# vaultah/replicat

Hardware: AMD Instinct MI355X
Metric: GiB/s chunked, device-resident streams (higher is better)
Workload: dtype u8

## Files before the change

include/replicat_chunker.h:

```cpp
#ifndef REPLICAT_CHUNKER_H
#define REPLICAT_CHUNKER_H

#include <stdint.h>

#ifdef __cplusplus
extern "C" {
#endif

#define RC_OK 0
#define RC_ERR_KEY_LENGTH 1
#define RC_ERR_MIN_GT_MAX 2
#define RC_ERR_BAD_KEY 3
#define RC_ERR_ARGUMENT 10
#define RC_ERR_ALIGN 11
#define RC_ERR_HIP 12
#define RC_ERR_OVERFLOW 13
#define RC_ERR_NO_DEVICE 14
#define RC_ERR_DEVICE_FAULT 15

#define RC_COUNT_OVERFLOW (-1)
#define RC_COUNT_FAULT (-3)

#define RC_OPEN 1u
#define RC_PIPELINED 2u
#define RC_PIPELINE_END 4u

typedef struct rc_chunker rc_chunker;

int rc_version(void);

const char *rc_build_id(void);

const char *rc_last_error(void);

int rc_chunker_create(uint64_t min_length, uint64_t max_length, const uint8_t *key,
                      uint64_t key_len, int device, rc_chunker **out);
void rc_chunker_destroy(rc_chunker *ch);

uint64_t rc_chunker_min_length(const rc_chunker *ch);
uint64_t rc_chunker_max_length(const rc_chunker *ch);

int rc_next_cut(rc_chunker *ch, const uint8_t *buffer, uint64_t size, int final,
                uint64_t *out_cut);

uint64_t rc_cut_capacity(const rc_chunker *ch, uint64_t n, const uint64_t *lens,
                         uint64_t *caps );

int rc_chunk_device(rc_chunker *ch, uint64_t n, const uint8_t *const *d_streams,
                    const uint64_t *lens, const uint64_t *last_piece, uint32_t flags,
                    uint64_t *d_cuts, int64_t *d_counts, void *hip_stream);

int rc_chunker_overlap(rc_chunker *ch, uint32_t reserve_cus);
uint32_t rc_chunker_overlap_cus(const rc_chunker *ch);
uint64_t rc_chunker_pipelined_calls(const rc_chunker *ch);

int rc_chunk_wait(rc_chunker *ch, void *hip_stream);

int rc_stream_create(int device, void **out_stream);
void rc_stream_destroy(void *stream);

int rc_chunk_host(rc_chunker *ch, uint64_t n, const uint8_t *const *streams,
                  const uint64_t *lens, const uint64_t *last_piece, uint32_t flags,
                  uint64_t *cuts, int64_t *counts);

int rc_chunker_check(rc_chunker *ch);

int rc_timing_enable(rc_chunker *ch, int enable);
int rc_timing_read_kernels(rc_chunker *ch, double *tile_ms, double *edge_ms, double *chain_ms,
                           uint64_t *calls);
int rc_timing_read(rc_chunker *ch, double *phase_a_ms, double *phase_b_ms, uint64_t *calls);

int rc_fill_splitmix(uint8_t *d_dst, uint64_t nbytes, uint64_t seed, uint64_t stream,
                     void *hip_stream);
int rc_fill_splitmix_streams(uint8_t *d_dst, uint64_t n, uint64_t nbytes, uint64_t slot,
                             uint64_t seed, uint64_t first_stream, uint64_t stream_step,
                             void *hip_stream);
int rc_fill_splitmix_at(uint8_t *d_dst, uint64_t nbytes, uint64_t seed, uint64_t stream,
                        uint64_t word0, void *hip_stream);

int rc_read_probe(const uint8_t *d_src, uint64_t nbytes, uint32_t *d_out, void *hip_stream);
int rc_chunker_read_probe(rc_chunker *ch, const uint8_t *d_src, uint64_t nbytes, uint32_t *d_out,
                          void *hip_stream);

uint64_t rc_keys_needed(uint64_t max_length, uint64_t L, uint64_t P);

uint64_t rc_host_key(const rc_chunker *ch, uint64_t d);

int rc_tile_records(rc_chunker *ch, uint64_t n, const uint8_t *const *d_streams,
                    const uint64_t *lens, const uint64_t *last_piece, uint64_t *keys,
                    uint64_t *js, uint64_t *gmax, uint64_t *ghot, uint64_t cap,
                    uint64_t *n_tiles);
uint32_t rc_group_hot_threshold(const rc_chunker *ch);
uint64_t rc_tile_keys(void);

int rc_tile_schedule(uint64_t n_tiles, uint32_t waves, uint32_t permille, uint32_t chunk,
                     uint32_t dyn_min, uint32_t *ranges, uint64_t cap, uint64_t *n_units);

int rc_tables_key(const uint8_t *key16, uint64_t n, const uint64_t *ds, uint64_t *out,
                  uint32_t *top16);

#ifdef __cplusplus
}
#endif

#endif
```

replicat_amd/_lib.py:

```python
import ctypes
import os
import threading

HERE = os.path.dirname(os.path.abspath(__file__))
LIB_PATH = os.environ.get('RC_LIB_PATH') or os.path.join(HERE, 'libreplicat_chunker.so')

RC_OK = 0
RC_ERR_KEY_LENGTH = 1
RC_ERR_MIN_GT_MAX = 2
RC_ERR_BAD_KEY = 3
RC_ERR_DIGEST_SIZE = 4
RC_ERR_B2_PARAM = 5
RC_ERR_KEY_SIZE = 6
RC_ERR_NONCE_SIZE = 7
RC_ERR_TAG = 8
RC_ERR_DIGEST_BITS = 9
RC_ERR_ARGUMENT = 10
RC_ERR_ALIGN = 11
RC_ERR_HIP = 12
RC_ERR_OVERFLOW = 13
RC_ERR_NO_DEVICE = 14
RC_ERR_DEVICE_FAULT = 15
RC_ERR_CORRUPT = 16
RC_ERR_INDEX_FULL = 17
RC_ERR_PROBE_BOUND = 18
RC_INDEX_ABSENT, RC_INDEX_EXHAUSTED = -1, -2
RC_GC_REFERENCED, RC_GC_DELETE, RC_GC_TAG_MISMATCH, RC_GC_EXHAUSTED = 0, 1, 2, 3
RC_COUNT_OVERFLOW = -1
RC_COUNT_FAULT = -3
RC_OPEN = 1
RC_PIPELINED = 2
RC_PIPELINE_END = 4
RC_DIGEST_SLOT = 64
RC_HASH_BLAKE2B, RC_HASH_SHA2, RC_HASH_SHA3 = 0, 1, 2
RC_CIPHER_NONE, RC_CIPHER_AES_GCM, RC_CIPHER_CHACHA20_POLY1305 = 0, 1, 2
RC_CHUNK_OK, RC_CHUNK_BAD_TAG, RC_CHUNK_CORRUPT = 0, 1, 2
RC_TABLE_OK, RC_TABLE_BAD_TAG, RC_TABLE_NOT_CANONICAL = 0, 1, 2
RC_PARTS_OK, RC_PARTS_NOT_CANONICAL = 0, 2
RC_PART_FIRST, RC_PART_LAST = 1, 2
RC_SNAPSHOT_PART_WORDS = 8
RC_SNAPSHOT_TEXT_DESC_BYTES = 32

_u64, _i64, _u32, _int, _p = ctypes.c_uint64, ctypes.c_int64, ctypes.c_uint32, ctypes.c_int, ctypes.c_void_p
SIGNATURES = {
    'rc_version': (_int, []),
    'rc_build_id': (ctypes.c_char_p, []),
    'rc_last_error': (ctypes.c_char_p, []),
    'rc_chunker_create': (_int, [_u64, _u64, _p, _u64, _int, ctypes.POINTER(_p)]),
    'rc_chunker_destroy': (None, [_p]),
    'rc_chunker_min_length': (_u64, [_p]),
    'rc_chunker_max_length': (_u64, [_p]),
    'rc_next_cut': (_int, [_p, _p, _u64, _int, ctypes.POINTER(_u64)]),
    'rc_cut_capacity': (_u64, [_p, _u64, _p, _p]),
    'rc_chunk_device': (_int, [_p, _u64, _p, _p, _p, _u32, _p, _p, _p]),
    'rc_chunk_host': (_int, [_p, _u64, _p, _p, _p, _u32, _p, _p]),
    'rc_chunker_overlap': (_int, [_p, _u32]),
    'rc_chunker_overlap_cus': (_u32, [_p]),
    'rc_chunker_pipelined_calls': (_u64, [_p]),
    'rc_chunker_check': (_int, [_p]),
    'rc_chunk_wait': (_int, [_p, _p]),
    'rc_stream_create': (_int, [_int, ctypes.POINTER(_p)]),
    'rc_stream_destroy': (None, [_p]),
    'rc_timing_enable': (_int, [_p, _int]),
    'rc_timing_read': (_int, [_p, ctypes.POINTER(ctypes.c_double), ctypes.POINTER(ctypes.c_double),
                              ctypes.POINTER(_u64)]),
    'rc_timing_read_kernels': (_int, [_p, ctypes.POINTER(ctypes.c_double),
                                      ctypes.POINTER(ctypes.c_double),
                                      ctypes.POINTER(ctypes.c_double), ctypes.POINTER(_u64)]),
    'rc_fill_splitmix': (_int, [_p, _u64, _u64, _u64, _p]),
    'rc_fill_splitmix_at': (_int, [_p, _u64, _u64, _u64, _u64, _p]),
    'rc_fill_splitmix_streams': (_int, [_p, _u64, _u64, _u64, _u64, _u64, _u64, _p]),
    'rc_read_probe': (_int, [_p, _u64, _p, _p]),
    'rc_chunker_read_probe': (_int, [_p, _p, _u64, _p, _p]),
    'rc_keys_needed': (_u64, [_u64, _u64, _u64]),
    'rc_host_key': (_u64, [_p, _u64]),
    'rc_tables_key': (_int, [_p, _u64, _p, _p, _p]),
    'rc_tile_records': (_int, [_p, _u64, _p, _p, _p, _p, _p, _p, _p, _u64, ctypes.POINTER(_u64)]),
    'rc_group_hot_threshold': (_u32, [_p]),
    'rc_tile_keys': (_u64, []),
    'rc_tile_schedule': (_int, [_u64, _u32, _u32, _u32, _u32, _p, _u64, ctypes.POINTER(_u64)]),
    'rc_blake2b_create': (_int, [_u32, _int, ctypes.POINTER(_p)]),
    'rc_blake2b_destroy': (None, [_p]),
    'rc_blake2b_digest_size': (_u32, [_p]),
    'rc_blake2b_device': (_int, [_p, _u64, _p, _p, _p, _p]),
    'rc_blake2b_host': (_int, [_p, _u64, _p, _p, _p]),
    'rc_blake2b_chunks': (_int, [_p, _p, _u64, _p, _p, _p, _p, _p, _p]),
    'rc_chunk_digest_host': (_int, [_p, _p, _u64, _p, _p, _p, _u32, _p, _p, _p]),
    'rc_blake2b_state_init': (_int, [_u32, _p, _u32, _p, _u32, _p, _u32, _p]),
    'rc_blake2b_update_device': (_int, [_p, _u64, _p, _p, _p, _p, _p, _p]),
    'rc_blake2b_timing_enable': (_int, [_p, _int]),
    'rc_blake2b_timing_read': (_int, [_p, ctypes.POINTER(ctypes.c_double), ctypes.POINTER(_u64)]),
    'rc_blake2b_derive_chunks': (_int, [_p, _p, _u64, _p, _p, _p, _p, _u32, _p, _p]),
    'rc_sha2_create': (_int, [_u32, _int, ctypes.POINTER(_p)]),
    'rc_sha3_create': (_int, [_u32, _int, ctypes.POINTER(_p)]),
    'rc_sha2_state_init': (_int, [_u32, _p]),
    'rc_sha3_state_init': (_int, [_u32, _p]),
    'rc_hash_destroy': (None, [_p]),
    'rc_hash_digest_size': (_u32, [_p]),
    'rc_hash_algorithm': (_u32, [_p]),
    'rc_hash_device': (_int, [_p, _u64, _p, _p, _p, _p]),
    'rc_hash_host': (_int, [_p, _u64, _p, _p, _p]),
    'rc_hash_chunks': (_int, [_p, _p, _u64, _p, _p, _p, _p, _p, _p]),
    'rc_hash_update_device': (_int, [_p, _u64, _p, _p, _p, _p, _p, _p]),
    'rc_hash_timing_enable': (_int, [_p, _int]),
    'rc_hash_timing_read': (_int, [_p, ctypes.POINTER(ctypes.c_double), ctypes.POINTER(_u64)]),
    'rc_gcm_create': (_int, [_u32, _u32, _int, ctypes.POINTER(_p)]),
    'rc_gcm_destroy': (None, [_p]),
    'rc_gcm_key_bytes': (_u32, [_p]),
    'rc_gcm_nonce_bytes': (_u32, [_p]),
    'rc_gcm_encrypt_device': (_int, [_p, _u64, _p, _p, _p, _p, _p, _p]),
    'rc_gcm_decrypt_device': (_int, [_p, _u64, _p, _p, _p, _p, _p, _p]),
    'rc_gcm_encrypt_host': (_int, [_p, _u64, _p, _p, _p, _p, _p]),
    'rc_gcm_decrypt_host': (_int, [_p, _u64, _p, _p, _p, _p, _p]),
    'rc_gcm_chunks_layout': (_u64, [_p, _p, _u64, _p, _p]),
    'rc_gcm_encrypt_chunks': (_int, [_p, _p, _u64, _p, _p, _p, _p, _p, _p, _p, _p]),
    'rc_gcm_encrypt_chunks_select': (_int, [_p, _p, _u64, _p, _p, _p, _p, _p, _p, _p, _p, _p, _p, _p]),
    'rc_gcm_timing_enable': (_int, [_p, _int]),
    'rc_gcm_timing_read': (_int, [_p, ctypes.POINTER(ctypes.c_double), ctypes.POINTER(_u64)]),
    'rc_chacha_create': (_int, [_int, ctypes.POINTER(_p)]),
    'rc_chacha_destroy': (None, [_p]),
    'rc_chacha_key_bytes': (_u32, [_p]),
    'rc_chacha_nonce_bytes': (_u32, [_p]),
    'rc_chacha_encrypt_device': (_int, [_p, _u64, _p, _p, _p, _p, _p, _p]),
    'rc_chacha_decrypt_device': (_int, [_p, _u64, _p, _p, _p, _p, _p, _p]),
    'rc_chacha_encrypt_host': (_int, [_p, _u64, _p, _p, _p, _p, _p]),
    'rc_chacha_decrypt_host': (_int, [_p, _u64, _p, _p, _p, _p, _p]),
    'rc_chacha_chunks_layout': (_u64, [_p, _p, _u64, _p, _p]),
    'rc_chacha_encrypt_chunks': (_int, [_p, _p, _u64, _p, _p, _p, _p, _p, _p, _p, _p]),
    'rc_chacha_encrypt_chunks_select': (_int, [_p, _p, _u64, _p, _p, _p, _p, _p, _p, _p, _p, _p, _p, _p]),
    'rc_chacha_timing_enable': (_int, [_p, _int]),
    'rc_chacha_timing_read': (_int, [_p, ctypes.POINTER(ctypes.c_double), ctypes.POINTER(_u64)]),
    'rc_poly1305_host': (_int, [_u64, _p, _p, _p, _p]),
    'rc_restore_create': (_int, [_p, _int, _p, _p, ctypes.POINTER(_p)]),
    'rc_restore_destroy': (None, [_p]),
    'rc_restore_overhead': (_u32, [_p]),
    'rc_restore_verify_device': (_int, [_p, _u64, _p, _p, _p, _p, _p, _p]),
    'rc_restore_verify_host': (_int, [_p, _u64, _p, _p, _p, _p, _p]),
    'rc_restore_timing_enable': (_int, [_p, _int]),
    'rc_restore_timing_read': (_int, [_p, ctypes.POINTER(ctypes.c_double), ctypes.POINTER(_u64)]),
    'rc_index_create': (_int, [_u32, _u64, _int, ctypes.POINTER(_p)]),
    'rc_index_destroy': (None, [_p]),
    'rc_index_name_bytes': (_u32, [_p]),
    'rc_index_used': (_u64, [_p]),
    'rc_index_add_host': (_int, [_p, _u64, _p, ctypes.POINTER(_u64)]),
    'rc_index_resolve_chunks': (_int, [_p, _p, _u64, _p, _p, _p, ctypes.POINTER(_u64), _p, _p, _p]),
    'rc_index_reserve': (_int, [_p, _u64]),
    'rc_index_lookup_device': (_int, [_p, _u64, _p, _p, _p]),
    'rc_index_resolve_names_device': (_int, [_p, _u64, _p, ctypes.POINTER(_u64), _p, _p, _p]),
    'rc_gc_create': (_int, [_u32, _u32, _p, _u32, _u64, _int, ctypes.POINTER(_p)]),
    'rc_gc_destroy': (None, [_p]),
    'rc_gc_name_bytes': (_u32, [_p]),
    'rc_gc_used': (_u64, [_p]),
    'rc_gc_capacity': (_u64, [_p]),
    'rc_gc_reference_host': (_int, [_p, _u64, _p]),
    'rc_gc_reference_device': (_int, [_p, _u64, _p]),
    'rc_gc_sweep_device': (_int, [_p, _u64, _p, _p, _u64, _p, _p, _p, _p]),
    'rc_gc_sweep_host': (_int, [_p, _u64, _p, _p, _p, _p, ctypes.POINTER(_u64)]),
    'rc_gc_unreferenced_host': (_int, [_p, _u64, _p, _p, _p, _p, ctypes.POINTER(_u64)]),
    'rc_gc_timing_enable': (_int, [_p, _int]),
    'rc_gc_timing_read': (_int, [_p, ctypes.POINTER(ctypes.c_double), ctypes.POINTER(ctypes.c_double),
                                 ctypes.POINTER(ctypes.c_double), ctypes.POINTER(_u64)]),
    'rc_snapshot_create': (_int, [_u32, _int, _p, _p, _int, ctypes.POINTER(_p)]),
    'rc_snapshot_destroy': (None, [_p]),
    'rc_snapshot_stride': (_u32, [_p]),
    'rc_snapshot_overhead': (_u32, [_p]),
    'rc_snapshot_table_count': (_u64, [_p, _u64]),
    'rc_snapshot_table_count_for': (_u64, [_u32, _u64]),
    'rc_snapshot_tables_device': (_int, [_p, _u64, _p, _p, _p, _p, _p, _p, _p, _p]),
    'rc_snapshot_tables_host': (_int, [_p, _u64, _p, _p, _p, _p, _p, _p]),
    'rc_snapshot_b64_device': (_int, [_p, _u64, _p, _p, _p, _p, _p]),
    'rc_snapshot_timing_enable': (_int, [_p, _int]),
    'rc_snapshot_timing_read': (_int, [_p, ctypes.POINTER(ctypes.c_double), ctypes.POINTER(ctypes.c_double),
                                       ctypes.POINTER(ctypes.c_double), ctypes.POINTER(_u64)]),
    'rc_snapshot_table_len': (_u64, [_p, _u64]),
    'rc_snapshot_table_len_for': (_u64, [_u32, _u64]),
    'rc_snapshot_b64_len': (_u64, [_u64]),
    'rc_snapshot_b64_encode_device': (_int, [_p, _u64, _p, _p, _p, _p]),
    'rc_snapshot_seal_tables_device': (_int, [_p, _u64, _p, _p, _p, _p, _p, _p, _p, _p]),
    'rc_snapshot_seal_tables_host': (_int, [_p, _u64, _p, _p, _p, _p, _p]),
    'rc_snapshot_write_timing_read': (_int, [_p, ctypes.POINTER(ctypes.c_double), ctypes.POINTER(ctypes.c_double),
                                             ctypes.POINTER(ctypes.c_double), ctypes.POINTER(_u64)]),
    'rc_snapshot_part_len_for': (_u32, [_u32, _u32, _u32, _u32]),
    'rc_snapshot_parts_capacity': (_u64, [_u64, _u64]),
    'rc_snapshot_parts_device': (_int, [_p, _u64, _p, _p, _u32, _u64, _p, _p, _p, _p, _p, _p, _p]),
    'rc_snapshot_data_len_device': (_int, [_p, _u64, _u64, _p, _p, _p, _p, _p, _p, _p]),
    'rc_snapshot_encode_data_device': (_int, [_p, _u64, _u64, _p, _p, _p, _p, _p, _p, _p, _p]),
    'rc_snapshot_data_timing_read': (_int, [_p, ctypes.POINTER(ctypes.c_double), ctypes.POINTER(ctypes.c_double),
                                            ctypes.POINTER(ctypes.c_double), ctypes.POINTER(_u64)]),
    'rc_snapshot_path_text_len_for': (_u64, [_p, _u64]),
    'rc_snapshot_int64_len_for': (_u32, [ctypes.c_int64]),
    'rc_snapshot_file_text_len_device': (_int, [_p, _u64, _p, _p, _p, _u32, _p, _p, _p, _u64, _u64, _p, _p]),
    'rc_snapshot_encode_file_text_device': (_int, [_p, _u64, _p, _p, _p, _u32, _p, _p, _p, _p, _u64, _p, _u64, _p, _p,
                                                   _p]),
    'rc_snapshot_file_text_timing_read': (_int, [_p, ctypes.POINTER(ctypes.c_double), ctypes.POINTER(ctypes.c_double),
                                                 ctypes.POINTER(_u64)]),
    'rc_snapshot_parts_room': (_u64, [_u64]),
    'rc_snapshot_find_parts_device': (_int, [_p, _u64, _p, _p, _p, _p, _p, _p, _p, _p]),
    'rc_snapshot_parse_parts_device': (_int, [_p, _u64, _p, _u64, _p, _p, _p, _p, _p, _p, _p, _p]),
    'rc_snapshot_part_sums_device': (_int, [_p, _u64, _u64, _p, _p, _p, _p, _p, _p, _p, _p, _p, _p, _p, _p]),
    'rc_snapshot_strip_parts_device': (_int, [_p, _u64, _p, _u64, _p, _p, _p, _p, _p, _p, _p, _p, _p]),
    'rc_snapshot_read_timing_read': (_int, [_p, ctypes.POINTER(ctypes.c_double), ctypes.POINTER(ctypes.c_double),
                                            ctypes.POINTER(ctypes.c_double), ctypes.POINTER(ctypes.c_double),
                                            ctypes.POINTER(_u64)]),
}



class ChunkerUnavailable(RuntimeError):
    """The HIP chunker library is not built or cannot run here."""


class ChunkerError(RuntimeError):
    def __init__(self, code, message):
        super().__init__(f'{message} (rc={code})')
        self.code = code


class ChunkCorrupted(ChunkerError):
    """A chunk's digest is not the one the snapshot recorded (RC_ERR_CORRUPT): the reference's
    ReplicatError('Chunk at ... is corrupted') (repository.py:1738-1739)."""


class ChunkerFault(ChunkerError):
    """The tile kernel took its fail-safe stop (RC_ERR_DEVICE_FAULT, RC_COUNT_FAULT): the call's
    cuts are not the reference's and must not be used."""


class IndexFull(ChunkerError):
    """A call would take a chunk-name index past its max_names (RC_ERR_INDEX_FULL): reserve()
    more room first."""


def check_counts(counts):
    import numpy as np
    c = np.asarray(counts).reshape(-1)
    if c.size == 0 or int(c.min()) >= 0:
        return
    if (c == RC_COUNT_FAULT).any():
        raise ChunkerFault(RC_ERR_DEVICE_FAULT, 'tile kernel fail-safe stop: a workgroup grab was '
                           'never published, so the call\'s cuts are not the reference\'s')
    raise ChunkerError(RC_ERR_OVERFLOW, f'stream {int(np.argmax(c < 0))} overflowed its cut capacity')


_lock = threading.Lock()
_lib = None


def lib():
    global _lib
    if _lib is not None:
        return _lib
    with _lock:
        if _lib is None:
            if not os.path.exists(LIB_PATH):
                raise ChunkerUnavailable(
                    f'{LIB_PATH} is missing: build it with `python -m replicat_amd.build` '
                    '(hipcc, gfx950); there is no CPU fallback')
            try:
                L = ctypes.CDLL(LIB_PATH)
            except OSError as e:
                raise ChunkerUnavailable(f'cannot load {LIB_PATH}: {e}') from e
            for name, (res, args) in SIGNATURES.items():
                f = getattr(L, name)
                f.restype = res
                f.argtypes = args
            _lib = L
    return _lib


def last_error():
    msg = lib().rc_last_error()
    return msg.decode('utf-8', 'replace') if msg else ''


def check(code):
    if code == RC_OK:
        return
    msg = last_error()
    if code in (RC_ERR_KEY_LENGTH, RC_ERR_MIN_GT_MAX, RC_ERR_BAD_KEY, RC_ERR_DIGEST_SIZE,
                RC_ERR_B2_PARAM, RC_ERR_KEY_SIZE, RC_ERR_NONCE_SIZE, RC_ERR_DIGEST_BITS):
        raise ValueError(msg)
    if code == RC_ERR_NO_DEVICE:
        raise ChunkerUnavailable(msg)
    if code == RC_ERR_DEVICE_FAULT:
        raise ChunkerFault(code, msg)
    if code == RC_ERR_CORRUPT:
        raise ChunkCorrupted(code, msg)
    if code == RC_ERR_INDEX_FULL:
        raise IndexFull(code, msg)
    raise ChunkerError(code, msg)
```

replicat_amd/csrc/capi.cpp:

```cpp
#include <hip/hip_runtime.h>

#include <algorithm>
#include <array>
#include <cstdarg>
#include <cstdio>
#include <cstdlib>
#include <cstring>
#include <mutex>
#include <vector>

#include "../../include/replicat_chunker.h"
#include "capi_internal.h"
#include "gclmul.h"
#include "knobs.h"

using namespace rc;

static_assert(kCountFault == RC_COUNT_FAULT && kCtrFaultsWord * 4 < 256, "counter buffer layout");

constexpr uint64_t kDigestSlot = RC_DIGEST_SLOT;

namespace {

thread_local char g_err[512];

void clmul64(uint64_t a, uint64_t b, uint64_t &lo, uint64_t &hi) {
    lo = hi = 0;
    for (int i = 0; i < 64; ++i)
        if ((b >> i) & 1) {
            lo ^= a << i;
            if (i) hi ^= a >> (64 - i);
        }
}

uint64_t key_linear(uint64_t k0, uint64_t d) {
    uint64_t lo, hi, rlo, rhi;
    clmul64(k0, d, lo, hi);
    clmul64(0x1B, hi, rlo, rhi);
    return lo ^ rlo;
}

void build_tables(uint64_t k0, uint64_t k1, KeyTables &t) {
    uint64_t col[64];
    for (int c = 0; c < 64; ++c) col[c] = key_linear(k0, 1ull << c);
    for (int b = 0; b < 4; ++b)
        for (int v = 0; v < 256; ++v) {
            uint64_t l = 0, h = 0;
            for (int i = 0; i < 8; ++i)
                if ((v >> i) & 1) {
                    l ^= col[8 * b + i];
                    h ^= col[32 + 8 * b + i];
                }
            if (b == 0) h ^= k1;
            t.tl[b][v] = l;
            t.th[b][v] = h;
            t.pf[b][v] = (uint32_t)((l >> 48) << 16) | (uint32_t)(h >> 48);
        }
}

uint64_t load_le64(const uint8_t *p) {
    uint64_t v = 0;
    for (int i = 7; i >= 0; --i) v = (v << 8) | p[i];
    return v;
}

uint64_t window_keys(uint64_t max_length) { return max_length >= 1 ? (max_length - 1) / 4 : 0; }

}

int rc_fail(int code, const char *fmt, ...) {
    va_list ap;
    va_start(ap, fmt);
    vsnprintf(g_err, sizeof g_err, fmt, ap);
    va_end(ap);
    return code;
}

namespace {

struct LiveHandle {
    void *h;
    void (*destroy)(void *);
};
std::mutex g_live_mu;
std::vector<LiveHandle> *g_live = nullptr;
bool g_exiting = false;

void destroy_live_at_exit() {
    std::vector<LiveHandle> left;
    {
        std::lock_guard<std::mutex> lock(g_live_mu);
        g_exiting = true;
        if (g_live) left.swap(*g_live);
    }
    for (auto it = left.rbegin(); it != left.rend(); ++it) it->destroy(it->h);
}

}

void rc_track(void *handle, void (*destroy)(void *)) {
    std::lock_guard<std::mutex> lock(g_live_mu);
    if (!g_live) {
        g_live = new std::vector<LiveHandle>();
        std::atexit(destroy_live_at_exit);
    }
    g_live->push_back({handle, destroy});
}

void rc_untrack(void *handle) {
    std::lock_guard<std::mutex> lock(g_live_mu);
    if (!g_live || g_exiting) return;
    for (size_t i = 0; i < g_live->size(); ++i)
        if ((*g_live)[i].h == handle) {
            (*g_live)[i] = g_live->back();
            g_live->pop_back();
            return;
        }
}

struct rc_chunker {
    uint64_t min_length = 0, max_length = 0, window = 0;
    bool small = false;
    bool groups = false;
    uint64_t seg_force = 0, ext_steps = 2;
    uint64_t seg_floor = 2;
    uint64_t k0 = 0, k1 = 0;
    int device = 0;
    Knobs knobs;
    TileSched sched;
    KeyTables tables;
    KeyTables *d_tables = nullptr;
    std::mutex mu;

    struct Workspace {
        PinnedBuf h_desc;
        DevBuf d_desc;
        DevBuf d_records;
        DevBuf d_scratch;
        DevBuf d_seg_counts;
        DevBuf d_ctr;
        bool ctr_dirty = false;
        uint64_t epoch = 0;
        std::vector<uint64_t> xtiles;
        hipEvent_t done = nullptr;
        bool pending = false;
        bool piped = false;
    } ws[2];
    unsigned next_ws = 0;

    DevBuf d_buf, d_out;
    PinnedBuf h_out;

    DevBuf d_stage[2], d_hcuts[2], d_hcounts[2], d_hdig[2];
    hipStream_t hstream[2] = {nullptr, nullptr};

    hipStream_t cstream = nullptr;
    hipEvent_t uploaded[2] = {nullptr, nullptr};

    uint32_t reserve_req = 0;
    uint32_t reserve = 0, tile_cus = 0;
    hipStream_t tstream = nullptr, xstream = nullptr;
    hipStream_t tstream2 = nullptr;
    hipStream_t fstream = nullptr;
    hipEvent_t in_ev[2] = {nullptr, nullptr}, tiled[2] = {nullptr, nullptr};
    uint64_t pipelined_calls = 0;
    bool overlap_failed = false;

    bool timing = false;
    std::vector<hipEvent_t> ev_pool, ev_pool_sync;
    std::vector<std::array<hipEvent_t, 4>> ev_rec;
};

namespace {

struct Plan {
    uint64_t n = 0, n_tiles = 0, total_cap = 0, max_len = 0;
    uint64_t n_segs = 0, scratch_entries = 0;
    uint64_t seg_bytes = 0, seg_cap = 0;
    bool any_multi = false;
    size_t bytes = 0;
};

StreamDesc desc_view(void *base, uint64_t n) {
    uint64_t *u = static_cast<uint64_t *>(base);
    StreamDesc d;
    d.ptr = reinterpret_cast<const uint8_t *const *>(u);
    d.len = u + n;
    d.last = u + 2 * n;
    d.jneed = u + 3 * n;
    d.tile_base = u + 4 * n;
    d.cut_base = u + 5 * n + 1;
    d.cut_cap = u + 6 * n + 1;
    d.seg_base = u + 7 * n + 1;
    d.scratch_base = u + 8 * n + 2;
    d.xtiles = u + 9 * n + 2;
    return d;
}

bool argmax_bound(uint64_t max_length, uint64_t L, uint64_t P, uint64_t &bound) {
    bool any = false;
    bound = 0;
    if (P >= max_length) {
        any = true;
        bound = P - max_length;
    }
    if (L >= 2 * max_length) {
        const uint64_t b2 = L - 2 * max_length;
        if (!any || b2 > bound) bound = b2;
        any = true;
    }
    return any;
}

uint64_t cut_cap_of(uint64_t min_length, uint64_t L) {
    const uint64_t step = std::max<uint64_t>(4, (min_length + 3) & ~3ull);
    return L / step + 3;
}

int validate_streams(uint64_t n, const uint8_t *const *ptrs, const uint64_t *lens,
                     const uint64_t *last, bool device_aligned) {
    if (n && (!ptrs || !lens)) return rc_fail(RC_ERR_ARGUMENT, "null stream arrays");
    if (n >= (1ull << 31))
        return rc_fail(RC_ERR_ARGUMENT, "too many streams in one call: %llu", (unsigned long long)n);
    for (uint64_t i = 0; i < n; ++i) {
        const uint64_t P = last ? last[i] : 0;
        if (P > lens[i]) return rc_fail(RC_ERR_ARGUMENT, "stream %llu: last piece start %llu > length %llu",
                                        (unsigned long long)i, (unsigned long long)P,
                                        (unsigned long long)lens[i]);
        if (lens[i] && !ptrs[i]) return rc_fail(RC_ERR_ARGUMENT, "stream %llu: null pointer", (unsigned long long)i);
        if (device_aligned && lens[i] && (reinterpret_cast<uintptr_t>(ptrs[i]) & 15))
            return rc_fail(RC_ERR_ALIGN, "stream %llu: device pointer not 16-byte aligned",
                           (unsigned long long)i);
    }
    return 0;
}

using Workspace = rc_chunker::Workspace;

Workspace &acquire_ws(rc_chunker *ch) {
    Workspace &w = ch->ws[ch->next_ws & 1];
    ++ch->next_ws;
    return w;
}

int stage_descriptors(rc_chunker *ch, Workspace &ws, uint64_t n, const uint8_t *const *ptrs,
                      const uint64_t *lens, const uint64_t *last, Plan &plan, bool open = false,
                      bool single = false, uint64_t walkers = 0) {
    plan.n = n;
    if (ws.pending) {
        RC_HIP_TRY(hipEventSynchronize(ws.done));
        ws.pending = false;
    }
    std::vector<uint64_t> &xt = ws.xtiles;
    xt.clear();
    {
        uint64_t tiles = 0;
        for (uint64_t i = 0; i < n; ++i) {
            const uint64_t L = lens[i], P = open ? L : (last ? last[i] : 0);
            const uint64_t jneed = rc_keys_needed(ch->max_length, L, P);
            const uint64_t nt = jneed ? jneed / kTileKeys + 1 : 0;
            const uint64_t jmax = L >= 8 ? (L - 4) / 4 : 0;
            auto fast = [&](uint64_t t) { return L >= 8 && t * kTileKeys + kTileKeys - 1 <= jmax; };
            if (nt && !fast(0)) xt.push_back(tiles);
            if (nt > 1 && !fast(nt - 1)) xt.push_back(tiles + nt - 1);
            tiles += nt;
        }
    }
    plan.bytes = (9 * n + 3 + xt.size()) * sizeof(uint64_t);
    if (int rc = ws.h_desc.ensure(plan.bytes)) return rc;
    uint64_t *u = static_cast<uint64_t *>(ws.h_desc.p);
    u[9 * n + 2] = xt.size();
    std::copy(xt.begin(), xt.end(), u + 9 * n + 3);
    {
        const uint64_t kChainWalkers = walkers ? walkers : 4096;
        uint64_t total = 0;
        for (uint64_t i = 0; i < n; ++i) {
            uint64_t b = 0;
            const uint64_t P = open ? lens[i] : (last ? last[i] : 0);
            if (argmax_bound(ch->max_length, lens[i], P, b)) total += b;
        }
        uint64_t seg = ch->seg_force ? ch->seg_force
                                     : std::max<uint64_t>(total / kChainWalkers / 4 * 5 + 4, 1);
        const uint64_t floor_len =
            ch->max_length < (1ull << 60) ? ch->seg_floor * ch->max_length : ~0ull >> 2;
        if (!ch->seg_force) seg = std::max(seg, std::max<uint64_t>(floor_len, 4ull << 20));
        seg = std::max<uint64_t>((seg + 3) & ~3ull, 4);
        const uint64_t step = std::max<uint64_t>(4, (ch->min_length + 3) & ~3ull);
        plan.seg_bytes = seg;
        plan.seg_cap = seg / step + ch->ext_steps + 4;
    }
    uint64_t tiles = 0, cuts = 0, segs = 0, scratch = 0;
    plan.any_multi = false;
    for (uint64_t i = 0; i < n; ++i) {
        const uint64_t L = lens[i], P = open ? L : (last ? last[i] : 0);
        uint64_t bound = 0, nseg = 1;
        if (!single && argmax_bound(ch->max_length, L, P, bound)) nseg = bound / plan.seg_bytes + 1;
        u[7 * n + 1 + i] = segs;
        u[8 * n + 2 + i] = scratch;
        segs += nseg;
        if (nseg > 1) {
            scratch += nseg * plan.seg_cap;
            plan.any_multi = true;
        }
        const uint64_t jneed = rc_keys_needed(ch->max_length, L, P);
        plan.max_len = std::max(plan.max_len, L);
        u[i] = reinterpret_cast<uint64_t>(ptrs[i]);
        u[n + i] = L;
        u[2 * n + i] = P;
        u[3 * n + i] = jneed;
        u[4 * n + i] = tiles;
        tiles += jneed ? jneed / kTileKeys + 1 : 0;
        const uint64_t cap = cut_cap_of(ch->min_length, L);
        u[5 * n + 1 + i] = cuts;
        u[6 * n + 1 + i] = cap;
        cuts += cap;
    }
    u[5 * n] = tiles;
    u[8 * n + 1] = segs;
    if (tiles >= (1ull << 32) - (1ull << 20))
        return rc_fail(RC_ERR_ARGUMENT, "too many bytes in one call: %llu tiles", (unsigned long long)tiles);
    plan.n_tiles = tiles;
    plan.total_cap = cuts;
    plan.n_segs = segs;
    plan.scratch_entries = scratch;
    return 0;
}

GroupRecord *group_records(Workspace &ws, const Plan &plan) {
    return reinterpret_cast<GroupRecord *>(static_cast<char *>(ws.d_records.p) +
                                           (plan.n_tiles + 1) * sizeof(TileRecord));
}

uint32_t *tie_lists(Workspace &ws, const Plan &plan) {
    return reinterpret_cast<uint32_t *>(group_records(ws, plan) + plan.n_tiles + 1);
}

size_t records_bytes(const Plan &plan) {
    return (plan.n_tiles + 1) * (sizeof(TileRecord) + sizeof(GroupRecord)) +
           rc_tie_list_words(plan.n_tiles) * 4;
}

int ensure_ctr(Workspace &ws, hipStream_t st) {
    size_t zero = kCtrFaultsWord * 4;
    if (!ws.d_ctr.p) {
        if (int rc = ws.d_ctr.ensure(256)) return rc;
        ws.ctr_dirty = true;
        zero = 256;
    }
    if (ws.ctr_dirty) {
        RC_HIP_TRY(hipMemsetAsync(ws.d_ctr.p, 0, zero, st));
        ws.ctr_dirty = false;
    }
    return 0;
}

const char kFaultMsg[] =
    "tile kernel fail-safe stop: a workgroup grab was never published, so the launch's records "
    "are incomplete and its cuts are not the reference's";

int grab_fault(Workspace &ws) {
    if (!ws.d_ctr.p || !ws.epoch) return 0;
    uint64_t stamp = 0;
    RC_HIP_TRY(hipMemcpy(&stamp, static_cast<uint32_t *>(ws.d_ctr.p) + kCtrStampWord, 8,
                         hipMemcpyDeviceToHost));
    return stamp == ws.epoch ? rc_fail(RC_ERR_DEVICE_FAULT, "%s", kFaultMsg) : 0;
}

int take_faults(Workspace &ws, uint32_t &n) {
    n = 0;
    if (!ws.d_ctr.p) return 0;
    uint32_t *w = static_cast<uint32_t *>(ws.d_ctr.p) + kCtrFaultsWord;
    RC_HIP_TRY(hipMemcpy(&n, w, 4, hipMemcpyDeviceToHost));
    if (n) RC_HIP_TRY(hipMemset(w, 0, 4));
    return 0;
}

int abandon_launch(Workspace &ws, hipStream_t ts, hipStream_t xs, int rc) {
    (void)hipStreamSynchronize(ts);
    if (xs != ts) (void)hipStreamSynchronize(xs);
    ws.ctr_dirty = true;
    ws.pending = false;
    return rc;
}

constexpr uint64_t kLaneMinStreams = 256;

int upload_and_launch(rc_chunker *ch, Workspace &ws, const Plan &plan, ChainParams prm,
                      uint64_t *d_cuts, int64_t *d_counts, hipStream_t stream,
                      bool pipelined = false, bool end = false) {
    if (int rc = ws.d_desc.ensure(plan.bytes)) return rc;
    if (int rc = ws.d_records.ensure(records_bytes(plan))) return rc;
    if (int rc = ws.d_scratch.ensure(std::max<uint64_t>(plan.scratch_entries, 1) * 8)) return rc;
    if (int rc = ws.d_seg_counts.ensure(std::max<uint64_t>(plan.n_segs, 1) * 40)) return rc;
    const int wi = &ws == &ch->ws[0] ? 0 : 1;
    if (!ch->cstream) RC_HIP_TRY(hipStreamCreateWithFlags(&ch->cstream, hipStreamNonBlocking));
    if (!ch->uploaded[wi]) RC_HIP_TRY(hipEventCreateWithFlags(&ch->uploaded[wi], hipEventDisableTiming));
    RC_HIP_TRY(hipMemcpyAsync(ws.d_desc.p, ws.h_desc.p, plan.bytes, hipMemcpyHostToDevice, ch->cstream));
    RC_HIP_TRY(hipEventRecord(ch->uploaded[wi], ch->cstream));
    hipStream_t ts = stream, xs = stream;
    if (pipelined) {
        ts = wi == 1 && ch->tstream2 ? ch->tstream2 : ch->tstream;
        xs = end ? ch->fstream : ch->xstream;
        if (hipStreamQuery(stream) != hipSuccess) {
            RC_HIP_TRY(hipEventRecord(ch->in_ev[wi], stream));
            RC_HIP_TRY(hipStreamWaitEvent(ts, ch->in_ev[wi], 0));
        }
        RC_HIP_TRY(hipStreamWaitEvent(xs, ch->ws[wi ^ 1].done, 0));
    }
    RC_HIP_TRY(hipStreamWaitEvent(ts, ch->uploaded[wi], 0));
    if (int rc = ensure_ctr(ws, ts)) return rc;
    prm.fault = reinterpret_cast<const uint64_t *>(static_cast<uint32_t *>(ws.d_ctr.p) + kCtrStampWord);
    prm.epoch = ++ws.epoch;
    const StreamDesc d = desc_view(ws.d_desc.p, plan.n);
    std::array<hipEvent_t, 4> ev{};
    if (ch->timing) {
        for (int k = 0; k < 4; ++k) {
            std::vector<hipEvent_t> &pool = k == 1 ? ch->ev_pool_sync : ch->ev_pool;
            if (pool.empty()) {
                RC_HIP_TRY(k == 1 ? hipEventCreate(&ev[k])
                                  : hipEventCreateWithFlags(&ev[k], hipEventDisableSystemFence));
            } else {
                ev[k] = pool.back();
                pool.pop_back();
            }
        }
        RC_HIP_TRY(hipEventRecord(ev[0], ts));
    }
    GroupRecord *grp = ch->groups ? group_records(ws, plan) : nullptr;
    prm.grp = grp;
    prm.n_tiles = plan.n_tiles;
    switch (ch->knobs[knLaneChain]) {
    case 1: prm.lane = 0u; break;
    case 2: prm.lane = 2u; break;
    default: prm.lane = plan.n >= kLaneMinStreams ? 1u : 0u;
    }
    prm.lean = ch->small && plan.max_len < (16ull << 30) ? 1u : 0u;
    prm.hot = group_hot_threshold(ch->window);
    if (int rc = rc_launch_tiles(ch->d_tables, d, plan.n, plan.n_tiles,
                                 static_cast<TileRecord *>(ws.d_records.p), grp, prm.hot, tie_lists(ws, plan),
                                 static_cast<uint32_t *>(ws.d_ctr.p), prm.epoch, ts,
                                 ch->timing ? ev[1] : nullptr,
                                 pipelined ? ch->tile_cus : 0u, xs,
                                 !pipelined ? nullptr : ch->timing ? ev[1] : ch->tiled[wi], ch->sched))
        return abandon_launch(ws, ts, xs, rc);
    const Workspace &prev = ch->ws[wi ^ 1];
    if (!pipelined && prev.piped && hipStreamWaitEvent(xs, prev.done, 0) != hipSuccess)
        return abandon_launch(ws, ts, xs, rc_fail(RC_ERR_HIP, "hipStreamWaitEvent failed"));
    if (ch->timing && hipEventRecord(ev[2], xs) != hipSuccess)
        return abandon_launch(ws, ts, xs, rc_fail(RC_ERR_HIP, "hipEventRecord failed"));
    const uint32_t join = (ch->knobs[knJoinWalk] ? RC_JOIN_WALK_ONLY : 0u) |
                          (ch->knobs[knRepair] ? RC_JOIN_REPAIR : 0u);
    if (int rc = rc_launch_chain(ch->d_tables, d, plan.n, prm, plan.n_segs,
                                 static_cast<const TileRecord *>(ws.d_records.p), d_cuts, d_counts,
                                 static_cast<uint64_t *>(ws.d_scratch.p),
                                 static_cast<uint64_t *>(ws.d_seg_counts.p), plan.any_multi, join, xs))
        return abandon_launch(ws, ts, xs, rc);
    if (hipEventRecord(ws.done, xs) != hipSuccess)
        return abandon_launch(ws, ts, xs, rc_fail(RC_ERR_HIP, "hipEventRecord failed"));
    ws.pending = true;
    ws.piped = pipelined;
    if (ch->timing) {
        RC_HIP_TRY(hipEventRecord(ev[3], xs));
        ch->ev_rec.push_back(ev);
    }
    return 0;
}

int setup_overlap(rc_chunker *ch) {
    const uint32_t want = ch->reserve_req ? ch->reserve_req : (uint32_t)ch->knobs[knOverlapCus];
    if (ch->tstream && ch->reserve == want) return 0;
    int cus = 0;
    RC_HIP_TRY(hipDeviceGetAttribute(&cus, hipDeviceAttributeMultiprocessorCount, ch->device));
    if (want == 0 || (int)want >= cus)
        return rc_fail(RC_ERR_ARGUMENT, "overlap: %u reserved CUs of %d", want, cus);
    if (ch->tstream) {
        if (ch->tstream2) {
            RC_HIP_TRY(hipStreamSynchronize(ch->tstream2));
            (void)hipStreamDestroy(ch->tstream2);
            ch->tstream2 = nullptr;
        }
        RC_HIP_TRY(hipStreamSynchronize(ch->tstream));
        RC_HIP_TRY(hipStreamSynchronize(ch->xstream));
        (void)hipStreamDestroy(ch->tstream);
        (void)hipStreamDestroy(ch->xstream);
        ch->tstream = ch->xstream = nullptr;
    }
    std::vector<uint32_t> tm((cus + 31) / 32, 0u), xm((cus + 31) / 32, 0u);
    for (int i = 0; i < cus; ++i) ((uint32_t)i < want ? xm : tm)[i / 32] |= 1u << (i % 32);
    const int64_t tmask = ch->knobs[knTileMask];
    if (tmask == 1)
        for (int i = 0; i < cus; ++i) tm[i / 32] |= 1u << (i % 32);
    if (tmask == 2)
        RC_HIP_TRY(hipStreamCreateWithFlags(&ch->tstream, hipStreamNonBlocking));
    else
        RC_HIP_TRY(hipExtStreamCreateWithCUMask(&ch->tstream, (uint32_t)tm.size(), tm.data()));
    const hipError_t ex = hipExtStreamCreateWithCUMask(&ch->xstream, (uint32_t)xm.size(), xm.data());
    if (ex != hipSuccess) {
        (void)hipStreamDestroy(ch->tstream);
        ch->tstream = ch->xstream = nullptr;
        return rc_fail(RC_ERR_HIP, "hipExtStreamCreateWithCUMask failed: %s", hipGetErrorString(ex));
    }
    if (ch->knobs[knTileStreams] == 2 &&
        (tmask == 2 ? hipStreamCreateWithFlags(&ch->tstream2, hipStreamNonBlocking)
                    : hipExtStreamCreateWithCUMask(&ch->tstream2, (uint32_t)tm.size(), tm.data())) !=
            hipSuccess)
        ch->tstream2 = nullptr;
    if (!ch->fstream) RC_HIP_TRY(hipStreamCreateWithFlags(&ch->fstream, hipStreamNonBlocking));
    for (int i = 0; i < 2; ++i) {
        if (!ch->in_ev[i]) RC_HIP_TRY(hipEventCreateWithFlags(&ch->in_ev[i], hipEventDisableTiming));
        if (!ch->tiled[i]) RC_HIP_TRY(hipEventCreateWithFlags(&ch->tiled[i], hipEventDisableTiming));
    }
    ch->reserve = want;
    ch->tile_cus = (uint32_t)cus - (tmask ? 0u : want);
    return 0;
}

ChainParams chain_params(const rc_chunker *ch, const Plan &plan, uint64_t max_steps,
                         uint32_t flags = 0) {
    ChainParams p;
    p.open = (flags & RC_OPEN) ? 1u : 0u;
    p.min_length = ch->min_length;
    p.max_length = ch->max_length;
    p.window = ch->window;
    p.max_steps = max_steps;
    p.seg_bytes = plan.seg_bytes;
    p.seg_cap = plan.seg_cap;
    p.ext_steps = ch->ext_steps;
    p.grp = nullptr;
    p.n_tiles = 0;
    p.lean = 0;
    p.lane = 0;
    p.hot = 0;
    p.fault = nullptr;
    p.epoch = 0;
    return p;
}

}

extern "C" {

int rc_version(void) { return 300; }

#ifndef RC_BUILD_ID
#define RC_BUILD_ID "unknown"
#endif
static const char kBuildId[] = "RC_BUILD_ID:" RC_BUILD_ID;
const char *rc_build_id(void) { return kBuildId + 12; }

const char *rc_last_error(void) { return g_err; }

uint32_t rc_group_hot_threshold(const rc_chunker *ch) { return ch ? group_hot_threshold(ch->window) : 0u; }

uint64_t rc_keys_needed(uint64_t max_length, uint64_t L, uint64_t P) {
    const uint64_t T = window_keys(max_length);
    if (T == 0 || L < 8) return 0;
    bool any = false;
    uint64_t bound = 0;
    if (P >= max_length) {
        any = true;
        bound = P - max_length;
    }
    if (L >= 2 * max_length) {
        const uint64_t b2 = L - 2 * max_length;
        if (!any || b2 > bound) bound = b2;
        any = true;
    }
    if (!any) return 0;
    const uint64_t jneed = bound / 4 + T, jmax = (L - 4) / 4;
    return std::min(jneed, jmax);
}

int rc_chunker_create(uint64_t min_length, uint64_t max_length, const uint8_t *key,
                      uint64_t key_len, int device, rc_chunker **out) {
    if (!out) return rc_fail(RC_ERR_ARGUMENT, "null output handle");
    *out = nullptr;
    if (key_len != 16 || !key) return rc_fail(RC_ERR_KEY_LENGTH, "key must contain exactly 16 characters");
    if (min_length > max_length)
        return rc_fail(RC_ERR_MIN_GT_MAX, "Minimum length is greater than the maximum one");
    const uint64_t k0 = load_le64(key), k1 = load_le64(key + 8);
    if (k0 == 0) return rc_fail(RC_ERR_BAD_KEY, "Bad key contents");
    Knobs knobs;
    if (read_knobs(knobs, g_err, sizeof g_err)) return RC_ERR_ARGUMENT;

    int ndev = 0;
    if (hipGetDeviceCount(&ndev) != hipSuccess || ndev <= 0)
        return rc_fail(RC_ERR_NO_DEVICE, "no HIP device available (the chunker runs on MI355X only)");
    if (device < 0 || device >= ndev) return rc_fail(RC_ERR_NO_DEVICE, "device %d out of range", device);
    hipDeviceProp_t prop;
    RC_HIP_TRY(hipGetDeviceProperties(&prop, device));
    if (std::strncmp(prop.gcnArchName, "gfx950", 6) != 0)
        return rc_fail(RC_ERR_NO_DEVICE, "device %d is %s, not gfx950", device, prop.gcnArchName);

    rc_chunker *ch = new rc_chunker();
    ch->min_length = min_length;
    ch->max_length = max_length;
    ch->window = window_keys(max_length);
    ch->knobs = knobs;
    ch->small = ch->window / kTileKeys + 3 <= 64;
    ch->groups = knobs[knTileGroups] == 0 ? ch->small : knobs[knTileGroups] == 2;
    if (knobs[knChainLean] == 1) ch->small = false;
    ch->sched.permille = (uint32_t)knobs[knTileStatic];
    ch->sched.chunk = (uint32_t)knobs[knTileChunk];
    ch->sched.dyn_min = (uint32_t)knobs[knTileDynMin];
    ch->sched.group = (uint32_t)knobs[knTileGroup];
    ch->k0 = k0;
    ch->k1 = k1;
    ch->device = device;
    build_tables(k0, k1, ch->tables);
    ch->seg_force = (uint64_t)knobs[knSegmentBytes];
    ch->ext_steps = (uint64_t)knobs[knSegmentExt];
    ch->seg_floor = (uint64_t)knobs[knSegmentFloor];
    {
        DeviceGuard g(device);
        hipError_t e = hipMalloc(&ch->d_tables, sizeof(KeyTables));
        if (e == hipSuccess)
            e = hipMemcpy(ch->d_tables, &ch->tables, sizeof(KeyTables), hipMemcpyHostToDevice);
        for (auto &w : ch->ws)
            if (e == hipSuccess) e = hipEventCreateWithFlags(&w.done, hipEventDisableTiming);
        if (e != hipSuccess) {
            rc_chunker_destroy(ch);
            return rc_fail(RC_ERR_HIP, "device setup failed: %s", hipGetErrorString(e));
        }
    }
    rc_track(ch, [](void *h) { rc_chunker_destroy(static_cast<rc_chunker *>(h)); });
    *out = ch;
    return RC_OK;
}

void rc_chunker_destroy(rc_chunker *ch) {
    if (!ch) return;
    teardown(ch, [ch] {
        if (ch->d_tables) (void)hipFree(ch->d_tables);
        for (auto &w : ch->ws) {
            w.d_desc.release();
            w.d_records.release();
            w.d_scratch.release();
            w.d_seg_counts.release();
            w.d_ctr.release();
            w.h_desc.release();
            if (w.done) (void)hipEventDestroy(w.done);
        }
        ch->d_buf.release();
        ch->d_out.release();
        for (int i = 0; i < 2; ++i) {
            ch->d_stage[i].release();
            ch->d_hcuts[i].release();
            ch->d_hcounts[i].release();
            ch->d_hdig[i].release();
            if (ch->hstream[i]) (void)hipStreamDestroy(ch->hstream[i]);
        }
        ch->h_out.release();
        if (ch->cstream) (void)hipStreamDestroy(ch->cstream);
        if (ch->tstream) (void)hipStreamDestroy(ch->tstream);
        if (ch->tstream2) (void)hipStreamDestroy(ch->tstream2);
        if (ch->xstream) (void)hipStreamDestroy(ch->xstream);
        if (ch->fstream) (void)hipStreamDestroy(ch->fstream);
        for (auto e : ch->uploaded)
            if (e) (void)hipEventDestroy(e);
        for (int i = 0; i < 2; ++i) {
            if (ch->in_ev[i]) (void)hipEventDestroy(ch->in_ev[i]);
            if (ch->tiled[i]) (void)hipEventDestroy(ch->tiled[i]);
        }
        for (auto &r : ch->ev_rec)
            for (auto e : r) (void)hipEventDestroy(e);
        for (auto e : ch->ev_pool) (void)hipEventDestroy(e);
        for (auto e : ch->ev_pool_sync) (void)hipEventDestroy(e);
    });
    delete ch;
}

uint64_t rc_chunker_min_length(const rc_chunker *ch) { return ch ? ch->min_length : 0; }
uint64_t rc_chunker_max_length(const rc_chunker *ch) { return ch ? ch->max_length : 0; }

uint64_t rc_host_key(const rc_chunker *ch, uint64_t d) {
    const uint32_t lo = (uint32_t)d, hi = (uint32_t)(d >> 32);
    uint64_t k = 0;
    for (int b = 0; b < 4; ++b) k ^= ch->tables.tl[b][(lo >> (8 * b)) & 255] ^ ch->tables.th[b][(hi >> (8 * b)) & 255];
    return k;
}

int rc_tables_key(const uint8_t *key16, uint64_t n, const uint64_t *ds, uint64_t *out,
                  uint32_t *top16) {
    if (!key16 || (n && (!ds || !out))) return rc_fail(RC_ERR_ARGUMENT, "null argument");
    KeyTables *t = new KeyTables;
    build_tables(load_le64(key16), load_le64(key16 + 8), *t);
    for (uint64_t i = 0; i < n; ++i) {
        const uint32_t lo = (uint32_t)ds[i], hi = (uint32_t)(ds[i] >> 32);
        uint64_t k = 0;
        uint32_t el = 0, eh = 0;
        for (int b = 0; b < 4; ++b) {
            k ^= t->tl[b][(lo >> (8 * b)) & 255] ^ t->th[b][(hi >> (8 * b)) & 255];
            el ^= t->pf[b][(lo >> (8 * b)) & 255];
            eh ^= t->pf[b][(hi >> (8 * b)) & 255];
        }
        out[i] = k;
        if (top16) top16[i] = ((el & 0xffff0000u) ^ (eh << 16)) >> 16;
    }
    delete t;
    return RC_OK;
}

uint64_t rc_cut_capacity(const rc_chunker *ch, uint64_t n, const uint64_t *lens, uint64_t *caps) {
    uint64_t total = 0;
    for (uint64_t i = 0; i < n; ++i) {
        const uint64_t c = cut_cap_of(ch->min_length, lens[i]);
        if (caps) caps[i] = c;
        total += c;
    }
    return total;
}

int rc_next_cut(rc_chunker *ch, const uint8_t *buffer, uint64_t size, int final, uint64_t *out_cut) {
    if (!ch || !out_cut) return rc_fail(RC_ERR_ARGUMENT, "null argument");
    if (size && !buffer) return rc_fail(RC_ERR_ARGUMENT, "null buffer");
    const uint64_t mn = ch->min_length, mx = ch->max_length;
    if (final && size < 2 * mx) {
        *out_cut = size <= mx ? size : (size < mx + mn ? size / 2 : mx);
        return RC_OK;
    }
    if (!final && size < mx) {
        *out_cut = 0;
        return RC_OK;
    }
    if (ch->window == 0) {
        *out_cut = (mn + 3) & ~3ull;
        return RC_OK;
    }
    std::lock_guard<std::mutex> lock(ch->mu);
    DeviceGuard g(ch->device);
    const uint64_t ncopy = std::min<uint64_t>(size, 4 * ch->window + 4);
    if (int rc = ch->d_buf.ensure(ncopy + 16)) return rc;
    if (int rc = ch->d_out.ensure(64)) return rc;
    if (int rc = ch->h_out.ensure(64)) return rc;
    hipStream_t stream = nullptr;
    RC_HIP_TRY(hipMemcpyAsync(ch->d_buf.p, buffer, ncopy, hipMemcpyHostToDevice, stream));
    const uint8_t *ptr = static_cast<const uint8_t *>(ch->d_buf.p);
    const uint64_t L = ncopy, P = ncopy;
    Plan plan;
    Workspace &ws = acquire_ws(ch);
    if (int rc = stage_descriptors(ch, ws, 1, &ptr, &L, &P, plan, false, true)) return rc;
    uint64_t *d_cut = static_cast<uint64_t *>(ch->d_out.p);
    int64_t *d_count = reinterpret_cast<int64_t *>(d_cut + 1);
    const bool timing = ch->timing;
    ch->timing = false;
    int rc = upload_and_launch(ch, ws, plan, chain_params(ch, plan, 0), d_cut, d_count, stream);
    ch->timing = timing;
    if (rc) return rc;
    RC_HIP_TRY(hipMemcpyAsync(ch->h_out.p, d_cut, 16, hipMemcpyDeviceToHost, stream));
    RC_HIP_TRY(hipStreamSynchronize(stream));
    const uint64_t *h = static_cast<const uint64_t *>(ch->h_out.p);
    if ((int64_t)h[1] == kCountFault) return rc_fail(RC_ERR_DEVICE_FAULT, "%s", kFaultMsg);
    if ((int64_t)h[1] != 1) return rc_fail(RC_ERR_OVERFLOW, "device chain returned %lld cuts", (long long)h[1]);
    *out_cut = h[0];
    return RC_OK;
}

int rc_chunk_device(rc_chunker *ch, uint64_t n, const uint8_t *const *d_streams,
                    const uint64_t *lens, const uint64_t *last_piece, uint32_t flags,
                    uint64_t *d_cuts, int64_t *d_counts, void *hip_stream) {
    if (!ch) return rc_fail(RC_ERR_ARGUMENT, "null chunker");
    if (n == 0) return RC_OK;
    if (!d_cuts || !d_counts) return rc_fail(RC_ERR_ARGUMENT, "null output arrays");
    const bool open = (flags & RC_OPEN) != 0;
    if (int rc = validate_streams(n, d_streams, lens, open ? nullptr : last_piece, true)) return rc;
    std::lock_guard<std::mutex> lock(ch->mu);
    DeviceGuard g(ch->device);
    const bool all = ch->knobs[knPipeAll] != 0;
    bool pipelined = (flags & RC_PIPELINED) != 0 && (all || !ch->groups);
    if (pipelined && !ch->overlap_failed && setup_overlap(ch) != 0) {
        ch->overlap_failed = true;
        fprintf(stderr, "replicat_amd: pipelined calls run in sequence: %s\n", g_err);
    }
    if (ch->overlap_failed && !ch->tstream) pipelined = false;
    if (pipelined && !all) {
        uint64_t tiles = 0;
        for (uint64_t i = 0; i < n; ++i) {
            const uint64_t P = open ? lens[i] : (last_piece ? last_piece[i] : 0);
            const uint64_t j = rc_keys_needed(ch->max_length, lens[i], P);
            tiles += j ? j / kTileKeys + 1 : 0;
        }
        if (tiles < 16ull * ch->tile_cus) pipelined = false;
    }
    ch->pipelined_calls += pipelined ? 1 : 0;
    Plan plan;
    Workspace &ws = acquire_ws(ch);
    if (int rc = stage_descriptors(ch, ws, n, d_streams, lens, last_piece, plan, open, false,
                                   pipelined ? 16ull * ch->reserve : 0))
        return rc;
    return upload_and_launch(ch, ws, plan, chain_params(ch, plan, ~0ull, flags), d_cuts, d_counts,
                             static_cast<hipStream_t>(hip_stream), pipelined,
                             (flags & RC_PIPELINE_END) != 0);
}

int rc_stream_create(int device, void **out_stream) {
    if (!out_stream) return rc_fail(RC_ERR_ARGUMENT, "null output stream");
    *out_stream = nullptr;
    if (int rc = check_device(device)) return rc;
    DeviceGuard g(device);
    int cus = 0;
    RC_HIP_TRY(hipDeviceGetAttribute(&cus, hipDeviceAttributeMultiprocessorCount, device));
    std::vector<uint32_t> mask((cus + 31) / 32, 0u);
    for (int i = 0; i < cus; ++i) mask[i / 32] |= 1u << (i % 32);
    hipStream_t s = nullptr;
    RC_HIP_TRY(hipExtStreamCreateWithCUMask(&s, (uint32_t)mask.size(), mask.data()));
    rc_track(s, [](void *h) { rc_stream_destroy(h); });
    *out_stream = s;
    return RC_OK;
}

void rc_stream_destroy(void *stream) {
    if (!stream) return;
    rc_untrack(stream);
    (void)hipStreamSynchronize(static_cast<hipStream_t>(stream));
    (void)hipStreamDestroy(static_cast<hipStream_t>(stream));
}

int rc_chunker_overlap(rc_chunker *ch, uint32_t reserve_cus) {
    if (!ch) return rc_fail(RC_ERR_ARGUMENT, "null chunker");
    std::lock_guard<std::mutex> lock(ch->mu);
    DeviceGuard g(ch->device);
    ch->reserve_req = reserve_cus;
    const int rc = setup_overlap(ch);
    ch->overlap_failed = rc != 0 && !ch->tstream;
    return rc;
}

uint32_t rc_chunker_overlap_cus(const rc_chunker *ch) { return ch ? ch->reserve : 0u; }

uint64_t rc_chunker_pipelined_calls(const rc_chunker *ch) { return ch ? ch->pipelined_calls : 0; }

int rc_chunker_check(rc_chunker *ch) {
    if (!ch) return rc_fail(RC_ERR_ARGUMENT, "null chunker");
    std::lock_guard<std::mutex> lock(ch->mu);
    DeviceGuard g(ch->device);
    uint32_t faults = 0;
    for (auto &w : ch->ws) {
        if (w.pending) RC_HIP_TRY(hipEventSynchronize(w.done));
        uint32_t n = 0;
        if (int rc = take_faults(w, n)) return rc;
        faults += n;
    }
    if (faults)
        return rc_fail(RC_ERR_DEVICE_FAULT, "%s (%u call(s) since the last check)", kFaultMsg, faults);
    return RC_OK;
}

int rc_chunk_wait(rc_chunker *ch, void *hip_stream) {
    if (!ch) return rc_fail(RC_ERR_ARGUMENT, "null chunker");
    std::lock_guard<std::mutex> lock(ch->mu);
    DeviceGuard g(ch->device);
    for (auto &w : ch->ws)
        RC_HIP_TRY(hipStreamWaitEvent(static_cast<hipStream_t>(hip_stream), w.done, 0));
    return RC_OK;
}

}

namespace {

int chunk_host_impl(rc_chunker *ch, rc_hasher *hasher, uint64_t n, const uint8_t *const *streams,
                    const uint64_t *lens, const uint64_t *last_piece, uint32_t flags,
                    uint64_t *cuts, int64_t *counts, uint8_t *digests) {
    if (!ch) return rc_fail(RC_ERR_ARGUMENT, "null chunker");
    if (n == 0) return RC_OK;
    if (!cuts || !counts) return rc_fail(RC_ERR_ARGUMENT, "null output arrays");
    if (hasher && !digests) return rc_fail(RC_ERR_ARGUMENT, "null digest array");
    const bool open = (flags & RC_OPEN) != 0;
    if (int rc = validate_streams(n, streams, lens, open ? nullptr : last_piece, false)) return rc;
    std::lock_guard<std::mutex> lock(ch->mu);
    DeviceGuard g(ch->device);
    for (int i = 0; i < 2; ++i)
        if (!ch->hstream[i]) RC_HIP_TRY(hipStreamCreateWithFlags(&ch->hstream[i], hipStreamNonBlocking));
    struct Drain {
        rc_chunker *ch;
        bool armed = true;
        ~Drain() {
            if (!armed) return;
            for (hipStream_t s : ch->hstream)
                if (s) (void)hipStreamSynchronize(s);
        }
    } drain{ch};

    const uint64_t budget = uint64_t(ch->knobs[knHostBatchBytes]);
    std::vector<uint64_t> cut_base(n + 1, 0);
    for (uint64_t i = 0; i < n; ++i) cut_base[i + 1] = cut_base[i] + cut_cap_of(ch->min_length, lens[i]);

    struct Batch {
        uint64_t first = 0, count = 0;
    } inflight[2];
    bool busy[2] = {false, false};
    std::vector<const uint8_t *> dptr;
    std::vector<uint64_t> off;

    auto finish = [&](int slot) -> int {
        if (!busy[slot]) return 0;
        RC_HIP_TRY(hipStreamSynchronize(ch->hstream[slot]));
        busy[slot] = false;
        const Batch &b = inflight[slot];
        for (uint64_t i = 0; i < b.count; ++i) {
            if (counts[b.first + i] == kCountFault) return rc_fail(RC_ERR_DEVICE_FAULT, "%s", kFaultMsg);
            if (counts[b.first + i] < 0)
                return rc_fail(RC_ERR_OVERFLOW, "stream %llu overflowed its cut capacity",
                               (unsigned long long)(b.first + i));
        }
        return 0;
    };

    uint64_t i = 0;
    int slot = 0;
    while (i < n) {
        uint64_t j = i, bytes = 0;
        while (j < n && (j == i || bytes + ((lens[j] + 15) & ~15ull) <= budget)) {
            bytes += (lens[j] + 15) & ~15ull;
            ++j;
        }
        if (int rc = finish(slot)) return rc;
        const uint64_t nb = j - i;
        if (int rc = ch->d_stage[slot].ensure(bytes + 16)) return rc;
        const uint64_t ncut = cut_base[j] - cut_base[i];
        if (int rc = ch->d_hcuts[slot].ensure(ncut * 8)) return rc;
        if (int rc = ch->d_hcounts[slot].ensure(nb * 8)) return rc;
        hipStream_t st = ch->hstream[slot];
        dptr.resize(nb);
        uint64_t o = 0;
        for (uint64_t k = 0; k < nb; ++k) {
            uint8_t *dst = static_cast<uint8_t *>(ch->d_stage[slot].p) + o;
            dptr[k] = dst;
            if (lens[i + k]) RC_HIP_TRY(hipMemcpyAsync(dst, streams[i + k], lens[i + k], hipMemcpyHostToDevice, st));
            o += (lens[i + k] + 15) & ~15ull;
        }
        Plan plan;
        Workspace &ws = acquire_ws(ch);
        if (int rc = stage_descriptors(ch, ws, nb, dptr.data(), lens + i,
                                       last_piece ? last_piece + i : nullptr, plan, open))
            return rc;
        uint64_t *dc = static_cast<uint64_t *>(ch->d_hcuts[slot].p);
        int64_t *dn = static_cast<int64_t *>(ch->d_hcounts[slot].p);
        if (int rc = upload_and_launch(ch, ws, plan, chain_params(ch, plan, ~0ull, flags), dc, dn, st))
            return rc;
        if (hasher) {
            if (int rc = ch->d_hdig[slot].ensure(ncut * kDigestSlot)) return rc;
            uint8_t *dd = static_cast<uint8_t *>(ch->d_hdig[slot].p);
            std::vector<uint64_t> cb(nb);
            for (uint64_t k = 0; k < nb; ++k) cb[k] = cut_base[i + k] - cut_base[i];
            uint64_t bytes = 0, longest = 0;
            for (uint64_t k = 0; k < nb; ++k) {
                bytes += lens[i + k];
                longest = std::max(longest, lens[i + k]);
            }
            if (int rc = rc_hasher_enqueue_chunks(hasher, nb, dptr.data(), cb.data(), dc, dn, ncut,
                                                  bytes, std::min(longest, ch->max_length), dd, st))
                return rc;
            RC_HIP_TRY(hipMemcpyAsync(digests + cut_base[i] * kDigestSlot, dd, ncut * kDigestSlot,
                                      hipMemcpyDeviceToHost, st));
        }
        RC_HIP_TRY(hipMemcpyAsync(cuts + cut_base[i], dc, ncut * 8, hipMemcpyDeviceToHost, st));
        RC_HIP_TRY(hipMemcpyAsync(counts + i, dn, nb * 8, hipMemcpyDeviceToHost, st));
        inflight[slot] = {i, nb};
        busy[slot] = true;
        i = j;
        slot ^= 1;
    }
    if (int rc = finish(0)) return rc;
    if (int rc = finish(1)) return rc;
    drain.armed = false;
    return RC_OK;
}

}

extern "C" {

int rc_chunk_host(rc_chunker *ch, uint64_t n, const uint8_t *const *streams, const uint64_t *lens,
                  const uint64_t *last_piece, uint32_t flags, uint64_t *cuts, int64_t *counts) {
    return chunk_host_impl(ch, nullptr, n, streams, lens, last_piece, flags, cuts, counts, nullptr);
}

int rc_chunk_digest_host(rc_chunker *ch, rc_hasher *h, uint64_t n, const uint8_t *const *streams,
                         const uint64_t *lens, const uint64_t *last_piece, uint32_t flags,
                         uint64_t *cuts, int64_t *counts, uint8_t *digests) {
    if (!h) return rc_fail(RC_ERR_ARGUMENT, "null hasher");
    return chunk_host_impl(ch, h, n, streams, lens, last_piece, flags, cuts, counts, digests);
}

uint64_t rc_tile_keys(void) { return kTileKeys; }

int rc_tile_records(rc_chunker *ch, uint64_t n, const uint8_t *const *d_streams,
                    const uint64_t *lens, const uint64_t *last_piece, uint64_t *keys,
                    uint64_t *js, uint64_t *gmax, uint64_t *ghot, uint64_t cap,
                    uint64_t *n_tiles) {
    if (!ch || !n_tiles) return rc_fail(RC_ERR_ARGUMENT, "null argument");
    if (int rc = validate_streams(n, d_streams, lens, last_piece, true)) return rc;
    std::lock_guard<std::mutex> lock(ch->mu);
    DeviceGuard g(ch->device);
    Plan plan;
    Workspace &ws = acquire_ws(ch);
    if (int rc = stage_descriptors(ch, ws, n, d_streams, lens, last_piece, plan)) return rc;
    if (int rc = ws.d_desc.ensure(plan.bytes)) return rc;
    if (int rc = ws.d_records.ensure(records_bytes(plan))) return rc;
    RC_HIP_TRY(hipMemcpy(ws.d_desc.p, ws.h_desc.p, plan.bytes, hipMemcpyHostToDevice));
    if (int rc = ensure_ctr(ws, nullptr)) return rc;
    GroupRecord *d_grp = ch->groups ? group_records(ws, plan) : nullptr;
    if (plan.n_tiles)
        RC_HIP_TRY(hipMemset(ws.d_records.p, 0xab, (plan.n_tiles + 1) * sizeof(TileRecord)));
    if (int rc = rc_launch_tiles(ch->d_tables, desc_view(ws.d_desc.p, n), n, plan.n_tiles,
                                 static_cast<TileRecord *>(ws.d_records.p), d_grp,
                                 group_hot_threshold(ch->window), tie_lists(ws, plan),
                                 static_cast<uint32_t *>(ws.d_ctr.p), ++ws.epoch, nullptr, nullptr, 0u,
                                 nullptr, nullptr, ch->sched))
        return abandon_launch(ws, nullptr, nullptr, rc);
    RC_HIP_TRY(hipDeviceSynchronize());
    if (int rc = grab_fault(ws)) return rc;
    std::vector<TileRecord> h(plan.n_tiles);
    std::vector<GroupRecord> hg(plan.n_tiles, GroupRecord{~0ull, {~0ull, ~0ull, ~0ull, ~0ull}, 0ull});
    if (plan.n_tiles) {
        RC_HIP_TRY(hipMemcpy(h.data(), ws.d_records.p, plan.n_tiles * sizeof(TileRecord),
                             hipMemcpyDeviceToHost));
        if (d_grp)
            RC_HIP_TRY(hipMemcpy(hg.data(), d_grp, plan.n_tiles * sizeof(GroupRecord), hipMemcpyDeviceToHost));
    }
    *n_tiles = plan.n_tiles;
    for (uint64_t t = 0; t < plan.n_tiles && t < cap; ++t) {
        keys[t] = h[t].key;
        js[t] = h[t].j;
        if (gmax) gmax[t] = hg[t].max;
        if (ghot)
            for (int g = 0; g < kTileGroups; ++g) ghot[kTileGroups * t + g] = hg[t].hot[g];
    }
    return RC_OK;
}

int rc_timing_enable(rc_chunker *ch, int enable) {
    if (!ch) return rc_fail(RC_ERR_ARGUMENT, "null chunker");
    ch->timing = enable != 0;
    return RC_OK;
}

int rc_timing_read_kernels(rc_chunker *ch, double *tile_ms, double *edge_ms, double *chain_ms,
                           uint64_t *calls) {
    if (!ch) return rc_fail(RC_ERR_ARGUMENT, "null chunker");
    std::lock_guard<std::mutex> lock(ch->mu);
    DeviceGuard g(ch->device);
    double t[3] = {0, 0, 0};
    for (auto &r : ch->ev_rec) {
        RC_HIP_TRY(hipEventSynchronize(r[3]));
        for (int k = 0; k < 3; ++k) {
            float x = 0;
            RC_HIP_TRY(hipEventElapsedTime(&x, r[k], r[k + 1]));
            t[k] += x;
        }
        for (int k = 0; k < 4; ++k) (k == 1 ? ch->ev_pool_sync : ch->ev_pool).push_back(r[k]);
    }
    if (tile_ms) *tile_ms = t[0];
    if (edge_ms) *edge_ms = t[1];
    if (chain_ms) *chain_ms = t[2];
    if (calls) *calls = ch->ev_rec.size();
    ch->ev_rec.clear();
    return RC_OK;
}

int rc_timing_read(rc_chunker *ch, double *phase_a_ms, double *phase_b_ms, uint64_t *calls) {
    double tile = 0, edge = 0, chain = 0;
    if (int rc = rc_timing_read_kernels(ch, &tile, &edge, &chain, calls)) return rc;
    if (phase_a_ms) *phase_a_ms = tile + edge;
    if (phase_b_ms) *phase_b_ms = chain;
    return RC_OK;
}

int rc_read_probe(const uint8_t *d_src, uint64_t nbytes, uint32_t *d_out, void *hip_stream) {
    if (nbytes && (!d_src || !d_out)) return rc_fail(RC_ERR_ARGUMENT, "null argument");
    if (reinterpret_cast<uintptr_t>(d_src) & 15) return rc_fail(RC_ERR_ALIGN, "source not 16-byte aligned");
    const Knobs &k = process_knobs();
    TileSched sched;
    sched.permille = (uint32_t)k[knTileStatic];
    sched.chunk = (uint32_t)k[knTileChunk];
    sched.dyn_min = (uint32_t)k[knTileDynMin];
    sched.group = (uint32_t)k[knTileGroup];
    return rc_launch_read_probe(d_src, nbytes, d_out, (uint32_t)k[knProbeBlock], sched, hip_stream);
}

int rc_chunker_read_probe(rc_chunker *ch, const uint8_t *d_src, uint64_t nbytes, uint32_t *d_out,
                          void *hip_stream) {
    if (!ch) return rc_fail(RC_ERR_ARGUMENT, "null chunker");
    if (nbytes && (!d_src || !d_out)) return rc_fail(RC_ERR_ARGUMENT, "null argument");
    if (reinterpret_cast<uintptr_t>(d_src) & 15) return rc_fail(RC_ERR_ALIGN, "source not 16-byte aligned");
    DeviceGuard g(ch->device);
    return rc_launch_read_probe(d_src, nbytes, d_out, 0, ch->sched, hip_stream);
}

int rc_fill_splitmix(uint8_t *d_dst, uint64_t nbytes, uint64_t seed, uint64_t stream, void *hip_stream) {
// ... 23 lines not shown
```

replicat_amd/csrc/gclmul.h:

```cpp
#pragma once
#include <stdint.h>

namespace rc {

#ifndef RC_TILE_ITERS
#define RC_TILE_ITERS 16
#endif
constexpr int kTileIters = RC_TILE_ITERS;
constexpr int kTileKeys = 64 * 4 * kTileIters;
constexpr int kWaveSize = 64;
constexpr int kTileWaves = 16;
constexpr int kChainWaves = 4;
#ifndef RC_TILE_GROUPS
#define RC_TILE_GROUPS 4
#endif
constexpr int kTileGroups = RC_TILE_GROUPS;
constexpr int kGroupKeys = kTileKeys / kTileGroups;

constexpr uint32_t kPfBytes = 131072;
constexpr uint32_t kFullOff = kPfBytes;
constexpr uint32_t kFullBytes = 2 * 4 * 256 * 8;
constexpr uint32_t kTileLdsBytes = kPfBytes + kFullBytes;

struct KeyTables {
    uint64_t tl[4][256];
    uint64_t th[4][256];
    uint32_t pf[4][256];
};

struct StreamDesc {
    const uint8_t *const *ptr;
    const uint64_t *len;
    const uint64_t *last;
    const uint64_t *jneed;
    const uint64_t *tile_base;
    const uint64_t *cut_base;
    const uint64_t *cut_cap;
    const uint64_t *seg_base;
    const uint64_t *scratch_base;
    const uint64_t *xtiles;
};

struct TileRecord {
    uint64_t key;
    uint64_t j;
};

struct GroupRecord {
    uint64_t max;
    uint64_t hot[kTileGroups];
    uint64_t pad;
};
static_assert(kTileGroups % 2 == 0 && sizeof(GroupRecord) % 16 == 0, "group record layout");

__host__ __device__ inline uint32_t group_hot_threshold(uint64_t window) {
    if (window < (uint64_t)kTileKeys) return 0;
    const uint64_t below = (10 * 65536 + window - 1) / window;
    return below >= 65536 ? 0u : (uint32_t)(65536 - below);
}

struct ChainParams {
    uint64_t min_length;
    uint64_t max_length;
    uint64_t window;
    uint64_t max_steps;
    uint64_t seg_bytes;
    uint64_t seg_cap;
    uint64_t ext_steps;
    const GroupRecord *grp;
    uint64_t n_tiles;
    uint32_t open;
    uint32_t lean;
    uint32_t lane;
    uint32_t hot;
    const uint64_t *fault;
    uint64_t epoch;
};

constexpr uint32_t kCtrErrWord = 32, kCtrStampWord = 34, kCtrFaultsWord = 36;
constexpr int64_t kCountFault = -3;

struct TileSched {
    uint32_t permille = 0;
    uint32_t chunk = 3;
    uint32_t dyn_min = 0;
    uint32_t group = 64;
};

__host__ __device__ inline uint64_t splitmix64(uint64_t x) {
    uint64_t z = x + 0x9E3779B97F4A7C15ull;
    z = (z ^ (z >> 30)) * 0xBF58476D1CE4E5B9ull;
    z = (z ^ (z >> 27)) * 0x94D049BB133111EBull;
    return z ^ (z >> 31);
}

}

extern "C" {
int rc_launch_tiles(const rc::KeyTables *d_tables, rc::StreamDesc desc, uint64_t n_streams,
                    uint64_t n_tiles, rc::TileRecord *d_records, rc::GroupRecord *d_grp,
                    uint32_t hot, uint32_t *d_xlist, uint32_t *d_ctr, uint64_t epoch,
                    void *stream, void *mid_event, uint32_t cus, void *edge_stream, void *tiled,
                    rc::TileSched sched);
uint64_t rc_tie_list_words(uint64_t n_tiles);
enum : uint32_t { RC_JOIN_WALK_ONLY = 1, RC_JOIN_REPAIR = 2 };
int rc_launch_chain(const rc::KeyTables *d_tables, rc::StreamDesc desc, uint64_t n_streams,
                    rc::ChainParams prm, uint64_t n_segs, const rc::TileRecord *d_records,
                    uint64_t *d_cuts, int64_t *d_counts, uint64_t *d_scratch,
                    uint64_t *d_seg_counts, bool any_multi, uint32_t join, void *stream);
int rc_launch_fill(uint8_t *d_dst, uint64_t nbytes, uint64_t seed, uint64_t stream_id,
                   uint64_t word0, void *stream);
int rc_launch_fill_streams(uint8_t *d_dst, uint64_t n, uint64_t nbytes, uint64_t slot,
                           uint64_t seed, uint64_t id0, uint64_t id_step, void *stream);
int rc_launch_read_probe(const uint8_t *d_src, uint64_t nbytes, uint32_t *d_out, uint32_t block,
                         rc::TileSched sched, void *stream);
}
```

replicat_amd/csrc/kernels.hip:

```cpp
#include <hip/hip_runtime.h>
#include <stdint.h>

#include "capi_internal.h"
#include "gclmul.h"
#include "diag.h"

using namespace rc;

namespace {

typedef uint32_t u32x4 __attribute__((ext_vector_type(4)));
typedef __attribute__((address_space(1))) const u32x4 gu32x4;
typedef __attribute__((address_space(1))) const uint32_t gu32;

constexpr int kStreamAux = RC_DIAG_STREAM_AUX;

__device__ __forceinline__ __amdgpu_buffer_rsrc_t tile_rsrc(const uint8_t *base,
                                                             uint32_t bytes = 0xffffffffu) {
    return __builtin_amdgcn_make_buffer_rsrc(const_cast<uint8_t *>(base), 0, bytes, 0x00020000);
}
__device__ __forceinline__ u32x4 ring_load(__amdgpu_buffer_rsrc_t r, uint32_t lane_off, int it) {
    return __builtin_amdgcn_raw_buffer_load_b128(r, lane_off, it * 1024, kStreamAux);
}

__device__ __forceinline__ uint32_t lane_id() { return threadIdx.x & 63; }

__device__ __forceinline__ uint32_t max3_u32(uint32_t a, uint32_t b, uint32_t c) {
    uint32_t r;
    asm("v_max3_u32 %0, %1, %2, %3" : "=v"(r) : "v"(a), "v"(b), "v"(c));
    return r;
}


__device__ __forceinline__ uint64_t lane_u64(uint64_t v, int l) {
    const uint32_t lo = (uint32_t)__builtin_amdgcn_readlane((uint32_t)v, l);
    const uint32_t hi = (uint32_t)__builtin_amdgcn_readlane((uint32_t)(v >> 32), l);
    return ((uint64_t)hi << 32) | lo;
}

typedef __attribute__((address_space(4))) const uint64_t cu64;
__device__ __forceinline__ uint64_t sload(const uint64_t *p) { return *(cu64 *)(p); }
__device__ __forceinline__ const uint8_t *sload_ptr(const uint8_t *const *p) {
    return reinterpret_cast<const uint8_t *>(sload(reinterpret_cast<const uint64_t *>(p)));
}

__device__ __forceinline__ uint32_t ld_u32(const uint8_t *p) {
    return *(gu32 *)(p);
}
__device__ __forceinline__ gu32x4 *as_global_x4(const uint8_t *p) { return (gu32x4 *)(p); }

__device__ __forceinline__ uint64_t full_key(const uint64_t *__restrict__ tl,
                                             const uint64_t *__restrict__ th, uint32_t wlo,
                                             uint32_t whi) {
    return tl[wlo & 255] ^ tl[256 + ((wlo >> 8) & 255)] ^ tl[512 + ((wlo >> 16) & 255)] ^
           tl[768 + (wlo >> 24)] ^ th[whi & 255] ^ th[256 + ((whi >> 8) & 255)] ^
           th[512 + ((whi >> 16) & 255)] ^ th[768 + (whi >> 24)];
}

template <int kCtrl, int kRowMask>
__device__ __forceinline__ uint64_t dpp_u64(uint64_t v) {
    const uint32_t lo = (uint32_t)__builtin_amdgcn_update_dpp((int)(uint32_t)v, (int)(uint32_t)v,
                                                              kCtrl, kRowMask, 0xf, false);
    const uint32_t hi = (uint32_t)__builtin_amdgcn_update_dpp((int)(uint32_t)(v >> 32),
                                                              (int)(uint32_t)(v >> 32), kCtrl,
                                                              kRowMask, 0xf, false);
    return ((uint64_t)hi << 32) | lo;
}

template <int kCtrl, int kRowMask>
__device__ __forceinline__ void best_step(uint64_t &k, uint64_t &j) {
    const uint64_t ko = dpp_u64<kCtrl, kRowMask>(k), jo = dpp_u64<kCtrl, kRowMask>(j);
    if (ko > k || (ko == k && jo < j)) {
        k = ko;
        j = jo;
    }
}

__device__ __forceinline__ void wave_best(uint64_t &k, uint64_t &j) {
    best_step<0x111, 0xf>(k, j);
    best_step<0x112, 0xf>(k, j);
    best_step<0x114, 0xf>(k, j);
    best_step<0x118, 0xf>(k, j);
    best_step<0x142, 0xa>(k, j);
    best_step<0x143, 0xc>(k, j);
    k = lane_u64(k, 63);
    j = lane_u64(j, 63);
}


__shared__ __attribute__((aligned(16))) uint32_t s_tile_lds[kTileLdsBytes / 4];

__device__ __forceinline__ uint32_t pf_lds(uint32_t byte_addr) {
    return *reinterpret_cast<const uint32_t *>(reinterpret_cast<const char *>(s_tile_lds) +
                                               byte_addr);
}

__device__ __forceinline__ void pf_addrs(uint32_t w, uint32_t lb_a, uint32_t lb_b, uint32_t *a) {
    a[0] = __builtin_amdgcn_perm(w, lb_a, 0x0c020400u);
    a[1] = __builtin_amdgcn_perm(w, lb_a, 0x0c020500u) + 128;
    a[2] = __builtin_amdgcn_perm(w, lb_b, 0x0c020600u);
    a[3] = __builtin_amdgcn_perm(w, lb_b, 0x0c020700u) + 128;
}
__device__ __forceinline__ uint32_t pf_gather(const uint32_t *a) {
    return __builtin_amdgcn_bitop3_b32(pf_lds(a[0]), pf_lds(a[1]), pf_lds(a[2]), 0x96) ^ pf_lds(a[3]);
}

__device__ __forceinline__ uint32_t pf_entry(uint32_t w, uint32_t lb_a, uint32_t lb_b) {
    const uint32_t a0 = __builtin_amdgcn_perm(w, lb_a, 0x0c020400u);
    const uint32_t a1 = __builtin_amdgcn_perm(w, lb_a, 0x0c020500u);
    const uint32_t a2 = __builtin_amdgcn_perm(w, lb_b, 0x0c020600u);
    const uint32_t a3 = __builtin_amdgcn_perm(w, lb_b, 0x0c020700u);
    return pf_lds(a0) ^ pf_lds(a1 + 128) ^ pf_lds(a2) ^ pf_lds(a3 + 128);
}

__shared__ __attribute__((aligned(16))) uint32_t s_chain_lds[1024 + 4096];

__device__ __forceinline__ uint32_t pfc_entry(const uint32_t *pf, uint32_t w) {
    return pf[w & 255] ^ pf[256 + ((w >> 8) & 255)] ^ pf[512 + ((w >> 16) & 255)] ^
           pf[768 + (w >> 24)];
}

__device__ __forceinline__ void stage_chain_tables(const KeyTables *tab) {
    const uint32_t nt = blockDim.x;
    const uint32_t *gpf = &tab->pf[0][0];
    for (uint32_t i = threadIdx.x; i < 1024u; i += nt) s_chain_lds[i] = gpf[i];
    uint64_t *full = reinterpret_cast<uint64_t *>(s_chain_lds + 1024);
    const uint64_t *gfull = &tab->tl[0][0];
    for (uint32_t i = threadIdx.x; i < 2048u; i += nt) full[i] = gfull[i];
    __syncthreads();
}

template <typename I>
__device__ __forceinline__ void take_best(uint64_t k, I j, uint64_t &bk, I &bj) {
    if (k > bk || (k == bk && j < bj)) {
        bk = k;
        bj = j;
    }
}

constexpr int kScanUnroll = 16;
#ifndef RC_CHAIN_SCAN_UNROLL
#define RC_CHAIN_SCAN_UNROLL 4
#endif
constexpr int kChainScanUnroll = RC_CHAIN_SCAN_UNROLL;

template <int kScanUnroll>
__device__ __forceinline__ void scan_ranges(const uint64_t *tl, const uint64_t *th,
                                            const uint8_t *base, uint64_t a0, uint64_t b0,
                                            uint64_t a1, uint64_t b1, uint64_t &bk,
                                            uint64_t &bj) {
    const bool e0 = a0 <= b0, e1 = a1 <= b1;
    if (!e0 && !e1) return;
    if (!e0) a0 = b0 = a1;
    if (!e1) a1 = b1 = a0;
    const uint64_t lane = lane_id();
    for (uint64_t r = 0;; r += 64 * kScanUnroll) {
        const bool live0 = e0 && a0 + r <= b0, live1 = e1 && a1 + r <= b1;
        if (!live0 && !live1) break;
        uint2 w0[kScanUnroll], w1[kScanUnroll];
#pragma unroll
        for (int u = 0; u < kScanUnroll; ++u) {
            const uint64_t j0 = min(a0 + r + 64 * u + lane, b0);
            const uint64_t j1 = min(a1 + r + 64 * u + lane, b1);
            w0[u].x = ld_u32(base + 4 * j0 - 4);
            w0[u].y = ld_u32(base + 4 * j0);
            w1[u].x = ld_u32(base + 4 * j1 - 4);
            w1[u].y = ld_u32(base + 4 * j1);
        }
#pragma unroll
        for (int u = 0; u < kScanUnroll; ++u) {
            const uint64_t j0 = a0 + r + 64 * u + lane, j1 = a1 + r + 64 * u + lane;
            if (e0 && j0 <= b0) take_best(full_key(tl, th, w0[u].x, w0[u].y), j0, bk, bj);
            if (e1 && j1 <= b1) take_best(full_key(tl, th, w1[u].x, w1[u].y), j1, bk, bj);
        }
    }
}

#ifndef RC_REC_UNROLL
#define RC_REC_UNROLL 4
#endif
constexpr int kRecUnroll = RC_REC_UNROLL;

__device__ __forceinline__ void scan_records(const TileRecord *rec, uint64_t t_lo, uint64_t t_hi,
                                             uint64_t &bk, uint64_t &bj) {
    const uint64_t lane = lane_id();
    for (uint64_t r = t_lo; r < t_hi; r += 64 * kRecUnroll) {
        TileRecord v[kRecUnroll];
#pragma unroll
        for (int u = 0; u < kRecUnroll; ++u) v[u] = rec[min(r + 64 * u + lane, t_hi - 1)];
#pragma unroll
        for (int u = 0; u < kRecUnroll; ++u)
            if (r + 64 * u + lane < t_hi && v[u].key != 0) take_best(v[u].key, v[u].j, bk, bj);
    }
}

struct TileRef {
    const uint8_t *base;
    uint64_t j0;
    uint32_t s;
    uint32_t fast;
};

__device__ __forceinline__ bool tile_fast(uint64_t j0, uint64_t L) {
    return L >= 8 && j0 + kTileKeys - 1 <= (L - 4) / 4;
}

__device__ __forceinline__ uint64_t tile_key_end(uint64_t j0, uint64_t L, uint64_t jneed) {
    return tile_fast(j0, L) ? j0 + kTileKeys - 1 : min(j0 + kTileKeys - 1, jneed);
}

constexpr uint64_t kTieMark = ~0ull;

__device__ __forceinline__ uint32_t key_top16(uint32_t a, uint32_t b) {
    uint32_t r;
    asm("v_xor_b32_sdwa %0, %1, %2 dst_sel:WORD_1 dst_unused:UNUSED_PAD src0_sel:WORD_1 "
        "src1_sel:WORD_0"
        : "=v"(r) : "v"(a), "v"(b));
    return r;
}
__device__ __forceinline__ uint32_t max_u32_op(uint32_t a, uint32_t b) {
    uint32_t r;
    asm("v_max_u32 %0, %1, %2" : "=v"(r) : "v"(a), "v"(b));
    return r;
}

template <int G>
__device__ __forceinline__ void tile_scan(const TileRef &tr, const TileRef &nx,
                                          u32x4 (&x)[kTileIters], uint32_t &prev_word,
                                          uint32_t lb_a, uint32_t lb_b, uint32_t &top,
                                          uint32_t &fs, uint32_t &ls,
                                          uint32_t (&gpk)[(G + 1) / 2]) {
    static_assert(G == 1 || (G % 2 == 0 && kTileIters % G == 0), "groups: 1 or an even divisor");
    static_assert(kTileIters <= 16, "slice indices: 4 bits");
    constexpr int kPer = kTileIters / G;
    const uint32_t lane = lane_id();
    const uint8_t *nbase = nx.fast ? nx.base + 4 * nx.j0 : tr.base + 4 * tr.j0;
    const __amdgpu_buffer_rsrc_t nsrc =
        G > 1 ? tile_rsrc(nbase, (nx.fast ? nx.fast : tr.fast) * 1024u) : tile_rsrc(nbase);
    uint32_t carry = pf_entry(prev_word, lb_a, lb_b);
    const uint64_t nj0 = nx.fast ? nx.j0 : tr.j0;
    const bool consec = nx.fast && nx.s == tr.s && nx.j0 == tr.j0 + kTileKeys;
    const uint32_t pw_loaded = __builtin_amdgcn_raw_buffer_load_b32(
        tile_rsrc(nj0 ? nbase - 4 : nbase, consec ? 0u : 4u), 0, 0, 0);
    uint32_t last_w = 0;
    const uint32_t key0_mask = (tr.j0 == 0 && lane == 0) ? 0u : ~0u;
    uint32_t acc_first = 0, acc_last = 0, acc_grp = 0;
#pragma unroll
    for (int it = 0; it < kTileIters; ++it) {
        uint32_t a[16], r[16];
        pf_addrs(x[it].x, lb_a, lb_b, a + 0);
        pf_addrs(x[it].y, lb_a, lb_b, a + 4);
        pf_addrs(x[it].z, lb_a, lb_b, a + 8);
        pf_addrs(x[it].w, lb_a, lb_b, a + 12);
        if (it == kTileIters - 1) last_w = (uint32_t)__builtin_amdgcn_readlane(x[it].w, 63);
        x[it] = ring_load(nsrc, lane * 16, it);
        uint32_t e0, e1, e2, e3;
        if constexpr (RC_DIAG_SLICE_FENCE) {
#pragma unroll
            for (int q = 0; q < 16; ++q) r[q] = pf_lds(a[q]);
            __builtin_amdgcn_sched_barrier(0);
            e0 = __builtin_amdgcn_bitop3_b32(r[0], r[1], r[2], 0x96) ^ r[3];
            e1 = __builtin_amdgcn_bitop3_b32(r[4], r[5], r[6], 0x96) ^ r[7];
            e2 = __builtin_amdgcn_bitop3_b32(r[8], r[9], r[10], 0x96) ^ r[11];
            e3 = __builtin_amdgcn_bitop3_b32(r[12], r[13], r[14], 0x96) ^ r[15];
        } else {
            e0 = pf_gather(a + 0);
            e1 = pf_gather(a + 4);
            e2 = pf_gather(a + 8);
            e3 = pf_gather(a + 12);
        }
        const uint32_t rot = __builtin_amdgcn_mov_dpp(e3, 0x13C, 0xf, 0xf, false);
        const uint32_t ep = lane == 0 ? carry : rot;
        carry = rot;
        uint32_t b0 = key_top16(ep, e0);
        if (it == 0) b0 &= key0_mask;
        const uint32_t b1 = key_top16(e0, e1), b2 = key_top16(e1, e2), b3 = key_top16(e2, e3);
        uint32_t sm = max_u32_op(max3_u32(b0, b1, b2), b3);
        if constexpr (G > 1) sm &= (uint32_t)it < tr.fast ? ~0u : 0u;
        acc_first = max_u32_op(acc_first, sm | (uint32_t)(kTileIters - 1 - it));
        acc_last = max_u32_op(acc_last, sm | (uint32_t)it);
        if constexpr (G > 1) {
            acc_grp = max_u32_op(acc_grp, sm);
            if ((it + 1) % kPer == 0) {
                const int g = it / kPer;
                if (g % 2 == 0) gpk[g / 2] = acc_grp >> 16;
                else gpk[g / 2] |= acc_grp & 0xffff0000u;
                acc_grp = 0;
            }
        }
    }
    top = acc_first >> 16;
    fs = (uint32_t)(kTileIters - 1) - (acc_first & 0xffffu);
    ls = acc_last & 0xffffu;
    prev_word = consec ? last_w : pw_loaded;
}

__device__ __forceinline__ uint32_t wave_max_u32(uint32_t v) {
    v = max(v, (uint32_t)__builtin_amdgcn_update_dpp(0, (int)v, 0x111, 0xf, 0xf, false));
    v = max(v, (uint32_t)__builtin_amdgcn_update_dpp(0, (int)v, 0x112, 0xf, 0xf, false));
    v = max(v, (uint32_t)__builtin_amdgcn_update_dpp(0, (int)v, 0x114, 0xf, 0xf, false));
    v = max(v, (uint32_t)__builtin_amdgcn_update_dpp(0, (int)v, 0x118, 0xf, 0xf, false));
    const uint32_t r0 = __builtin_amdgcn_readlane(v, 15), r1 = __builtin_amdgcn_readlane(v, 31);
    const uint32_t r2 = __builtin_amdgcn_readlane(v, 47), r3 = __builtin_amdgcn_readlane(v, 63);
    return max(max(r0, r1), max(r2, r3));
}

__device__ __forceinline__ uint32_t pk_max_u16(uint32_t a, uint32_t b) {
    uint32_t r;
    asm("v_pk_max_u16 %0, %1, %2" : "=v"(r) : "v"(a), "v"(b));
    return r;
}
__device__ __forceinline__ uint32_t pk_max_u16_s(uint32_t a, uint32_t b) {
    return max(a & 0xffffu, b & 0xffffu) | (max(a >> 16, b >> 16) << 16);
}

__device__ __forceinline__ uint32_t wave_max_pk16(uint32_t v) {
    v = pk_max_u16(v, (uint32_t)__builtin_amdgcn_update_dpp(0, (int)v, 0x111, 0xf, 0xf, false));
    v = pk_max_u16(v, (uint32_t)__builtin_amdgcn_update_dpp(0, (int)v, 0x112, 0xf, 0xf, false));
    v = pk_max_u16(v, (uint32_t)__builtin_amdgcn_update_dpp(0, (int)v, 0x114, 0xf, 0xf, false));
    v = pk_max_u16(v, (uint32_t)__builtin_amdgcn_update_dpp(0, (int)v, 0x118, 0xf, 0xf, false));
    const uint32_t r0 = __builtin_amdgcn_readlane(v, 15), r1 = __builtin_amdgcn_readlane(v, 31);
    const uint32_t r2 = __builtin_amdgcn_readlane(v, 47), r3 = __builtin_amdgcn_readlane(v, 63);
    return pk_max_u16_s(pk_max_u16_s(r0, r1), pk_max_u16_s(r2, r3));
}

template <bool kCache, bool kClip = false>
struct TileCursor {
    StreamDesc d;
    uint64_t s, cur, next;
    const uint8_t *base;
    uint32_t nfast;
    uint32_t nlast;
    __device__ void enter() {
        if constexpr (!kCache) return;
        base = sload_ptr(d.ptr + s);
        const uint64_t L = sload(d.len + s);
        nfast = L >= 8 && (L - 4) / 4 >= kTileKeys - 1
                    ? (uint32_t)(((L - 4) / 4 - (kTileKeys - 1)) / kTileKeys + 1) : 0u;
        if constexpr (kClip) {
            const uint64_t jl = sload(d.jneed + s) - (next - cur - 1) * kTileKeys;
            nlast = jl < (uint64_t)kTileKeys ? (uint32_t)(jl >> 8) + 1u : (uint32_t)kTileIters;
        }
    }
    __device__ void init(const StreamDesc &dd, uint64_t n_streams, uint64_t t) {
        d = dd;
        uint64_t lo = 0, hi = n_streams;
        while (hi - lo > 1) {
            const uint64_t mid = (lo + hi) >> 1;
            if (sload(d.tile_base + mid) <= t) lo = mid;
            else hi = mid;
        }
        s = lo;
        cur = sload(d.tile_base + s);
        next = sload(d.tile_base + s + 1);
        enter();
    }
    __device__ TileRef at(uint64_t t) {
        if (t >= next) {
            do {
                ++s;
                cur = next;
                next = sload(d.tile_base + s + 1);
            } while (t >= next);
            enter();
        }
        TileRef r;
        r.j0 = (t - cur) * kTileKeys;
        r.s = (uint32_t)s;
        if constexpr (kCache) {
            r.base = base;
            r.fast = t - cur < nfast ? (kClip && t + 1 == next ? nlast : (uint32_t)kTileIters) : 0u;
        } else {
            r.base = sload_ptr(d.ptr + s);
            r.fast = __builtin_amdgcn_readfirstlane((uint32_t)tile_fast(r.j0, sload(d.len + s))) != 0;
        }
        return r;
    }
};

__device__ __forceinline__ void stage_tile_tables_nb(const KeyTables *tab) {
    const uint32_t nt = blockDim.x;
    for (uint32_t e0 = 0; e0 < 1024u; e0 += 4 * nt) {
        uint32_t v[4];
        uint32_t ent[4];
#pragma unroll
        for (int k = 0; k < 4; ++k) {
            ent[k] = e0 + k * nt + threadIdx.x;
            v[k] = ent[k] < 1024u ? (&tab->pf[0][0])[ent[k]] : 0u;
        }
#pragma unroll
        for (int k = 0; k < 4; ++k) {
            if (ent[k] >= 1024u) continue;
            const uint32_t b = ent[k] >> 8, vv = ent[k] & 255;
            uint32_t *row = s_tile_lds + ((b >> 1) * 65536u + vv * 256u + (b & 1) * 128u) / 4;
            for (uint32_t c = 0; c < 32; ++c) row[(c + threadIdx.x) & 31] = v[k];
        }
    }
    uint64_t *full = reinterpret_cast<uint64_t *>(s_tile_lds + kFullOff / 4);
    const uint64_t *gfull = &tab->tl[0][0];
    for (uint32_t i = threadIdx.x; i < 2048u; i += nt) full[i] = gfull[i];
}

template <int G>
__device__ __forceinline__ GroupRecord tile_groups(const uint32_t (&gpk)[(G + 1) / 2], uint32_t hot) {
    GroupRecord r;
    r.max = 0;
    r.pad = 0;
#pragma unroll
    for (int i = 0; i < (G + 1) / 2; ++i) {
        const uint32_t v = gpk[i];
        r.max |= (uint64_t)wave_max_pk16(v) << (32 * i);
        r.hot[2 * i] = __ballot((v & 0xffffu) >= hot);
        r.hot[2 * i + 1] = __ballot((v >> 16) >= hot);
    }
    return r;
}

struct TileUnits {
    uint32_t n_tiles, nw, s0, chunk, dyn0, n_units;
    uint32_t gshift;
    uint32_t n_groups;
    __device__ __host__ void range(uint32_t u, uint32_t &b, uint32_t &e) const {
        if (u < nw) {
            b = u * s0;
            e = b + s0;
        } else {
            b = dyn0 + (u - nw) * chunk;
            e = b + chunk;
        }
        if (b > n_tiles) b = n_tiles;
        if (e > n_tiles) e = n_tiles;
    }
};

constexpr uint64_t kDynChunkMin = 2;
constexpr uint32_t kGrabMinShift = 4;
__host__ inline TileUnits tile_units(uint64_t n_tiles, uint64_t nw, TileSched sched) {
    TileUnits U;
    U.n_tiles = (uint32_t)n_tiles;
    U.nw = (uint32_t)nw;
    U.gshift = 0;
    U.n_groups = 0;
    uint64_t permille = sched.permille, chunk = sched.chunk, dyn_min = sched.dyn_min;
    if (permille > 1000) permille = 1000;
    if (chunk < kDynChunkMin) chunk = kDynChunkMin;
    if (n_tiles < dyn_min * nw || permille == 1000) {
        U.s0 = (uint32_t)((n_tiles + nw - 1) / nw);
        U.chunk = 1;
        U.dyn0 = (uint32_t)n_tiles;
        U.n_units = (uint32_t)nw;
        return U;
    }
    U.s0 = (uint32_t)(n_tiles * permille / 1000 / nw);
    const uint64_t dyn = n_tiles - nw * U.s0, fit = dyn / (4 * nw);
    if (chunk > fit) chunk = fit > kDynChunkMin ? fit : kDynChunkMin;
    U.chunk = (uint32_t)chunk;
    U.dyn0 = (uint32_t)(nw * U.s0);
    U.n_units = (uint32_t)(nw + (n_tiles - U.dyn0 + chunk - 1) / chunk);
    if (sched.group) {
        uint32_t sh = 0;
        while ((2u << sh) <= sched.group && sh < 8) ++sh;
        if (sh < kGrabMinShift) sh = kGrabMinShift;
        U.gshift = sh;
        U.n_groups = (uint32_t)(((uint64_t)(U.n_units - U.nw) + (1u << sh) - 1) >> sh);
    }
    return U;
}

constexpr uint32_t kGrabSlots = 16;
constexpr uint32_t kGrabSpinLimit = 1u << 24;
__shared__ uint32_t s_grab_ord;
__shared__ uint32_t s_grab_cfg[2];
__shared__ uint64_t s_grab_slot[kGrabSlots];

constexpr uint32_t kGrabErrWord = kCtrErrWord;

template <bool kGroup>
struct UnitGrab {
    uint32_t v;

    __device__ void start(const TileUnits &U, uint32_t *ctr) {
        v = 0;
        if (U.n_units <= U.nw) return;
        if (kGroup ? threadIdx.x == 0 : lane_id() == 0) v = atomicAdd(ctr, 1u);
    }
    __device__ void seed(const TileUnits &U) {
        if (!kGroup || U.n_units <= U.nw || threadIdx.x != 0) return;
        s_grab_ord = 0;
        s_grab_cfg[0] = U.gshift;
        s_grab_cfg[1] = U.n_groups;
        s_grab_slot[0] = (uint64_t)v;
        for (uint32_t i = 1; i < kGrabSlots; ++i) s_grab_slot[i] = ~0ull;
    }
    __device__ uint32_t next(const TileUnits &U, uint32_t *ctr, uint32_t *err) {
        if (U.n_units <= U.nw) return U.n_units;
        if constexpr (!kGroup) {
            const uint32_t u = U.nw + (uint32_t)__builtin_amdgcn_readfirstlane(v);
            if (u < U.n_units && lane_id() == 0) v = atomicAdd(ctr, 1u);
            return u;
        }
        uint32_t o = 0;
        if (lane_id() == 0)
            o = __hip_atomic_fetch_add(&s_grab_ord, 1u, __ATOMIC_RELAXED, __HIP_MEMORY_SCOPE_WORKGROUP);
        o = (uint32_t)__builtin_amdgcn_readfirstlane(o);
        const uint32_t gshift = (uint32_t)__builtin_amdgcn_readfirstlane(s_grab_cfg[0]);
        const uint32_t n_groups = (uint32_t)__builtin_amdgcn_readfirstlane(s_grab_cfg[1]);
        const uint32_t k = o >> gshift, sub = o & ((1u << gshift) - 1);
        uint32_t g = ~0u;
        for (uint32_t spins = 0;; ++spins) {
            const uint64_t e = __hip_atomic_load(&s_grab_slot[k % kGrabSlots], __ATOMIC_RELAXED,
                                                 __HIP_MEMORY_SCOPE_WORKGROUP);
            const uint32_t tag = (uint32_t)__builtin_amdgcn_readfirstlane((uint32_t)(e >> 32));
            if (tag == k) {
                g = (uint32_t)__builtin_amdgcn_readfirstlane((uint32_t)e);
                break;
            }
            if ((tag != ~0u && (int32_t)(tag - k) > 0) || spins == kGrabSpinLimit) {
                if (err && lane_id() == 0) atomicOr(err, 1u);
                break;
            }
            __builtin_amdgcn_s_sleep(2);
        }
        const bool live = g < n_groups;
        if (sub == 0) {
            uint32_t nv = ~0u;
            if (live && lane_id() == 0) nv = atomicAdd(ctr, 1u);
            nv = (uint32_t)__builtin_amdgcn_readfirstlane(nv);
            if (lane_id() == 0)
                __hip_atomic_store(&s_grab_slot[(k + 1) % kGrabSlots], ((uint64_t)(k + 1) << 32) | nv,
                                   __ATOMIC_RELAXED, __HIP_MEMORY_SCOPE_WORKGROUP);
        }
        if (RC_DIAG_FORCE_GRAB_STOP() && err) {
            if (lane_id() == 0) atomicOr(err, 1u);
            return U.n_units;
        }
        return live ? U.nw + (g << gshift) + sub : U.n_units;
    }
};

template <int G, bool kGroup>
__global__ __launch_bounds__(1024) void rc_tile_kernel(const KeyTables *__restrict__ tab,
                                                       StreamDesc d, uint64_t n_streams,
                                                       TileUnits U,
                                                       TileRecord *__restrict__ rec,
                                                       GroupRecord *__restrict__ grp,
                                                       uint32_t hot,
                                                       uint32_t *__restrict__ xlist,
                                                       uint32_t *__restrict__ xcount,
                                                       uint32_t *__restrict__ ctr) {
    UnitGrab<kGroup> grab;
    grab.start(U, ctr);
    stage_tile_tables_nb(tab);
    grab.seed(U);
    __syncthreads();
    const uint64_t *full = reinterpret_cast<const uint64_t *>(s_tile_lds + kFullOff / 4);
    const uint64_t *tl = full, *th = full + 1024;
    const uint64_t n_tiles = U.n_tiles;

    const uint32_t lane = lane_id();
    const uint32_t lb_a = (lane & 31) * 4, lb_b = lb_a | 0x10000u;
    const uint32_t wave = __builtin_amdgcn_readfirstlane(threadIdx.x >> 6);
    const uint64_t gw = (uint64_t)blockIdx.x * (blockDim.x >> 6) + wave;
    uint32_t u = (uint32_t)gw, ub, ue;
    U.range(u, ub, ue);
    uint32_t n_ties = 0;
    RC_TILE_STAMP_BEGIN();

    TileCursor<true, (G > 1)> cursor;
    TileRef cur;
    uint64_t t = ub;
    bool seek = true;
    for (;;) {
        if (t < ue) {
            if (seek) cursor.init(d, n_streams, t);
            seek = false;
            cur = cursor.at(t);
            if (cur.fast) break;
            ++t;
            continue;
        }
        if (lane == 0) xcount[u] = 0;
        u = grab.next(U, ctr, ctr + kGrabErrWord);
        if (u >= U.n_units) return;
        U.range(u, ub, ue);
        t = ub;
        seek = true;
    }
    u32x4 x[kTileIters];
    uint32_t prev_word = ld_u32(cur.base + 4 * cur.j0 - (cur.j0 ? 4 : 0));
    {
        const __amdgpu_buffer_rsrc_t src = tile_rsrc(cur.base + 4 * cur.j0);
#pragma unroll
        for (int it = 0; it < kTileIters; ++it) {
            x[it] = ring_load(src, lane * 16, it);
            __builtin_amdgcn_sched_barrier(0);
        }
    }
    uint64_t pend_t = n_tiles;
    uint64_t pend_jm = 0;
    uint64_t pend_mask = 0;
    uint32_t pend_st = 0;
    uint32_t pend_lo = 0, pend_hi = 0, pend_jl = 0;

    auto retire = [&]() {
        const uint64_t k = full_key(tl, th, pend_lo, pend_hi);
        const bool ptie = pend_st >> 31;
        const uint64_t pj0 = pend_jm & ((1ull << 48) - 1);
        const uint32_t pm = (uint32_t)(pend_jm >> 48);
        const uint64_t hold = ptie ? 0 : pend_mask;
        uint64_t bk = ptie ? pend_mask : 0, bj = kTieMark ^ (pend_st & 0x7fffffffu);
        const bool win = ((hold >> lane) & 1) && (uint32_t)(k >> 48) == pm &&
                         pj0 + pend_jl != 0;
        const uint64_t wm = __ballot(win);
        for (uint64_t m = wm; m; m &= m - 1) {
            const int l = __builtin_ctzll(m);
            const uint64_t kl = lane_u64(k, l);
            const uint64_t jl = pj0 + (uint32_t)__builtin_amdgcn_readlane(pend_jl, l);
            if (m == wm || kl > bk || (kl == bk && jl < bj)) {
                bk = kl;
                bj = jl;
            }
        }
        if (lane == 0) {
            rec[pend_t].key = bk;
            rec[pend_t].j = bj;
        }
    };

    for (;;) {
        TileRef nx = cur;
        nx.fast = false;
        uint64_t tn = t + 1;
        uint32_t nu = u, nub = ub, nue = ue;
        for (;;) {
            if (tn < nue) {
                nx = cursor.at(tn);
                if (nx.fast) break;
                ++tn;
                continue;
            }
            if (nu != u && lane == 0) xcount[nu] = 0;
            nu = grab.next(U, ctr, ctr + kGrabErrWord);
            if (nu >= U.n_units) {
                nu = u;
                break;
            }
            U.range(nu, nub, nue);
            tn = nub;
            if (tn < nue) cursor.init(d, n_streams, tn);
        }
        uint32_t top, fs, ls;
        uint32_t gpk[(G + 1) / 2];
        tile_scan<G>(cur, nx, x, prev_word, lb_a, lb_b, top, fs, ls, gpk);
        if constexpr (G > 1) {
            const GroupRecord g = tile_groups<G>(gpk, hot);
            if (lane == 0) grp[t] = g;
        }

        retire();

        const uint32_t M = wave_max_u32(top);
        const bool cand = top == M;
        const uint64_t cmask = __ballot(cand);
        const uint32_t nc = (uint32_t)__builtin_popcountll(cmask);
        const bool tie = __ballot(cand && fs != ls) != 0 || nc > 16;
        const uint32_t c0 = (uint32_t)__builtin_ctzll(cmask);
        const uint32_t f0 = (uint32_t)__builtin_amdgcn_readlane(fs, c0);
        uint32_t jl = f0 * 256 + c0 * 4 + (lane & 3);
        if (!tie) {
            uint64_t m = cmask & (cmask - 1);
            for (uint32_t q = 1; m; m &= m - 1, ++q) {
                const uint32_t c = (uint32_t)__builtin_ctzll(m);
                const uint32_t f = (uint32_t)__builtin_amdgcn_readlane(fs, c);
                if ((lane >> 2) == q) jl = f * 256 + c * 4 + (lane & 3);
            }
        }
        if (lane == 0) xlist[ub + n_ties] = (uint32_t)t;
        n_ties += tie ? 1u : 0u;
        pend_t = t;
        pend_jm = cur.j0 | ((uint64_t)M << 48);
        pend_mask = tie ? cmask : (nc >= 16 ? ~0ull : (1ull << (4 * nc)) - 1);
        pend_st = (tie ? 0x80000000u : 0u) | (uint32_t)cur.s;
        pend_jl = jl;
        const uint8_t *q = cur.base + 4 * (cur.j0 + pend_jl);
        pend_lo = ld_u32(q - (cur.j0 + pend_jl ? 4 : 0));
        pend_hi = ld_u32(q);
        RC_TILE_STAMP_TILE();
        if (nu != u) {
            if (lane == 0) xcount[u] = n_ties;
            n_ties = 0;
            u = nu;
            ub = nub;
            ue = nue;
        }
        if (!nx.fast) break;
        t = tn;
        cur = nx;
    }
    retire();
    if (lane == 0) {
        xcount[u] = n_ties;
        RC_TILE_STAMP_END(gw);
    }
}

__device__ __forceinline__ uint64_t stream_of_tile(const StreamDesc &d, uint64_t n_streams,
                                                   uint64_t t) {
    uint64_t lo = 0, hi = n_streams;
    while (hi - lo > 1) {
        const uint64_t mid = (lo + hi) >> 1;
        if (sload(d.tile_base + mid) <= t) lo = mid;
        else hi = mid;
    }
    return lo;
}

__device__ __forceinline__ void exact_tile(const uint64_t *tl, const uint64_t *th,
                                           const StreamDesc &d, uint64_t s, uint64_t t,
                                           TileRecord *rec, GroupRecord *grp) {
    const uint64_t j0 = (t - sload(d.tile_base + s)) * kTileKeys;
    const uint64_t jb = tile_key_end(j0, sload(d.len + s), sload(d.jneed + s));
    uint64_t bk = 0, bj = ~0ull;
    scan_ranges<kScanUnroll>(tl, th, sload_ptr(d.ptr + s), max(j0, (uint64_t)1), jb, 1, 0, bk, bj);
    wave_best(bk, bj);
    if (lane_id() == 0) {
        rec[t].key = bk;
        rec[t].j = bj;
        if (grp) grp[t] = GroupRecord{~0ull, {~0ull, ~0ull, ~0ull, ~0ull}, 0ull};
    }
}

constexpr int kTieLanes = 4;
__device__ __forceinline__ void exact_lanes(const uint64_t *tl, const uint64_t *th,
                                            const StreamDesc &d, uint64_t s, uint64_t t,
                                            uint64_t lanes, TileRecord *rec) {
    const uint64_t j0 = (t - sload(d.tile_base + s)) * kTileKeys;
    const uint8_t *base = sload_ptr(d.ptr + s);
    const uint32_t i = lane_id();
    const uint64_t local = (i >> 2) * 256 + (i & 3);
    uint32_t lo[kTieLanes], hi[kTieLanes];
    uint64_t jj[kTieLanes];
    uint64_t m = lanes;
#pragma unroll
    for (int q = 0; q < kTieLanes; ++q) {
        const uint32_t c = m ? (uint32_t)__builtin_ctzll(m) : 0u;
        const uint64_t j = j0 + local + 4 * c;
        const uint8_t *p = base + 4 * j;
        lo[q] = ld_u32(j ? p - 4 : p);
        hi[q] = ld_u32(p);
        jj[q] = (m && j) ? j : ~0ull;
        m &= m - 1;
    }
    uint64_t bk = 0, bj = ~0ull;
#pragma unroll
    for (int q = 0; q < kTieLanes; ++q)
        if (jj[q] != ~0ull) take_best(full_key(tl, th, lo[q], hi[q]), jj[q], bk, bj);
    wave_best(bk, bj);
    if (lane_id() == 0) {
        rec[t].key = bk;
        rec[t].j = bj;
    }
}

__global__ __launch_bounds__(256) void rc_edge_kernel(const KeyTables *__restrict__ tab,
                                                      StreamDesc d, uint64_t n_streams,
                                                      TileUnits U,
                                                      TileRecord *__restrict__ rec,
                                                      GroupRecord *__restrict__ grp,
                                                      const uint32_t *__restrict__ xlist,
                                                      const uint32_t *__restrict__ xcount,
                                                      uint32_t *__restrict__ ctr, uint64_t epoch) {
    __shared__ __attribute__((aligned(16))) uint64_t s_full[2048];
    __shared__ uint32_t s_fault;
    if (threadIdx.x == 0) {
        uint32_t *err = ctr + kCtrErrWord;
        uint64_t *stamp = reinterpret_cast<uint64_t *>(ctr + kCtrStampWord);
        uint32_t f = __hip_atomic_load(err, __ATOMIC_ACQUIRE, __HIP_MEMORY_SCOPE_AGENT);
        if (blockIdx.x == 0) {
            *ctr = 0u;
            if (f) {
                __hip_atomic_store(stamp, epoch, __ATOMIC_RELAXED, __HIP_MEMORY_SCOPE_AGENT);
                atomicAdd(ctr + kCtrFaultsWord, 1u);
                __hip_atomic_store(err, 0u, __ATOMIC_RELEASE, __HIP_MEMORY_SCOPE_AGENT);
            }
        } else if (!f) {
            f = __hip_atomic_load(stamp, __ATOMIC_RELAXED, __HIP_MEMORY_SCOPE_AGENT) == epoch;
        }
        s_fault = f;
    }
    __syncthreads();
    if (s_fault) return;
    const uint64_t gw = (uint64_t)blockIdx.x * (blockDim.x >> 6) +
                        __builtin_amdgcn_readfirstlane(threadIdx.x >> 6);
    const uint64_t nw = (uint64_t)gridDim.x * (blockDim.x >> 6);
    const uint64_t n_host = sload(d.xtiles);
    const uint64_t n_units = U.n_units;
    const uint64_t n_items = n_units + n_host;
    const uint32_t lane = lane_id();
    const uint64_t n_runs = (n_items + 63) / 64;
    auto needs = [&](uint64_t c) -> uint64_t {
        const uint64_t e = c * 64 + lane;
        const bool w = e < n_items && (e >= n_units || xcount[e] != 0);
        return __ballot(w);
    };
    bool work = false;
    for (uint64_t c = gw; c < n_runs && !work; c += nw) work = needs(c) != 0;
    if (!__syncthreads_or(work)) return;
    const uint64_t *gfull = &tab->tl[0][0];
    for (uint32_t i = threadIdx.x; i < 2048u; i += blockDim.x) s_full[i] = gfull[i];
    __syncthreads();
    const uint64_t *tl = s_full, *th = s_full + 1024;
    for (uint64_t c = gw; c < n_runs; c += nw) {
        for (uint64_t m = needs(c); m; m &= m - 1) {
            const uint64_t e = c * 64 + (uint64_t)__builtin_ctzll(m);
            if (e < n_units) {
                uint32_t t0, t1;
                U.range((uint32_t)e, t0, t1);
                const uint32_t c = (uint32_t)__builtin_amdgcn_readfirstlane(xcount[e]);
                for (uint32_t i = 0; i < c; ++i) {
                    const uint64_t t = (uint32_t)__builtin_amdgcn_readfirstlane(xlist[t0 + i]);
                    const uint64_t lanes = sload(&rec[t].key), s = ~sload(&rec[t].j) & 0x7fffffffu;
                    if (__builtin_popcountll(lanes) <= kTieLanes)
                        exact_lanes(tl, th, d, s, t, lanes, rec);
                    else
                        exact_tile(tl, th, d, s, t, rec, grp);
                }
            } else {
                const uint64_t t = sload(d.xtiles + 1 + (e - n_units));
                exact_tile(tl, th, d, stream_of_tile(d, n_streams, t), t, rec, grp);
            }
        }
    }
}


__device__ __forceinline__ bool call_faulted(const ChainParams &prm) {
    return prm.fault != nullptr && sload(prm.fault) == prm.epoch;
}
__device__ __forceinline__ void fault_counts(int64_t *counts, uint64_t n_streams) {
    for (uint64_t s = (uint64_t)blockIdx.x * blockDim.x + threadIdx.x; s < n_streams;
         s += (uint64_t)gridDim.x * blockDim.x)
        counts[s] = kCountFault;
}

struct ChainStream {
    const uint8_t *base;
    uint64_t L, P, tb0, nt, jmax;
    RC_DIAG_ONLY(bool diag;)
};

__device__ __forceinline__ ChainStream chain_stream(const StreamDesc &d, uint64_t s) {
    ChainStream st;
    st.base = sload_ptr(d.ptr + s);
    st.L = sload(d.len + s);
    st.P = sload(d.last + s);
    st.tb0 = sload(d.tile_base + s);
    st.nt = sload(d.tile_base + s + 1) - st.tb0;
    st.jmax = st.L >= 8 ? (st.L - 4) / 4 : 0;
    RC_DIAG_ONLY(st.diag = s == 0;)
    return st;
}

#ifndef RC_EDGE_ITERS
#define RC_EDGE_ITERS 2
#endif
constexpr int kEdgeIters = RC_EDGE_ITERS;

struct EdgeRange {
    const uint8_t *p;
    uint64_t a, q0;
    uint32_t nk, wlast;
    uint32_t lo, span;
    uint32_t it0;
    uint32_t carry;
    uint32_t carry_word;
    uint32_t R;
    bool live;

    __device__ void init(const uint8_t *base, uint64_t wmax, uint64_t a_, uint64_t b_, uint32_t R_) {
        R = R_;
        live = a_ <= b_;
        a = a_;
        q0 = a_ & ~3ull;
        nk = live ? (uint32_t)(b_ - q0) : 0;
        lo = (uint32_t)(a_ - q0);
        span = nk - lo;
        p = base + 4 * q0;
        wlast = live ? (uint32_t)(wmax - q0) : 0;
        it0 = 0;
        carry_word = 0;
        carry = 0;
    }
    __device__ bool more() const { return live && it0 * 256 <= nk; }
    __device__ void load(uint32_t (&w)[kEdgeIters][4]) {
        const uint32_t lane = lane_id();
        if (it0 == 0) carry_word = ld_u32(q0 ? p - 4 : p);
#pragma unroll
        for (int i = 0; i < kEdgeIters; ++i) {
            const uint32_t o = min((it0 + i) * 256 + lane * 4, wlast & ~3u);
            const u32x4 v = *as_global_x4(p + 4 * o);
            w[i][0] = v.x;
            w[i][1] = v.y;
            w[i][2] = v.z;
            w[i][3] = v.w;
        }
    }
    template <bool kCompact>
    __device__ void compute(const uint32_t (&w)[kEdgeIters][4], uint32_t lb_a, uint32_t lb_b,
                            const uint32_t *pf, uint32_t &acc_first, uint32_t &acc_last) {
        const uint32_t lane = lane_id();
        if (it0 == 0) carry = kCompact ? pfc_entry(pf, carry_word) : pf_entry(carry_word, lb_a, lb_b);
#pragma unroll
        for (int i = 0; i < kEdgeIters; ++i) {
            const uint32_t it = it0 + i;
            uint32_t e0, e1, e2, e3;
            if constexpr (kCompact) {
                e0 = pfc_entry(pf, w[i][0]);
                e1 = pfc_entry(pf, w[i][1]);
                e2 = pfc_entry(pf, w[i][2]);
                e3 = pfc_entry(pf, w[i][3]);
            } else {
                uint32_t ad[16];
                pf_addrs(w[i][0], lb_a, lb_b, ad + 0);
                pf_addrs(w[i][1], lb_a, lb_b, ad + 4);
                pf_addrs(w[i][2], lb_a, lb_b, ad + 8);
                pf_addrs(w[i][3], lb_a, lb_b, ad + 12);
                e0 = pf_gather(ad + 0);
                e1 = pf_gather(ad + 4);
                e2 = pf_gather(ad + 8);
                e3 = pf_gather(ad + 12);
            }
            const uint32_t rot = __builtin_amdgcn_mov_dpp(e3, 0x13C, 0xf, 0xf, false);
            const uint32_t ep = lane == 0 ? carry : rot;
            carry = rot;
            const uint32_t t[4] = {(ep & 0xffff0000u) ^ (e0 << 16), (e0 & 0xffff0000u) ^ (e1 << 16),
                                   (e1 & 0xffff0000u) ^ (e2 << 16), (e2 & 0xffff0000u) ^ (e3 << 16)};
            const uint32_t it_lo = it * 256u, it_hi = it * 256u + 255u;
            if (it_lo >= lo && it_hi <= nk) {
                const uint32_t lf = 511u - 256u * R - it * 4u, ll = 256u * R + it * 4u;
                acc_first = max3_u32(acc_first, t[0] | 0x8000u | lf, t[1] | 0x8000u | (lf - 1u));
                acc_first = max3_u32(acc_first, t[2] | 0x8000u | (lf - 2u), t[3] | 0x8000u | (lf - 3u));
                acc_last = max3_u32(acc_last, t[0] | 0x8000u | ll, t[1] | 0x8000u | (ll + 1u));
                acc_last = max3_u32(acc_last, t[2] | 0x8000u | (ll + 2u), t[3] | 0x8000u | (ll + 3u));
                continue;
            }
#pragma unroll
            for (int k = 0; k < 4; ++k) {
                const uint32_t off = it * 256 + lane * 4 + k;
                const bool valid = off - lo <= span;
                const uint32_t local = 256u * R + it * 4 + k;
                acc_first = max3_u32(acc_first, valid ? (t[k] | 0x8000u | (511u - local)) : 0u, 0u);
                acc_last = max3_u32(acc_last, valid ? (t[k] | 0x8000u | local) : 0u, 0u);
            }
        }
        it0 += kEdgeIters;
    }
};

enum : int { kStepStop = 0, kStepCut = 1, kStepTail1 = 2, kStepTail2 = 3 };

template <typename I>
__device__ __forceinline__ I argmax_offset(uint64_t bk, I bj, I s4, I minl) {
    I idx = bk > 0 ? 4 * (bj - s4) : 0;
    if (idx < minl) idx = (minl + 3) & ~(I)3;
    return idx;
}

__device__ __forceinline__ int step_cuts(bool argmax, uint64_t idx, bool far, bool open,
                                         uint64_t pos, uint64_t rem, uint64_t minl, uint64_t maxl,
                                         uint64_t L, uint64_t &c1, uint64_t &c2) {
    if (open && !argmax) return kStepStop;
    if (argmax) {
        if (idx != 0) {
            c1 = pos + idx;
            return kStepCut;
        }
        if (far || open) return kStepStop;
    }
    uint64_t c;
    if (rem <= maxl) c = rem;
    else if (rem < maxl + minl) c = rem / 2;
    else c = maxl;
    if (c == 0) return kStepStop;
    c1 = pos + c;
    if (c < rem) {
        c2 = L;
        return kStepTail2;
    }
    return kStepTail1;
}

template <typename I>
__device__ __forceinline__ void trim_groups(uint64_t gm, I te, uint32_t tb16, I &a, I &b) {
    const I tj0 = te * kTileKeys;
    uint32_t ga = (uint32_t)((a - tj0) / kGroupKeys), gb = (uint32_t)((b - tj0) / kGroupKeys);
    while (ga <= gb && ((gm >> (16 * ga)) & 0xffffu) < tb16) ++ga;
    while (gb > ga && ((gm >> (16 * gb)) & 0xffffu) < tb16) --gb;
    if (ga > gb) {
        a = 1;
        b = 0;
        return;
    }
    a = max(a, tj0 + (I)ga * kGroupKeys);
    b = min(b, tj0 + (I)(gb + 1) * kGroupKeys - 1);
}

template <int R>
struct RecCache {
    uint32_t c0 = 0, n = 0;
    TileRecord v[R];
    uint64_t g[R];

    __device__ bool has(uint64_t t) const { return t >= c0 && t - c0 < n; }
    __device__ void load(const TileRecord *rec, const GroupRecord *grp, const ChainStream &st,
                         uint64_t lo) {
        c0 = (uint32_t)lo;
        n = (uint32_t)min(st.nt - lo, (uint64_t)64 * R);
        const uint64_t lane = lane_id();
#pragma unroll
        for (int u = 0; u < R; ++u)
            if ((uint64_t)64 * u < n) {
                const uint64_t t = st.tb0 + lo + min((uint64_t)64 * u + lane, n - 1);
                v[u] = rec[t];
                if (grp) g[u] = grp[t].max;
            }
    }
    __device__ TileRecord get(uint64_t t, uint64_t &gm) const {
        const uint64_t off = t - c0;
        const int row = (int)(off >> 6), l = (int)(off & 63);
        TileRecord r = {0, 0};
        gm = ~0ull;
#pragma unroll
        for (int u = 0; u < R; ++u)
            if (u == row) {
                r.key = lane_u64(v[u].key, l);
                r.j = lane_u64(v[u].j, l);
                gm = lane_u64(g[u], l);
            }
        return r;
    }
    __device__ void reduce(uint64_t t_lo, uint64_t t_hi, uint64_t &bk, uint64_t &bj) const {
        const uint64_t lane = lane_id();
#pragma unroll
        for (int u = 0; u < R; ++u) {
            const uint64_t t = c0 + 64 * u + lane;
            if ((uint64_t)64 * u < n && t - c0 < n && t >= t_lo && t < t_hi && v[u].key != 0)
                take_best(v[u].key, v[u].j, bk, bj);
        }
    }
};


template <bool kTail, typename I>
__device__ __forceinline__ bool edge_settled(uint64_t rk, I rj, I a, I b, uint64_t &bk, I &bj) {
    const bool inr = rk != 0 && rj >= a && rj <= b;
    if (inr) take_best(rk, rj, bk, bj);
    return rk == 0 || inr || (kTail ? rk <= bk : rk < bk);
}

template <typename I>
__device__ __forceinline__ void scan_edges(const uint64_t *tl, const uint64_t *th,
                                           const uint32_t *pf, const ChainStream &st, I a0, I b0,
                                           I a1, I b1, uint32_t lb_a, uint32_t lb_b, uint64_t &bk,
                                           I &bj) {
    if (a0 > b0 && a1 > b1) return;
    EdgeRange r0, r1;
    r0.init(st.base, st.L / 4 - 1, a0, b0, 0);
    r1.init(st.base, st.L / 4 - 1, a1, b1, 1);
    uint32_t w0[kEdgeIters][4], w1[kEdgeIters][4];
    uint32_t acc_first = 0, acc_last = 0;
    if (r0.more()) r0.load(w0);
    if (r1.more()) r1.load(w1);
    for (;;) {
        const bool m0 = r0.more(), m1 = r1.more();
        if (!m0 && !m1) break;
        if (m0) {
            r0.template compute<true>(w0, lb_a, lb_b, pf, acc_first, acc_last);
            if (r0.more()) r0.load(w0);
        }
        if (m1) {
            r1.template compute<true>(w1, lb_a, lb_b, pf, acc_first, acc_last);
            if (r1.more()) r1.load(w1);
        }
    }
    const uint32_t m = wave_max_u32(acc_first);
    if (!((m & 0x8000u) && (m >> 16) >= (uint32_t)(bk >> 48))) return;
    const bool cand = (acc_first >> 16) == (m >> 16) && (acc_first & 0x8000u);
    const uint32_t fl = 511u - (acc_first & 0x1ffu), ll = acc_last & 0x1ffu;
    if (__any(cand && fl != ll)) {
        uint64_t ek = 0, ej = ~0ull;
        scan_ranges<kChainScanUnroll>(tl, th, st.base, a0, b0, a1, b1, ek, ej);
        uint64_t bj64 = bj == (I)~(I)0 ? ~0ull : bj;
        take_best(ek, ej, bk, bj64);
        wave_best(bk, bj64);
        bj = (I)bj64;
    } else {
        const uint32_t lo = fl & 255u;
        const I jc = ((fl < 256 ? a0 : a1) & ~(I)3) + 256u * (lo >> 2) + 4u * lane_id() + (lo & 3);
        const I jl = cand ? jc : a0 <= b0 ? a0 : a1;
        const uint64_t k = full_key(tl, th, ld_u32(st.base + 4ull * jl - 4),
                                    ld_u32(st.base + 4ull * jl));
        for (uint64_t cm = __ballot(cand); cm; cm &= cm - 1) {
            const int l = __builtin_ctzll(cm);
            take_best(lane_u64(k, l), (I)lane_u64(jl, l), bk, bj);
        }
    }
}

template <int R>
__device__ int chain_step(const uint64_t *tl, const uint64_t *th, const uint32_t *pf,
                          const TileRecord *rec, const ChainStream &st, const ChainParams &prm,
                          RecCache<R> &cache, uint64_t pos, uint32_t lb_a, uint32_t lb_b,
                          uint64_t &c1, uint64_t &c2) {
    const uint64_t minl = prm.min_length, maxl = prm.max_length, T = prm.window;
    const bool single = prm.max_steps == 0;
    const uint64_t rem = st.L - pos;
    const bool far = rem >= 2 * maxl;
    const bool argmax = single || (st.P >= pos && st.P - pos >= maxl) || far;
    if (argmax) {
        const uint64_t s4 = pos >> 2;
        const uint64_t ja = s4 + 1, jb = min(s4 + T, st.jmax);
        uint64_t bk = 0, bj = ~0ull;
        RC_STAMP(1);
        if (T > 0 && ja <= jb) {
            const uint64_t t_lo = (ja + kTileKeys - 1) / kTileKeys;
            const uint64_t t_hi = (jb + 1) / kTileKeys;
            uint64_t a0 = ja, b0 = jb, a1 = 1, b1 = 0;
            const bool have_rec = t_lo < t_hi;
            if (have_rec) {
                b0 = t_lo * kTileKeys - 1;
                a1 = t_hi * kTileKeys;
                b1 = jb;
            }
            bool live0 = a0 <= b0, live1 = a1 <= b1;
            const bool one0 = live0 && a0 / kTileKeys == b0 / kTileKeys;
            const bool one1 = live1 && a1 / kTileKeys == b1 / kTileKeys;
            const uint64_t te0 = a0 / kTileKeys, te1 = a1 / kTileKeys;
            uint64_t need_lo = ~0ull, need_hi = 0;
            if (have_rec) {
                need_lo = t_lo;
                need_hi = t_hi - 1;
            }
            if (one0) {
                need_lo = min(need_lo, te0);
                need_hi = max(need_hi, te0);
            }
            if (one1) {
                need_lo = min(need_lo, te1);
                need_hi = max(need_hi, te1);
            }
            if (need_lo <= need_hi && !(cache.has(need_lo) && cache.has(need_hi)))
                cache.load(rec, prm.grp, st, need_lo);
            TileRecord er0 = {}, er1 = {};
            uint64_t gm0 = ~0ull, gm1 = ~0ull;
            const bool g0 = one0 && !cache.has(te0), g1 = one1 && !cache.has(te1);
            if (g0) {
                er0 = rec[st.tb0 + te0];
                if (prm.grp) gm0 = prm.grp[st.tb0 + te0].max;
            }
            if (g1) {
                er1 = rec[st.tb0 + te1];
                if (prm.grp) gm1 = prm.grp[st.tb0 + te1].max;
            }
            if (have_rec) {
                cache.reduce(t_lo, t_hi, bk, bj);
                if (t_hi > cache.c0 + cache.n)
                    scan_records(rec, st.tb0 + max(cache.c0 + cache.n, t_lo), st.tb0 + t_hi, bk, bj);
            }
            if (one0 && !g0) er0 = cache.get(te0, gm0);
            if (one1 && !g1) er1 = cache.get(te1, gm1);
            wave_best(bk, bj);
            if (one0 && edge_settled<false>(er0.key, er0.j, a0, b0, bk, bj)) live0 = false;
            if (one1 && edge_settled<true>(er1.key, er1.j, a1, b1, bk, bj)) live1 = false;
            if (prm.grp) {
                const uint32_t tb16 = (uint32_t)(bk >> 48);
                if (one0 && live0) trim_groups(gm0, te0, tb16, a0, b0);
                if (one1 && live1) trim_groups(gm1, te1, tb16, a1, b1);
            }
            if (!live0) a0 = 1, b0 = 0;
            if (!live1) a1 = 1, b1 = 0;
            RC_STAMP(2);
            scan_edges<uint64_t>(tl, th, pf, st, a0, b0, a1, b1, lb_a, lb_b, bk, bj);
            RC_STAMP(3);
        }
        RC_STAMP(4);
        const uint64_t idx = argmax_offset<uint64_t>(bk, bj, s4, minl);
        if (single) {
            c1 = idx;
            return kStepCut;
        }
        return step_cuts(true, idx, far, prm.open, pos, rem, minl, maxl, st.L, c1, c2);
    }
    return step_cuts(false, 0, far, prm.open, pos, rem, minl, maxl, st.L, c1, c2);
}


__device__ __forceinline__ bool ge64(uint64_t a, uint32_t b) {
    return (uint32_t)(a >> 32) != 0u || (uint32_t)a >= b;
}

__device__ __forceinline__ void take_best32(uint64_t k, uint32_t j, uint64_t &bk, uint32_t &bj) {
    take_best(k, j, bk, bj);
}

__device__ int chain_step_small(const uint64_t *tl, const uint64_t *th, const uint32_t *pf,
                                const TileRecord *rec, const ChainStream &st,
                                const ChainParams &prm, RecCache<1> &cache, uint64_t pos,
                                uint32_t lb_a, uint32_t lb_b, uint64_t &c1, uint64_t &c2) {
    const uint32_t minl = (uint32_t)prm.min_length, maxl = (uint32_t)prm.max_length;
    const uint32_t T = (uint32_t)prm.window;
    const bool single = prm.max_steps == 0;
    const uint64_t rem = st.L - pos;
    const bool far = ge64(rem, 2 * maxl);
    const bool argmax = single || (st.P >= pos && ge64(st.P - pos, maxl)) || far;
    if (argmax) {
        const uint32_t s4 = (uint32_t)(pos >> 2), jmax = (uint32_t)st.jmax;
        const uint32_t ja = s4 + 1, jb = min(s4 + T, jmax);
        uint64_t bk = 0;
        uint32_t bj = ~0u;
        if (T > 0 && ja <= jb) {
            const uint32_t t_lo = (ja + kTileKeys - 1) / kTileKeys, t_hi = (jb + 1) / kTileKeys;
            const bool have_rec = t_lo < t_hi;
            uint32_t a0 = ja, b0 = jb, a1 = 1, b1 = 0;
            if (have_rec) {
                b0 = t_lo * kTileKeys - 1;
                a1 = t_hi * kTileKeys;
                b1 = jb;
            }
            const bool one0 = a0 <= b0 && a0 / kTileKeys == b0 / kTileKeys;
            const bool one1 = a1 <= b1 && a1 / kTileKeys == b1 / kTileKeys;
            const uint32_t te0 = a0 / kTileKeys, te1 = a1 / kTileKeys;
            uint32_t need_lo = have_rec ? t_lo : ~0u, need_hi = have_rec ? t_hi - 1 : 0u;
            if (one0) {
                need_lo = min(need_lo, te0);
                need_hi = max(need_hi, te0);
            }
            if (one1) {
                need_lo = min(need_lo, te1);
                need_hi = max(need_hi, te1);
            }
            if (need_lo <= need_hi && !(cache.has(need_lo) && cache.has(need_hi)))
                cache.load(rec, prm.grp, st, need_lo);
            const uint32_t lane = lane_id();
            const uint64_t key = cache.v[0].key;
            if (have_rec) {
                const uint32_t t = cache.c0 + lane;
                const bool inr = lane < cache.n && t >= t_lo && t < t_hi && key != 0;
                const uint32_t hi = inr ? (uint32_t)(key >> 32) : 0u;
                const uint32_t mhi = wave_max_u32(hi);
                const bool top = inr && hi == mhi;
                uint64_t m = __ballot(top);
                if (m & (m - 1)) {
                    const uint32_t lo = top ? (uint32_t)key : 0u;
                    const uint32_t mlo = wave_max_u32(lo);
                    m = __ballot(top && lo == mlo);
                }
                if (m) {
                    const int w = __builtin_ctzll(m);
                    bk = lane_u64(key, w);
                    bj = (uint32_t)__builtin_amdgcn_readlane((uint32_t)cache.v[0].j, w);
                }
            }
            uint64_t ek0 = 0, ek1 = 0, gm0 = ~0ull, gm1 = ~0ull;
            uint32_t ej0 = 0, ej1 = 0;
            if (one0) {
                const int l = (int)(te0 - cache.c0);
                ek0 = lane_u64(key, l);
                ej0 = (uint32_t)__builtin_amdgcn_readlane((uint32_t)cache.v[0].j, l);
                if (prm.grp) gm0 = lane_u64(cache.g[0], l);
            }
            if (one1) {
                const int l = (int)(te1 - cache.c0);
                ek1 = lane_u64(key, l);
                ej1 = (uint32_t)__builtin_amdgcn_readlane((uint32_t)cache.v[0].j, l);
                if (prm.grp) gm1 = lane_u64(cache.g[0], l);
            }
            bool live0 = a0 <= b0, live1 = a1 <= b1;
            if (one0 && edge_settled<false>(ek0, ej0, a0, b0, bk, bj)) live0 = false;
            if (one1 && edge_settled<true>(ek1, ej1, a1, b1, bk, bj)) live1 = false;
            if (prm.grp) {
                const uint32_t tb16 = (uint32_t)(bk >> 48);
                if (one0 && live0) trim_groups(gm0, te0, tb16, a0, b0);
                if (one1 && live1) trim_groups(gm1, te1, tb16, a1, b1);
            }
            if (!live0) a0 = 1, b0 = 0;
            if (!live1) a1 = 1, b1 = 0;
            scan_edges<uint32_t>(tl, th, pf, st, a0, b0, a1, b1, lb_a, lb_b, bk, bj);
        }
        const uint32_t idx = argmax_offset<uint32_t>(bk, bj, s4, minl);
        if (single) {
            c1 = idx;
            return kStepCut;
        }
        return step_cuts(true, idx, far, prm.open, pos, rem, minl, maxl, st.L, c1, c2);
    }
    return step_cuts(false, 0, far, prm.open, pos, rem, minl, maxl, st.L, c1, c2);
}

__device__ __forceinline__ uint64_t find_index(const uint64_t *base_arr, uint64_t n, uint64_t v) {
    uint64_t lo = 0, hi = n;
    while (hi - lo > 1) {
        const uint64_t mid = (lo + hi) >> 1;
        if (sload(base_arr + mid) <= v) lo = mid;
        else hi = mid;
    }
    return lo;
}

template <int R, bool kLean>
__global__ __launch_bounds__(kChainWaves * 64) void rc_spec_kernel(const KeyTables *__restrict__ tab,
                                                      StreamDesc d, uint64_t n_streams,
                                                      ChainParams prm, uint64_t n_segs,
                                                      const TileRecord *__restrict__ rec,
                                                      uint64_t *__restrict__ cuts,
                                                      int64_t *__restrict__ counts,
                                                      uint64_t *__restrict__ scratch,
                                                      uint64_t *__restrict__ seg_counts,
                                                      uint64_t *__restrict__ seg_rcount) {
    if (call_faulted(prm)) {
        fault_counts(counts, n_streams);
        return;
    }
    stage_chain_tables(tab);
    const uint32_t *pf = s_chain_lds;
    const uint64_t *full = reinterpret_cast<const uint64_t *>(s_chain_lds + 1024);
    const uint64_t *tl = full, *th = full + 1024;
    const uint32_t lane = lane_id();
    const uint32_t lb_a = (lane & 31) * 4, lb_b = lb_a | 0x10000u;
    const uint64_t q = (uint64_t)blockIdx.x * (blockDim.x >> 6) +
                       __builtin_amdgcn_readfirstlane(threadIdx.x >> 6);
    if (q >= n_segs) return;
    const uint64_t s = find_index(d.seg_base, n_streams + 1, q);
    const uint64_t sb = sload(d.seg_base + s), nseg = sload(d.seg_base + s + 1) - sb;
    const uint64_t i = q - sb;
    ChainStream st = chain_stream(d, s);
    RC_DIAG_ONLY(st.diag = st.diag && i == (nseg > 8 ? 7 : 0);)
    const bool direct = nseg == 1;
    uint64_t *out = direct ? cuts + sload(d.cut_base + s) : scratch + sload(d.scratch_base + s) + i * prm.seg_cap;
    const uint64_t cap = direct ? sload(d.cut_cap + s) : prm.seg_cap;
    const uint64_t seg_end = (i + 1) * prm.seg_bytes;
    const uint64_t steps = prm.max_steps == 0 ? 1 : prm.max_steps;

    uint64_t pos = i * prm.seg_bytes, n = 0, ext = 0;
    bool overflow = false, term = false;
    RecCache<R> cache;
    auto emit = [&](uint64_t c) {
        if (n >= cap) {
            overflow = true;
            return;
        }
        if (lane == 0) out[n] = c;
        ++n;
    };
    for (;;) {
        if (pos >= st.L || n >= steps) {
            term = true;
            break;
        }
        if (!direct && pos >= seg_end && ext++ >= prm.ext_steps) break;
        uint64_t c1 = 0, c2 = 0;
        int kind;
        if constexpr (kLean) {
            static_assert(R == 1, "the lean step works on the one-row cache");
            kind = chain_step_small(tl, th, pf, rec, st, prm, cache, pos, lb_a, lb_b, c1, c2);
        } else {
            kind = chain_step<R>(tl, th, pf, rec, st, prm, cache, pos, lb_a, lb_b, c1, c2);
        }
        if (kind == kStepStop) {
            term = true;
            break;
        }
        emit(c1);
        if (kind == kStepTail2) emit(c2);
        if (kind != kStepCut) {
            term = true;
            break;
        }
        if (overflow) break;
        pos = c1;
    }
    if (lane == 0) {
        if (direct) {
            counts[s] = overflow ? -1 : (int64_t)n;
        } else {
            const uint64_t v = overflow ? ~0ull : (n | (term ? (1ull << 63) : 0));
            seg_counts[q] = v;
            seg_rcount[q] = v;
        }
    }
}

constexpr int kLaneFull = 8;
constexpr int kLaneIters = kTileIters / kTileGroups;

constexpr uint32_t kLaneHotMax = 4;

__device__ __forceinline__ void lane_groups(bool live, const GroupRecord &g, uint32_t te,
                                            uint32_t a, uint32_t b, uint32_t t16, uint32_t hot,
                                            uint64_t (&mk)[kTileGroups], uint32_t &sc) {
    sc = 0;
#pragma unroll
    for (int q = 0; q < kTileGroups; ++q) mk[q] = 0;
    if (!live) return;
    const uint32_t tj0 = te * kTileKeys;
    const uint32_t qa = (a - tj0) / kGroupKeys, qb = (b - tj0) / kGroupKeys;
#pragma unroll
    for (int q = 0; q < kTileGroups; ++q) {
        if ((uint32_t)q < qa || (uint32_t)q > qb) continue;
        if (((uint32_t)(g.max >> (16 * q)) & 0xffffu) < t16) continue;
        const uint32_t nh = (uint32_t)__popcll(g.hot[q]);
        if (t16 < hot || nh > kLaneHotMax || nh == 0) sc |= 1u << q;
        else mk[q] = g.hot[q];
    }
}

__device__ __forceinline__ uint32_t top16_of(uint32_t e_lo_word, uint32_t e_hi_word) {
    return ((e_lo_word & 0xffff0000u) ^ (e_hi_word << 16)) >> 16;
}

template <int U>
__device__ __forceinline__ void scan_range(const uint64_t *tl, const uint64_t *th,
                                           const uint8_t *base, uint64_t a, uint64_t b,
                                           uint64_t &bk, uint64_t &bj) {
    const uint64_t lane = lane_id();
    for (uint64_t r = a; r <= b; r += 64 * U) {
        uint2 w[U];
#pragma unroll
        for (int u = 0; u < U; ++u) {
            const uint64_t j = min(r + 64 * u + lane, b);
            w[u].x = ld_u32(base + 4 * j - 4);
            w[u].y = ld_u32(base + 4 * j);
        }
#pragma unroll
        for (int u = 0; u < U; ++u) {
            const uint64_t j = r + 64 * u + lane;
            if (j <= b) take_best(full_key(tl, th, w[u].x, w[u].y), j, bk, bj);
        }
    }
}

template <int kCtrl>
__device__ __forceinline__ uint32_t qperm32(uint32_t v) {
    return (uint32_t)__builtin_amdgcn_mov_dpp((int)v, kCtrl, 0xf, 0xf, true);
}
template <int kCtrl>
__device__ __forceinline__ uint64_t qperm64(uint64_t v) {
    return (uint64_t)qperm32<kCtrl>((uint32_t)(v >> 32)) << 32 | qperm32<kCtrl>((uint32_t)v);
}
__device__ __forceinline__ void quad_best32(uint64_t &k, uint32_t &j) {
    {
        const uint64_t ko = qperm64<0xB1>(k);
        const uint32_t jo = qperm32<0xB1>(j);
        if (ko > k || (ko == k && jo < j)) k = ko, j = jo;
    }
    {
        const uint64_t ko = qperm64<0x4E>(k);
        const uint32_t jo = qperm32<0x4E>(j);
        if (ko > k || (ko == k && jo < j)) k = ko, j = jo;
    }
}

struct QuadIter {
    u32x4 v;
    uint32_t p;
};

__device__ __forceinline__ QuadIter qi_load(const uint8_t *base, uint32_t j4, uint32_t a,
                                            uint32_t b) {
    QuadIter x = {u32x4{0u, 0u, 0u, 0u}, 0u};
    if (j4 <= b && j4 + 3 >= a) {
        x.v = *as_global_x4(base + 4ull * j4);
        x.p = ld_u32(base + 4ull * j4 - (j4 ? 4 : 0));
    }
    return x;
}

__device__ __forceinline__ void qi_eval(const uint32_t *pf, const uint64_t *tl, const uint64_t *th,
                                        const uint8_t *base, const QuadIter &x, uint32_t j4,
                                        uint32_t a, uint32_t b, uint32_t t16, uint64_t &lk,
                                        uint32_t &lj) {
    if (!(j4 <= b && j4 + 3 >= a)) return;
    const uint32_t wd[5] = {x.p, x.v.x, x.v.y, x.v.z, x.v.w};
    uint32_t e[5];
#pragma unroll
    for (int k = 0; k < 5; ++k) e[k] = pfc_entry(pf, wd[k]);
    bool have = false, tie = false;
    uint32_t ct = 0, cj = 0, clo = 0, chi = 0;
#pragma unroll
    for (int k = 0; k < 4; ++k) {
        const uint32_t j = j4 + k, t = top16_of(e[k], e[k + 1]);
        const bool in = j >= a && j <= b && t >= t16;
        const bool take = in && (!have || t > ct);
        tie = take ? false : (tie || (in && t == ct));
        ct = take ? t : ct;
        cj = take ? j : cj;
        clo = take ? wd[k] : clo;
        chi = take ? wd[k + 1] : chi;
        have = have || in;
    }
    if (have) take_best32(full_key(tl, th, clo, chi), cj, lk, lj);
    if (tie) {
#pragma unroll 1
        for (uint32_t k = 0; k < 4; ++k) {
            const uint32_t j = j4 + k;
            if (j >= a && j <= b)
                take_best32(full_key(tl, th, ld_u32(base + 4ull * j - 4), ld_u32(base + 4ull * j)), j, lk, lj);
        }
    }
}

constexpr int kQuadTasks = 4;

template <int F>
__global__ __launch_bounds__(256) void rc_quad_chain_kernel(const KeyTables *__restrict__ tab,
                                                            StreamDesc d, uint64_t n_streams,
                                                            ChainParams prm,
                                                            const TileRecord *__restrict__ rec,
                                                            uint64_t *__restrict__ cuts,
                                                            int64_t *__restrict__ counts) {
    static_assert(F % 4 == 0 && kLaneIters == 4, "a quad lane per record row and per iteration");
    if (call_faulted(prm)) {
        fault_counts(counts, n_streams);
        return;
    }
    stage_chain_tables(tab);
    const uint32_t *pf = s_chain_lds;
    const uint64_t *full = reinterpret_cast<const uint64_t *>(s_chain_lds + 1024);
    const uint64_t *tl = full, *th = full + 1024;
    const uint32_t lane = lane_id(), q = lane & 3u;
    const uint64_t gid = ((uint64_t)blockIdx.x * blockDim.x + threadIdx.x) >> 2;
    if (gid - (lane >> 2) >= n_streams) return;
    const bool mine = gid < n_streams;
    const uint64_t s = mine ? gid : n_streams - 1;
    const GroupRecord *grp = prm.grp;
    const uint8_t *base = d.ptr[s];
    const uint64_t L = d.len[s], P = d.last[s];
    const uint64_t tb0 = d.tile_base[s], nt = d.tile_base[s + 1] - tb0;
    uint64_t *out = cuts + d.cut_base[s];
    const uint64_t cap = d.cut_cap[s];
    const uint32_t jmax = L >= 8 ? (uint32_t)((L - 4) / 4) : 0u;
    const uint32_t minl = (uint32_t)prm.min_length, maxl = (uint32_t)prm.max_length;
    const uint32_t T = (uint32_t)prm.window;
    auto gtile = [&](bool use, uint32_t t) -> uint64_t { return use && t < nt ? tb0 + t : prm.n_tiles; };

    uint64_t pos = 0, n = 0;
    bool walking = mine && L > 0 && prm.max_steps > 0, overflow = false;
    RC_DIAG_ONLY(const bool diag = gid < 16 && q == 0;)
    for (;;) {
        if (!__any(walking)) break;
        RC_LSTAMP(1);
        const uint64_t rem = L - pos;
        const bool far = rem >= 2ull * maxl;
        const bool argmax = (P >= pos && P - pos >= maxl) || far;
        const uint32_t s4 = (uint32_t)(pos >> 2);
        const uint32_t ja = s4 + 1, jb = min(s4 + T, jmax);
        const bool win = walking && argmax && T > 0 && ja <= jb;
        const uint32_t t_lo = (ja + kTileKeys - 1) / kTileKeys, t_hi = (jb + 1) / kTileKeys;
        const uint32_t nf = win && t_hi > t_lo ? t_hi - t_lo : 0u;
        const uint32_t a0 = ja, b0 = min(jb, t_lo * kTileKeys - 1), te0 = ja / kTileKeys;
        const uint32_t a1 = t_hi * kTileKeys, b1 = jb, te1 = t_hi;
        bool live0 = win && ja < t_lo * kTileKeys;
        bool live1 = win && t_hi >= t_lo && jb >= a1;

        TileRecord fr[F / 4];
#pragma unroll
        for (int i = 0; i < F / 4; ++i) {
            const uint32_t t = 4 * i + q;
            fr[i] = rec[gtile(t < nf, t_lo + t)];
        }
        const TileRecord r0 = rec[gtile(live0, te0)], r1 = rec[gtile(live1, te1)];
        const GroupRecord g0 = grp[gtile(live0, te0)], g1 = grp[gtile(live1, te1)];
        const bool spec = live0;
        const uint32_t lc = (s4 & 255u) >> 2, qc = (s4 & (kTileKeys - 1)) / kGroupKeys;
        const uint32_t jqc = (s4 & ~(uint32_t)(kGroupKeys - 1)) + 4 * lc;
        QuadIter x[kQuadTasks];
        x[0] = qi_load(base, jqc + 256 * q, spec ? a0 : 1u, spec ? b0 : 0u);

        uint64_t bk = 0;
        uint32_t bj = ~0u;
#pragma unroll
        for (int i = 0; i < F / 4; ++i)
            if (4 * (uint32_t)i + q < nf && fr[i].key != 0) take_best32(fr[i].key, (uint32_t)fr[i].j, bk, bj);
        quad_best32(bk, bj);
        if (live0 && edge_settled<false>(r0.key, (uint32_t)r0.j, a0, b0, bk, bj)) live0 = false;
        if (live1 && edge_settled<true>(r1.key, (uint32_t)r1.j, a1, b1, bk, bj)) live1 = false;
        uint32_t sc0, sc1;
        RC_LSTAMP(2);
        uint64_t h[kTileGroups], t[kTileGroups];
        lane_groups(live0, g0, te0, a0, b0, (uint32_t)(bk >> 48), prm.hot, h, sc0);
        lane_groups(live1, g1, te1, a1, b1, (uint32_t)(bk >> 48), prm.hot, t, sc1);
        static_assert(kTileGroups == 4, "the task queue below spells out four groups");
        auto any_task = [&]() { return (h[0] | h[1] | h[2] | h[3] | t[0] | t[1] | t[2] | t[3]) != 0; };
        auto task = [&](uint32_t &jq, uint32_t &a, uint32_t &b) {
            int r = -1;
            uint32_t g = 0, l = 0;
#define RC_POP(M, R, Q)                            \
    if (r < 0 && M) {                              \
        l = (uint32_t)__builtin_ctzll(M);          \
        M &= M - 1;                                \
        r = R;                                     \
        g = Q;                                     \
    }
            RC_POP(h[0], 0, 0) RC_POP(h[1], 0, 1) RC_POP(h[2], 0, 2) RC_POP(h[3], 0, 3)
            RC_POP(t[0], 1, 0) RC_POP(t[1], 1, 1) RC_POP(t[2], 1, 2) RC_POP(t[3], 1, 3)
#undef RC_POP
            a = 1, b = 0;
            if (r < 0) return;
            jq = (r ? te1 : te0) * kTileKeys + g * kGroupKeys + 4 * l;
            a = r ? a1 : a0;
            b = r ? b1 : b0;
        };
        bool first = false;
#define RC_FIRST(Q)                                              \
    if (spec && qc == Q && (h[Q] >> lc & 1u)) {                  \
        h[Q] &= ~(1ull << lc);                                   \
        first = true;                                            \
    }
        RC_FIRST(0) RC_FIRST(1) RC_FIRST(2) RC_FIRST(3)
#undef RC_FIRST
        uint32_t jq[kQuadTasks], ra[kQuadTasks], rb[kQuadTasks];
        jq[0] = jqc, ra[0] = first ? a0 : 1u, rb[0] = first ? b0 : 0u;
        for (;;) {
            if (!__any(first || any_task())) break;
            bool used[kQuadTasks];
#pragma unroll
            for (int k = 0; k < kQuadTasks; ++k) {
                if (!(k == 0 && first)) {
                    task(jq[k], ra[k], rb[k]);
                    x[k] = qi_load(base, jq[k] + 256 * q, ra[k], rb[k]);
                }
                used[k] = __any(ra[k] <= rb[k]);
            }
            const uint32_t t16 = (uint32_t)(bk >> 48);
            uint64_t lk = 0;
            uint32_t lj = ~0u;
#pragma unroll
            for (int k = 0; k < kQuadTasks; ++k)
                if (used[k]) qi_eval(pf, tl, th, base, x[k], jq[k] + 256 * q, ra[k], rb[k], t16, lk, lj);
            quad_best32(lk, lj);
            if (lk != 0) take_best32(lk, lj, bk, bj);
            first = false;
            RC_LSTAMP(3);
        }
        RC_LSTAMP(4);

#pragma unroll 1
        for (int r = 0; r < 2; ++r) {
            const uint32_t sv = r == 0 ? +sc0 : +sc1;
            const uint32_t te = r == 0 ? +te0 : +te1, ra_ = r == 0 ? +a0 : +a1, rb_ = r == 0 ? +b0 : +b1;
            uint32_t sa = 1, sb = 0;
            if (sv) {
                const uint32_t qlo = (uint32_t)__builtin_ctz(sv), qhi = 31u - (uint32_t)__builtin_clz(sv);
                sa = max(ra_, te * kTileKeys + qlo * kGroupKeys);
                sb = min(rb_, te * kTileKeys + (qhi + 1) * kGroupKeys - 1);
            }
            for (uint64_t m = __ballot(q == 0 && sa <= sb); m; m &= m - 1) {
                const int l = __builtin_ctzll(m);
                const uint32_t la = (uint32_t)__builtin_amdgcn_readlane(sa, l);
                const uint32_t lb = (uint32_t)__builtin_amdgcn_readlane(sb, l);
                const uint8_t *lbase = reinterpret_cast<const uint8_t *>(lane_u64((uint64_t)base, l));
                uint64_t ek = 0, ej = ~0ull;
                scan_range<kGroupKeys / 64>(tl, th, lbase, la, lb, ek, ej);
                wave_best(ek, ej);
                if ((lane >> 2) == ((uint32_t)l >> 2) && ek != 0) take_best32(ek, (uint32_t)ej, bk, bj);
                RC_LSTAMP(5);
            }
        }
        RC_LSTAMP(6);

        if (walking) {
            uint64_t c1 = 0, c2 = 0;
            const uint32_t idx = argmax_offset<uint32_t>(bk, bj, s4, minl);
            const int kind = step_cuts(argmax, idx, far, prm.open, pos, rem, minl, maxl, L, c1, c2);
            if (kind != kStepStop) {
                if (n < cap) {
                    if (q == 0) out[n] = c1;
                    ++n;
                } else {
                    overflow = true;
                }
                if (kind == kStepTail2) {
                    if (n < cap) {
// ... 233 lines not shown
    if (s < n_streams && sload(d.seg_base + s + 1) - sload(d.seg_base + s) > 1)
        counts[s] = kNeedJoin;
}

template <int R>
__global__ __launch_bounds__(256) void rc_join_kernel(const KeyTables *__restrict__ tab,
                                                      StreamDesc d, uint64_t n_streams,
                                                      ChainParams prm,
                                                      const TileRecord *__restrict__ rec,
                                                      uint64_t *__restrict__ cuts,
                                                      int64_t *__restrict__ counts,
                                                      const uint64_t *__restrict__ scratch,
                                                      const uint64_t *__restrict__ seg_counts) {
    const uint64_t s = (uint64_t)blockIdx.x * (blockDim.x >> 6) +
                       __builtin_amdgcn_readfirstlane(threadIdx.x >> 6);
    const bool need = s < n_streams && counts[s] == kNeedJoin;
    if (!__syncthreads_or(need)) return;
    stage_chain_tables(tab);
    if (!need) return;
    const uint32_t *pf = s_chain_lds;
    const uint64_t *full = reinterpret_cast<const uint64_t *>(s_chain_lds + 1024);
    const uint64_t *tl = full, *th = full + 1024;
    const uint32_t lane = lane_id();
    const uint32_t lb_a = (lane & 31) * 4, lb_b = lb_a | 0x10000u;
    const uint64_t sb = sload(d.seg_base + s), nseg = sload(d.seg_base + s + 1) - sb;
    const ChainStream st = chain_stream(d, s);
    uint64_t *out = cuts + sload(d.cut_base + s);
    const uint64_t cap = sload(d.cut_cap + s);
    const uint64_t *lists = scratch + sload(d.scratch_base + s);
    const uint64_t S = prm.seg_bytes;

    auto list_of = [&](uint64_t k) { return lists + k * prm.seg_cap; };
    auto count_of = [&](uint64_t k, bool &term, bool &bad) {
        const uint64_t c = seg_counts[sb + k];
        bad = c == ~0ull;
        term = (c >> 63) != 0;
        return c & ~(1ull << 63);
    };

    uint64_t pos = 0, n = 0, src = 0, idx = 0;
    bool overflow = false, src_term, bad;
    RecCache<R> cache;
    uint64_t src_cnt = count_of(0, src_term, bad);
    overflow |= bad;
    while (!overflow) {
        const uint64_t g_next = src + 1 < nseg ? (src + 1) * S : ~0ull;
        const uint64_t *lst = list_of(src);
        for (;;) {
            const uint64_t k = idx + lane;
            const uint64_t v = k < src_cnt ? lst[k] : ~0ull;
            const uint64_t take = __ballot(v < g_next);
            const uint32_t m = __popcll(take);
            if (m == 0) break;
            if (n + m > cap) {
                overflow = true;
                break;
            }
            if (v < g_next) out[n + lane] = v;
            n += m;
            idx += m;
            pos = lane_u64(v, m - 1);
            if (m < 64) break;
        }
        if (overflow) break;
        if (idx >= src_cnt && src_term) break;
        bool hopped = false;
        const uint64_t kmax = min(pos / S, nseg - 1);
        for (uint64_t k = src + 1; k <= kmax && !hopped; ++k) {
            bool kt, kb;
            const uint64_t kc = count_of(k, kt, kb);
            if (kb) {
                overflow = true;
                break;
            }
            if (pos == k * S) {
                hopped = true;
                src = k;
                idx = 0;
                src_cnt = kc;
                src_term = kt;
                break;
            }
            const uint64_t *kl = list_of(k);
            for (uint64_t w = 0; w < kc; w += 64) {
                const uint64_t v = w + lane < kc ? kl[w + lane] : ~0ull;
                const uint64_t hit = __ballot(v == pos);
                if (hit) {
                    hopped = true;
                    src = k;
                    idx = w + __builtin_ctzll(hit) + 1;
                    src_cnt = kc;
                    src_term = kt;
                    break;
                }
                if (lane_u64(v, 63) > pos || w + 64 >= kc) break;
            }
        }
        if (overflow) break;
        if (hopped) continue;
        if (idx < src_cnt) {
            const uint64_t v = lst[idx++];
            if (n >= cap) {
                overflow = true;
                break;
            }
            if (lane == 0) out[n] = v;
            ++n;
            pos = v;
            if (idx >= src_cnt && src_term) break;
            continue;
        }
        if (pos >= st.L) break;
        uint64_t c1 = 0, c2 = 0;
        const int kind = chain_step<R>(tl, th, pf, rec, st, prm, cache, pos, lb_a, lb_b, c1, c2);
        if (kind == kStepStop) break;
        if (n + (kind == kStepTail2 ? 2 : 1) > cap) {
            overflow = true;
            break;
        }
        if (lane == 0) {
            out[n] = c1;
            if (kind == kStepTail2) out[n + 1] = c2;
        }
        n += kind == kStepTail2 ? 2 : 1;
        if (kind != kStepCut) break;
        pos = c1;
        src_cnt = idx;
    }
    if (lane == 0) counts[s] = overflow ? -1 : (int64_t)n;
}

__device__ __forceinline__ uint64_t probe_tile(uint64_t k, uint64_t gw, uint64_t nw,
                                               uint64_t block) {
    return (k / block * nw + gw) * block + k % block;
}

template <bool kGroup>
__global__ __launch_bounds__(1024) void rc_read_probe_kernel(const uint8_t *__restrict__ src,
                                                             uint64_t n_tiles,
                                                             uint32_t *__restrict__ out,
                                                             uint64_t block, TileUnits U,
                                                             uint32_t *__restrict__ ctr) {
    const uint32_t lane = lane_id();
    const uint32_t wave = __builtin_amdgcn_readfirstlane(threadIdx.x >> 6);
    const uint64_t gw = (uint64_t)blockIdx.x * (blockDim.x >> 6) + wave;
    const uint64_t nw = (uint64_t)gridDim.x * (blockDim.x >> 6);
    uint32_t acc = 0;
    if (block == 0) {
        UnitGrab<kGroup> grab;
        grab.start(U, ctr);
        grab.seed(U);
        __syncthreads();
        uint32_t u = (uint32_t)gw, ub, ue;
        U.range(u, ub, ue);
        auto next_unit = [&]() -> bool {
            for (;;) {
                u = grab.next(U, ctr, nullptr);
                if (u >= U.n_units) return false;
                U.range(u, ub, ue);
                if (ub < ue) return true;
            }
        };
        if (ub >= ue && !next_unit()) return;
        uint64_t t = ub;
        u32x4 x[kTileIters];
        gu32x4 *p = as_global_x4(src + t * (uint64_t)kTileKeys * 4) + lane;
#pragma unroll
        for (int it = 0; it < kTileIters; ++it) {
            x[it] = RC_STREAM_LOAD(p + it * 64);
            __builtin_amdgcn_sched_barrier(0);
        }
        for (;;) {
            uint64_t tn = t + 1;
            bool more = true;
            if (tn >= ue) {
                more = next_unit();
                tn = more ? ub : t;
            }
            gu32x4 *q = as_global_x4(src + tn * (uint64_t)kTileKeys * 4) + lane;
#pragma unroll
            for (int it = 0; it < kTileIters; ++it) {
                const u32x4 w = x[it];
                acc = max3_u32(acc, w.x ^ w.y, w.z ^ w.w);
                x[it] = RC_STREAM_LOAD(q + it * 64);
            }
            if (!more) break;
            t = tn;
        }
        if (acc == 0x9E3779B9u) out[0] = acc;
        return;
    }
    uint64_t t = 0, t_end = 0;
    while (probe_tile(t_end, gw, nw, block) < n_tiles) ++t_end;
    if (t >= t_end) return;
    u32x4 x[kTileIters];
    gu32x4 *p = as_global_x4(src + probe_tile(t, gw, nw, block) * (uint64_t)kTileKeys * 4) + lane;
#pragma unroll
    for (int it = 0; it < kTileIters; ++it) {
        x[it] = RC_STREAM_LOAD(p + it * 64);
        __builtin_amdgcn_sched_barrier(0);
    }
    for (; t < t_end; ++t) {
        const uint64_t tn = t + 1 < t_end ? t + 1 : t;
        gu32x4 *q = as_global_x4(src + probe_tile(tn, gw, nw, block) * (uint64_t)kTileKeys * 4) + lane;
#pragma unroll
        for (int it = 0; it < kTileIters; ++it) {
            const u32x4 w = x[it];
            acc = max3_u32(acc, w.x ^ w.y, w.z ^ w.w);
            x[it] = RC_STREAM_LOAD(q + it * 64);
        }
    }
    if (acc == 0x9E3779B9u) out[0] = acc;
}


__global__ void rc_fill_kernel(uint8_t *__restrict__ dst, uint64_t nbytes, uint64_t base,
                               uint64_t word0) {
    const uint64_t nwords = nbytes / 8;
    const uint64_t stride = (uint64_t)gridDim.x * blockDim.x;
    uint64_t *w = reinterpret_cast<uint64_t *>(dst);
    for (uint64_t i = (uint64_t)blockIdx.x * blockDim.x + threadIdx.x; i < nwords; i += stride)
        w[i] = splitmix64(base ^ (word0 + i));
    if (blockIdx.x == 0 && threadIdx.x < (nbytes & 7)) {
        const uint64_t v = splitmix64(base ^ (word0 + nwords));
        dst[nwords * 8 + threadIdx.x] = (uint8_t)(v >> (8 * threadIdx.x));
    }
}

__global__ void rc_fill_streams_kernel(uint8_t *__restrict__ dst, uint64_t n, uint64_t nbytes,
                                       uint64_t slot, uint64_t seed, uint64_t id0,
                                       uint64_t id_step) {
    const uint64_t wps = (nbytes + 7) / 8, total = n * wps;
    const uint64_t stride = (uint64_t)gridDim.x * blockDim.x;
    for (uint64_t i = (uint64_t)blockIdx.x * blockDim.x + threadIdx.x; i < total; i += stride) {
        const uint64_t k = i / wps, w = i - k * wps;
        const uint64_t base = (seed * 0x9E3779B97F4A7C15ull) ^ ((id0 + k * id_step) << 34);
        reinterpret_cast<uint64_t *>(dst + k * slot)[w] = splitmix64(base ^ w);
    }
}

int cu_count() {
    int dev = 0, cus = 0;
    if (hipGetDevice(&dev) != hipSuccess) return 256;
    if (hipDeviceGetAttribute(&cus, hipDeviceAttributeMultiprocessorCount, dev) != hipSuccess ||
        cus <= 0)
        return 256;
    return cus;
}

}

extern "C" {

int rc_launch_tiles(const KeyTables *d_tables, StreamDesc desc, uint64_t n_streams,
                    uint64_t n_tiles, TileRecord *d_records, GroupRecord *d_grp,
                    uint32_t hot, uint32_t *d_xlist, uint32_t *d_ctr, uint64_t epoch,
                    void *stream, void *mid_event, uint32_t tile_cus, void *edge_stream,
                    void *tiled, TileSched sched) {
    hipStream_t st = (hipStream_t)stream;
    hipStream_t est = edge_stream ? (hipStream_t)edge_stream : st;
    auto hand_over = [&]() -> int {
        if (est == st) return 0;
        if ((tiled != mid_event && hipEventRecord((hipEvent_t)tiled, st) != hipSuccess) ||
            hipStreamWaitEvent(est, (hipEvent_t)tiled, 0) != hipSuccess)
            return rc_fail(RC_ERR_HIP, "edge stream hand-over failed");
        return 0;
    };
    if (n_tiles == 0) {
        if (mid_event && hipEventRecord((hipEvent_t)mid_event, st) != hipSuccess)
            return rc_fail(RC_ERR_HIP, "hipEventRecord failed");
        return hand_over();
    }
    const uint64_t waves_per_wg = 1024 / kWaveSize;
    uint64_t grid = (n_tiles + waves_per_wg - 1) / waves_per_wg;
    const uint64_t cus = tile_cus ? (uint64_t)tile_cus : (uint64_t)cu_count();
    if (grid > cus) grid = cus;
    const uint64_t n_waves = grid * waves_per_wg;
    const TileUnits U = tile_units(n_tiles, n_waves, sched);
    uint32_t *d_xcount = d_xlist + n_tiles;
    const bool grp = U.n_groups != 0;
    if (d_grp && grp)
        hipLaunchKernelGGL((rc_tile_kernel<kTileGroups, true>), dim3((unsigned)grid), dim3(1024), 0,
                           st, d_tables, desc, n_streams, U, d_records, d_grp, hot, d_xlist,
                           d_xcount, d_ctr);
    else if (d_grp)
        hipLaunchKernelGGL((rc_tile_kernel<kTileGroups, false>), dim3((unsigned)grid), dim3(1024),
                           0, st, d_tables, desc, n_streams, U, d_records, d_grp, hot, d_xlist,
                           d_xcount, d_ctr);
    else if (grp)
        hipLaunchKernelGGL((rc_tile_kernel<1, true>), dim3((unsigned)grid), dim3(1024), 0, st,
                           d_tables, desc, n_streams, U, d_records, d_grp, hot, d_xlist, d_xcount,
                           d_ctr);
    else
        hipLaunchKernelGGL((rc_tile_kernel<1, false>), dim3((unsigned)grid), dim3(1024), 0, st,
                           d_tables, desc, n_streams, U, d_records, d_grp, hot, d_xlist, d_xcount,
                           d_ctr);
    if (int rc = launch_status("rc_tile_kernel")) return rc;
    if (mid_event && hipEventRecord((hipEvent_t)mid_event, st) != hipSuccess)
        return rc_fail(RC_ERR_HIP, "hipEventRecord failed");
    if (int rc = hand_over()) return rc;
    uint64_t egrid = (U.n_units + 3) / 4;
    if (egrid > 4 * cus) egrid = 4 * cus;
    if (egrid == 0) egrid = 1;
    hipLaunchKernelGGL(rc_edge_kernel, dim3((unsigned)egrid), dim3(256), 0, est, d_tables, desc,
                       n_streams, U, d_records, d_grp, (const uint32_t *)d_xlist,
                       (const uint32_t *)d_xcount, d_ctr, epoch);
    return launch_status("rc_edge_kernel");
}

int rc_tile_schedule(uint64_t n_tiles, uint32_t waves, uint32_t permille, uint32_t chunk,
                     uint32_t dyn_min, uint32_t *ranges, uint64_t cap, uint64_t *n_units) {
    if (!n_units || waves == 0 || n_tiles >= (1ull << 32)) return 1;
    TileSched sched;
    sched.permille = permille;
    sched.chunk = chunk;
    sched.dyn_min = dyn_min;
    const TileUnits U = tile_units(n_tiles, waves, sched);
    *n_units = U.n_units;
    for (uint32_t u = 0; u < U.n_units && u < cap && ranges; ++u) U.range(u, ranges[2 * u], ranges[2 * u + 1]);
    return 0;
}

uint64_t rc_tie_list_words(uint64_t n_tiles) {
    return 2 * n_tiles + n_tiles / kDynChunkMin + 64;
}

int rc_launch_chain(const KeyTables *d_tables, StreamDesc desc, uint64_t n_streams,
                    ChainParams prm, uint64_t n_segs, const TileRecord *d_records,
                    uint64_t *d_cuts, int64_t *d_counts, uint64_t *d_scratch,
                    uint64_t *d_seg_counts, bool any_multi, uint32_t join, void *stream) {
    if (n_streams == 0) return 0;
    hipStream_t st = (hipStream_t)stream;
    if (prm.lane && prm.lean && prm.grp && !any_multi && n_segs == n_streams &&
        prm.max_steps != 0 && prm.window / kTileKeys <= (uint64_t)kLaneFull) {
        const bool narrow = prm.window / kTileKeys <= 4;
        const uint64_t grid = (n_streams + 63) / 64;
        if (narrow)
            hipLaunchKernelGGL(rc_quad_chain_kernel<4>, dim3((unsigned)grid), dim3(256), 0, st,
                               d_tables, desc, n_streams, prm, d_records, d_cuts, d_counts);
        else
            hipLaunchKernelGGL(rc_quad_chain_kernel<kLaneFull>, dim3((unsigned)grid), dim3(256), 0,
                               st, d_tables, desc, n_streams, prm, d_records, d_cuts, d_counts);
        return launch_status("rc_quad_chain_kernel");
    }
    const bool small = prm.window / kTileKeys + 3 <= 64;
    const uint64_t grid = (n_segs + kChainWaves - 1) / kChainWaves;
    uint64_t *seg_merge = d_seg_counts + n_segs, *seg_off = seg_merge + n_segs;
    uint64_t *seg_slice = seg_off + n_segs, *seg_rcount = seg_slice + n_segs;
    if (small && prm.lean)
        hipLaunchKernelGGL((rc_spec_kernel<1, true>), dim3((unsigned)grid),
                           dim3(kChainWaves * kWaveSize), 0, st, d_tables, desc, n_streams, prm,
                           n_segs, d_records, d_cuts, d_counts, d_scratch, d_seg_counts, seg_rcount);
    else if (small)
        hipLaunchKernelGGL((rc_spec_kernel<1, false>), dim3((unsigned)grid),
                           dim3(kChainWaves * kWaveSize), 0, st, d_tables, desc, n_streams, prm,
                           n_segs, d_records, d_cuts, d_counts, d_scratch, d_seg_counts, seg_rcount);
    else
        hipLaunchKernelGGL((rc_spec_kernel<kRecUnroll, false>), dim3((unsigned)grid),
                           dim3(kChainWaves * kWaveSize), 0, st, d_tables, desc, n_streams, prm,
                           n_segs, d_records, d_cuts, d_counts, d_scratch, d_seg_counts, seg_rcount);
    if (int rc = launch_status("rc_spec_kernel")) return rc;
    if (!any_multi) return 0;
    const uint64_t sgrid = (n_segs + 3) / 4, jgrid = (n_streams + kChainWaves - 1) / kChainWaves;
    if (!(join & RC_JOIN_WALK_ONLY)) {
        const bool repair = (join & RC_JOIN_REPAIR) != 0;
        if (small)
            hipLaunchKernelGGL(rc_merge_kernel<1>, dim3((unsigned)sgrid), dim3(256), 0, st,
                               d_tables, desc, n_streams, prm, n_segs, d_records, d_scratch,
                               (const uint64_t *)d_seg_counts, seg_merge, seg_rcount, repair);
        else
            hipLaunchKernelGGL(rc_merge_kernel<kRecUnroll>, dim3((unsigned)sgrid), dim3(256), 0,
                               st, d_tables, desc, n_streams, prm, n_segs, d_records, d_scratch,
                               (const uint64_t *)d_seg_counts, seg_merge, seg_rcount, repair);
        if (int rc = launch_status("rc_merge_kernel")) return rc;
        hipLaunchKernelGGL(rc_scan_kernel, dim3((unsigned)jgrid), dim3(kChainWaves * kWaveSize), 0,
                           st, desc, n_streams, prm, (const uint64_t *)d_seg_counts,
                           (const uint64_t *)seg_merge, (const uint64_t *)seg_rcount, seg_off,
                           seg_slice, d_counts);
        if (int rc = launch_status("rc_scan_kernel")) return rc;
        hipLaunchKernelGGL(rc_copy_kernel, dim3((unsigned)sgrid), dim3(256), 0, st, desc,
                           n_streams, prm, n_segs, (const uint64_t *)d_scratch,
                           (const uint64_t *)seg_off, (const uint64_t *)seg_slice, d_cuts,
                           (const int64_t *)d_counts);
        if (int rc = launch_status("rc_copy_kernel")) return rc;
    } else {
        hipLaunchKernelGGL(rc_mark_kernel, dim3((unsigned)jgrid), dim3(kChainWaves * kWaveSize), 0,
                           st, desc, n_streams, prm, d_counts);
        if (int rc = launch_status("rc_mark_kernel")) return rc;
    }
    if (small)
        hipLaunchKernelGGL(rc_join_kernel<1>, dim3((unsigned)jgrid), dim3(kChainWaves * kWaveSize),
                           0, st, d_tables, desc, n_streams, prm, d_records, d_cuts, d_counts,
                           (const uint64_t *)d_scratch, (const uint64_t *)d_seg_counts);
    else
        hipLaunchKernelGGL(rc_join_kernel<kRecUnroll>, dim3((unsigned)jgrid),
                           dim3(kChainWaves * kWaveSize), 0, st, d_tables, desc, n_streams, prm,
                           d_records, d_cuts, d_counts, (const uint64_t *)d_scratch,
                           (const uint64_t *)d_seg_counts);
    return launch_status("rc_join_kernel");
}

int rc_launch_read_probe(const uint8_t *d_src, uint64_t nbytes, uint32_t *d_out, uint32_t block,
                         TileSched sched, void *stream) {
    const uint64_t n_tiles = nbytes / ((uint64_t)kTileKeys * 4);
    if (n_tiles == 0) return 0;
    uint64_t grid = (n_tiles + 15) / 16;
    const uint64_t cus = (uint64_t)cu_count();
    if (grid > cus) grid = cus;
    const TileUnits U = tile_units(n_tiles, grid * (1024 / kWaveSize), sched);
    if (block == 0 && U.n_units > U.nw &&
        hipMemsetAsync(d_out + 1, 0, sizeof(uint32_t), (hipStream_t)stream) != hipSuccess)
        return rc_fail(RC_ERR_HIP, "hipMemsetAsync failed");
    if (U.n_groups)
        hipLaunchKernelGGL(rc_read_probe_kernel<true>, dim3((unsigned)grid), dim3(1024), 0,
                           (hipStream_t)stream, d_src, n_tiles, d_out, (uint64_t)block, U, d_out + 1);
    else
        hipLaunchKernelGGL(rc_read_probe_kernel<false>, dim3((unsigned)grid), dim3(1024), 0,
                           (hipStream_t)stream, d_src, n_tiles, d_out, (uint64_t)block, U, d_out + 1);
    return launch_status("rc_read_probe_kernel");
}

int rc_launch_fill_streams(uint8_t *d_dst, uint64_t n, uint64_t nbytes, uint64_t slot,
                           uint64_t seed, uint64_t id0, uint64_t id_step, void *stream) {
    if (n == 0 || nbytes == 0) return 0;
    const uint64_t words = n * ((nbytes + 7) / 8);
    uint64_t grid = (words + 255) / 256;
    if (grid > 65536) grid = 65536;
    hipLaunchKernelGGL(rc_fill_streams_kernel, dim3((unsigned)grid), dim3(256), 0,
                       (hipStream_t)stream, d_dst, n, nbytes, slot, seed, id0, id_step);
    return launch_status("rc_fill_streams_kernel");
}

int rc_launch_fill(uint8_t *d_dst, uint64_t nbytes, uint64_t seed, uint64_t stream_id,
                   uint64_t word0, void *stream) {
    if (nbytes == 0) return 0;
    const uint64_t base = (seed * 0x9E3779B97F4A7C15ull) ^ (stream_id << 34);
    uint64_t grid = (nbytes / 8 + 255) / 256;
    if (grid > 8192) grid = 8192;
    if (grid == 0) grid = 1;
    hipLaunchKernelGGL(rc_fill_kernel, dim3((unsigned)grid), dim3(256), 0, (hipStream_t)stream,
                       d_dst, nbytes, base, word0);
    return launch_status("rc_fill_kernel");
}

}
```

replicat_amd/csrc/knobs.h:

```cpp
#pragma once
#include <stdint.h>

#include <cerrno>
#include <cstdio>
#include <cstdlib>
#include <cstring>

namespace rc {

enum Knob : int {
    knPipeAll,
    knOverlapCus,
    knLaneChain,
    knTileGroups,
    knChainLean,
    knSegmentBytes,
    knSegmentExt,
    knSegmentFloor,
    knTileStatic,
    knTileChunk,
    knTileDynMin,
    knJoinWalk,
    knRepair,
    knB2LaneMax,
    knB2LaneOnly,
    knShaLaneMax,
    knProbeBlock,
    knGcmDebug,
    knTileStreams,
    knTileGroup,
    knTileMask,
    knHostBatchBytes,
    kKnobCount
};

struct KnobSpec {
    const char *name;
    int64_t def, lo, hi;
    const char *words;
    const char *doc;
};

inline constexpr KnobSpec kKnobTable[kKnobCount] = {
    {"RC_PIPE_ALL", 0, 0, 1, "0|1",
     "1: every RC_PIPELINED request overlaps (otherwise small-window chunkers and requests "
     "under a tile per tile-kernel wave run in sequence, capi.cpp rc_chunk_device)"},
    {"RC_OVERLAP_CUS", 32, 1, 1024, nullptr,
     "CUs reserved for the chain kernels of pipelined calls (rc_chunker_overlap overrides; "
     "must be below the device's CU count)"},
    {"RC_LANE_CHAIN", 0, 0, 2, "auto|0|1",
     "chain kernel of small-window batches: auto (quads for >= 256 streams), 0 wave per "
     "stream, 1 quads whatever the count"},
    {"RC_TILE_GROUPS", 0, 0, 2, "auto|0|1",
     "per-quarter group records of the tile kernel: auto (small windows), 0 never, 1 always"},
    {"RC_CHAIN_LEAN", 0, 0, 1, "auto|0",
     "32-bit chain steps for small windows: auto, 0 never (comparison)"},
    {"RC_SEGMENT_BYTES", 0, 0, int64_t(1) << 50, nullptr,
     "chain segment length in bytes (0: sized per call for ~4096 walkers)"},
    {"RC_SEGMENT_EXT", 2, 0, 64, nullptr,
     "steps a speculative chain runs past its segment end"},
    {"RC_SEGMENT_FLOOR", 2, 1, 64, nullptr,
     "shortest automatic segment, in max_lengths"},
    {"RC_TILE_STATIC", 0, 0, 1000, nullptr,
     "share of the tiles handed out statically, per mille (1000: fully static)"},
    {"RC_TILE_CHUNK", 3, 2, 4096, nullptr,
     "tiles per dynamic unit of the tile kernel"},
    {"RC_TILE_DYN_MIN", 0, 0, int64_t(1) << 20, nullptr,
     "tiles per wave from which a launch hands out dynamic units"},
    {"RC_JOIN_WALK", 0, 0, 1, "0|1",
     "1: every multi-segment stream through the sequential join (comparison)"},
    {"RC_REPAIR", 1, 0, 1, "0|1",
     "0: no boundary repair in the merge kernel (a miss walks the stream)"},
    {"RC_B2_LANE_MAX", -1, -1, int64_t(1) << 62, nullptr,
     "BLAKE2b: longest message hashed by one lane (-1: the throughput rule, 0: quads only)"},
    {"RC_B2_LANE_ONLY", 0, 0, 2, "auto|0|1",
     "BLAKE2b: 0 never uses the lane-only kernel (the fused kernel's lane role instead); "
     "auto and 1 use it when every message fits a lane"},
    {"RC_SHA_LANE_MAX", -1, -1, int64_t(1) << 62, nullptr,
     "SHA-2 / SHA-3: longest message hashed by one lane, longer ones by the latency form (SHA-2: "
     "a wave per message, SHA-3: 25-lane groups); -1: the rule, 0: the latency form only"},
    {"RC_PROBE_BLOCK", 0, 0, int64_t(1) << 20, nullptr,
     "read probe: interleaved static runs of this many tiles (0: the tile kernel's schedule)"},
    {"RC_GCM_DEBUG", 0, 0, 1, "0|1",
     "1: stamp every host step of an AES-GCM call on stderr"},
    {"RC_TILE_STREAMS", 1, 1, 2, nullptr,
     "CU-masked tile streams of pipelined calls: 2 alternates them, so a call's tile kernel "
     "may start on CUs the previous one has left"},
    {"RC_TILE_GROUP", 64, 0, 256, nullptr,
     "dynamic units per workgroup grab of the tile kernel (a power of two: the workgroup's "
     "waves take that many units from one global grab through LDS; below 16 runs as 16, the "
     "LDS ring's margin); 0: one grab per unit"},
    {"RC_TILE_MASK", 0, 0, 2, "masked|full|plain",
     "tile stream of pipelined calls: masked (the CUs the chain stream does not reserve), full "
     "(its own queue with every CU in its mask) or plain (a non-blocking stream on the shared "
     "queues); with full / plain the tile kernel's workgroups take every CU the chain kernels "
     "leave (measurement switch)"},
    {"RC_HOST_BATCH_BYTES", int64_t(1) << 30, 16, int64_t(1) << 40, nullptr,
     "rc_chunk_host / rc_chunk_digest_host: bytes of whole streams per double-buffered batch "
     "(a stream longer than this is a batch of its own); test switch: a small value sends a "
     "few MiB through many batches, so the suite can check slot reuse and output offsets"},
};

struct Knobs {
    int64_t v[kKnobCount];
    int64_t operator[](Knob k) const { return v[k]; }
};

inline bool parse_knob(const KnobSpec &s, const char *text, int64_t &out) {
    if (s.words) {
        int64_t idx = 0;
        for (const char *w = s.words; *w; ++idx) {
            const char *bar = std::strchr(w, '|');
            const size_t n = bar ? size_t(bar - w) : std::strlen(w);
            if (std::strlen(text) == n && std::strncmp(text, w, n) == 0) {
                out = idx;
                return true;
            }
            w += n + (bar ? 1 : 0);
        }
        return false;
    }
    if (!*text) return false;
    char *end = nullptr;
    errno = 0;
    const long long x = std::strtoll(text, &end, 0);
    if (errno || *end || x < s.lo || x > s.hi) return false;
    out = x;
    return true;
}

inline int read_knobs(Knobs &k, char *err, size_t err_len) {
    for (int i = 0; i < kKnobCount; ++i) {
        const KnobSpec &s = kKnobTable[i];
        k.v[i] = s.def;
        const char *e = std::getenv(s.name);
        if (!e) continue;
        if (!parse_knob(s, e, k.v[i])) {
            if (s.words)
                std::snprintf(err, err_len, "%s=%s: not one of %s", s.name, e, s.words);
            else
                std::snprintf(err, err_len, "%s=%s: not an integer in [%lld, %lld]", s.name, e,
                              (long long)s.lo, (long long)s.hi);
            return i + 1;
        }
    }
    return 0;
}

inline const Knobs &process_knobs() {
    static const Knobs k = [] {
        Knobs r;
        char err[160];
        if (read_knobs(r, err, sizeof err))
            for (int i = 0; i < kKnobCount; ++i) r.v[i] = kKnobTable[i].def;
        return r;
    }();
    return k;
}

}
```

Measured before the change: 6894.

## Scan stream tails lazily in rounds driven by suspended chain walkers

For pipelined large-window calls, the tile kernel now scans only each stream's body tiles. The tail tiles, roughly the last max_length of each stream, are scanned in up to RC_TAIL_ROUNDS small rounds on the chain stream, and each round covers only as far as the suspended chain walkers need next. The chain kernel gains a lazy mode that saves its position and cut count and resumes after each round, with a final round that scans whatever is left. This aims to skip reading tail bytes the cut search never reaches. In exchange it adds several extra launches and serialisation on the chain stream per call, plus new descriptor layout and test knobs.

```diff
diff --git a/include/replicat_chunker.h b/include/replicat_chunker.h
--- a/include/replicat_chunker.h
+++ b/include/replicat_chunker.h
@@ -96,6 +96,10 @@
 int rc_tile_schedule(uint64_t n_tiles, uint32_t waves, uint32_t permille, uint32_t chunk,
                      uint32_t dyn_min, uint32_t *ranges, uint64_t cap, uint64_t *n_units);
 
+int rc_lazy_tail_split(uint64_t max_length, uint64_t L, uint64_t P, uint64_t *tiles,
+                       uint64_t *body_tiles);
+int rc_chunker_tail_scanned(rc_chunker *ch, uint32_t *rounds, uint64_t *scanned, uint64_t cap);
+
 int rc_tables_key(const uint8_t *key16, uint64_t n, const uint64_t *ds, uint64_t *out,
                   uint32_t *top16);
 
diff --git a/replicat_amd/_lib.py b/replicat_amd/_lib.py
--- a/replicat_amd/_lib.py
+++ b/replicat_amd/_lib.py
@@ -79,6 +79,8 @@
     'rc_group_hot_threshold': (_u32, [_p]),
     'rc_tile_keys': (_u64, []),
     'rc_tile_schedule': (_int, [_u64, _u32, _u32, _u32, _u32, _p, _u64, ctypes.POINTER(_u64)]),
+    'rc_lazy_tail_split': (_int, [_u64, _u64, _u64, ctypes.POINTER(_u64), ctypes.POINTER(_u64)]),
+    'rc_chunker_tail_scanned': (_int, [_p, ctypes.POINTER(_u32), _p, _u64]),
     'rc_blake2b_create': (_int, [_u32, _int, ctypes.POINTER(_p)]),
     'rc_blake2b_destroy': (None, [_p]),
     'rc_blake2b_digest_size': (_u32, [_p]),
diff --git a/replicat_amd/csrc/capi.cpp b/replicat_amd/csrc/capi.cpp
--- a/replicat_amd/csrc/capi.cpp
+++ b/replicat_amd/csrc/capi.cpp
@@ -145,6 +145,7 @@
         hipEvent_t done = nullptr;
         bool pending = false;
         bool piped = false;
+        uint32_t lazy_rounds = 0;
     } ws[2];
     unsigned next_ws = 0;
 
@@ -179,6 +180,9 @@
     uint64_t seg_bytes = 0, seg_cap = 0;
     bool any_multi = false;
     size_t bytes = 0;
+    bool lazy = false;
+    uint64_t n_tail = 0;
+    uint64_t xt_tail_off = 0, lz_off = 0;
 };
 
 StreamDesc desc_view(void *base, uint64_t n) {
@@ -245,32 +249,12 @@
 
 int stage_descriptors(rc_chunker *ch, Workspace &ws, uint64_t n, const uint8_t *const *ptrs,
                       const uint64_t *lens, const uint64_t *last, Plan &plan, bool open = false,
-                      bool single = false, uint64_t walkers = 0) {
+                      bool single = false, uint64_t walkers = 0, bool lazy_ok = false) {
     plan.n = n;
     if (ws.pending) {
         RC_HIP_TRY(hipEventSynchronize(ws.done));
         ws.pending = false;
     }
-    std::vector<uint64_t> &xt = ws.xtiles;
-    xt.clear();
-    {
-        uint64_t tiles = 0;
-        for (uint64_t i = 0; i < n; ++i) {
-            const uint64_t L = lens[i], P = open ? L : (last ? last[i] : 0);
-            const uint64_t jneed = rc_keys_needed(ch->max_length, L, P);
-            const uint64_t nt = jneed ? jneed / kTileKeys + 1 : 0;
-            const uint64_t jmax = L >= 8 ? (L - 4) / 4 : 0;
-            auto fast = [&](uint64_t t) { return L >= 8 && t * kTileKeys + kTileKeys - 1 <= jmax; };
-            if (nt && !fast(0)) xt.push_back(tiles);
-            if (nt > 1 && !fast(nt - 1)) xt.push_back(tiles + nt - 1);
-            tiles += nt;
-        }
-    }
-    plan.bytes = (9 * n + 3 + xt.size()) * sizeof(uint64_t);
-    if (int rc = ws.h_desc.ensure(plan.bytes)) return rc;
-    uint64_t *u = static_cast<uint64_t *>(ws.h_desc.p);
-    u[9 * n + 2] = xt.size();
-    std::copy(xt.begin(), xt.end(), u + 9 * n + 3);
     {
         const uint64_t kChainWalkers = walkers ? walkers : 4096;
         uint64_t total = 0;
@@ -289,7 +273,50 @@
         plan.seg_bytes = seg;
         plan.seg_cap = seg / step + ch->ext_steps + 4;
     }
-    uint64_t tiles = 0, cuts = 0, segs = 0, scratch = 0;
+    plan.lazy = lazy_ok;
+    uint64_t all_tail = 0, all_body = 0;
+    for (uint64_t i = 0; i < n && plan.lazy; ++i) {
+        uint64_t b = 0, nt = 0, nb = 0;
+        const uint64_t P = open ? lens[i] : (last ? last[i] : 0);
+        if (!single && argmax_bound(ch->max_length, lens[i], P, b) && b / plan.seg_bytes != 0)
+            plan.lazy = false;
+        rc_lazy_tail_split(ch->max_length, lens[i], P, &nt, &nb);
+        all_tail += nt - nb;
+        all_body += nb;
+    }
+    if (all_tail * 1000 > all_body * (uint64_t)ch->knobs[knTailShare]) plan.lazy = false;
+    std::vector<uint64_t> &xt = ws.xtiles;
+    std::vector<uint64_t> xt_tail;
+    xt.clear();
+    {
+        uint64_t tiles = 0;
+        for (uint64_t i = 0; i < n; ++i) {
+            const uint64_t L = lens[i], P = open ? L : (last ? last[i] : 0);
+            uint64_t nt = 0, nb = 0;
+            rc_lazy_tail_split(ch->max_length, L, P, &nt, &nb);
+            if (!plan.lazy) nb = nt;
+            const uint64_t jmax = L >= 8 ? (L - 4) / 4 : 0;
+            auto fast = [&](uint64_t t) { return L >= 8 && t * kTileKeys + kTileKeys - 1 <= jmax; };
+            auto list = [&](uint64_t t) { (t < nb ? xt : xt_tail).push_back(tiles + t); };
+            if (nt && !fast(0)) list(0);
+            if (nt > 1 && !fast(nt - 1)) list(nt - 1);
+            tiles += nt;
+        }
+    }
+    plan.xt_tail_off = 9 * n + 3 + xt.size();
+    plan.lz_off = plan.xt_tail_off + 1 + xt_tail.size();
+    plan.bytes = (plan.lazy ? plan.lz_off + 8 * n + 1 : plan.xt_tail_off) * sizeof(uint64_t);
+    if (int rc = ws.h_desc.ensure(plan.bytes)) return rc;
+    uint64_t *u = static_cast<uint64_t *>(ws.h_desc.p);
+    u[9 * n + 2] = xt.size();
+    std::copy(xt.begin(), xt.end(), u + 9 * n + 3);
+    uint64_t *lz = nullptr;
+    if (plan.lazy) {
+        u[plan.xt_tail_off] = xt_tail.size();
+        std::copy(xt_tail.begin(), xt_tail.end(), u + plan.xt_tail_off + 1);
+        lz = u + plan.lz_off;
+    }
+    uint64_t tiles = 0, cuts = 0, segs = 0, scratch = 0, tail = 0;
     plan.any_multi = false;
     for (uint64_t i = 0; i < n; ++i) {
         const uint64_t L = lens[i], P = open ? L : (last ? last[i] : 0);
@@ -309,14 +336,28 @@
         u[2 * n + i] = P;
         u[3 * n + i] = jneed;
         u[4 * n + i] = tiles;
+        if (plan.lazy) {
+            uint64_t nt = 0, nb = 0;
+            rc_lazy_tail_split(ch->max_length, L, P, &nt, &nb);
+            lz[i] = tail;
+            lz[n + 1 + i] = nb;
+            lz[2 * n + 1 + i] = tiles + nb - tail;
+            lz[3 * n + 1 + i] = std::min(L, nb * kTileKeys * 4);
+            lz[4 * n + 1 + i] = lz[5 * n + 1 + i] = nb * kTileKeys;
+            lz[6 * n + 1 + i] = lz[7 * n + 1 + i] = 0;
+            tail += nt - nb;
+        }
         tiles += jneed ? jneed / kTileKeys + 1 : 0;
         const uint64_t cap = cut_cap_of(ch->min_length, L);
         u[5 * n + 1 + i] = cuts;
-        u[6 * n + 1 + i] = cap;
+        const uint64_t cap_max = (uint64_t)ch->knobs[knCutCapMax];
+        u[6 * n + 1 + i] = cap_max ? std::min(cap, cap_max) : cap;
         cuts += cap;
     }
     u[5 * n] = tiles;
     u[8 * n + 1] = segs;
+    if (plan.lazy) lz[n] = tail;
+    plan.n_tail = tail;
     if (tiles >= (1ull << 32) - (1ull << 20))
         return rc_fail(RC_ERR_ARGUMENT, "too many bytes in one call: %llu tiles", (unsigned long long)tiles);
     plan.n_tiles = tiles;
@@ -335,9 +376,13 @@
     return reinterpret_cast<uint32_t *>(group_records(ws, plan) + plan.n_tiles + 1);
 }
 
+uint32_t *tail_tie_lists(Workspace &ws, const Plan &plan) {
+    return tie_lists(ws, plan) + rc_tie_list_words(plan.n_tiles);
+}
+
 size_t records_bytes(const Plan &plan) {
     return (plan.n_tiles + 1) * (sizeof(TileRecord) + sizeof(GroupRecord)) +
-           rc_tie_list_words(plan.n_tiles) * 4;
+           (rc_tie_list_words(plan.n_tiles) + (plan.lazy ? rc_tie_list_words(plan.n_tail) : 0)) * 4;
 }
 
 int ensure_ctr(Workspace &ws, hipStream_t st) {
@@ -412,6 +457,23 @@
     prm.fault = reinterpret_cast<const uint64_t *>(static_cast<uint32_t *>(ws.d_ctr.p) + kCtrStampWord);
     prm.epoch = ++ws.epoch;
     const StreamDesc d = desc_view(ws.d_desc.p, plan.n);
+    StreamDesc d_body = d, d_tail = d, d_tedge = d;
+    TileWindow win{};
+    const uint32_t rounds = plan.lazy && plan.n_tail ? (uint32_t)ch->knobs[knTailRounds] : 0u;
+    uint32_t *scanned = static_cast<uint32_t *>(ws.d_ctr.p) + kCtrScannedWord;
+    if (plan.lazy) {
+        uint64_t *lz = static_cast<uint64_t *>(ws.d_desc.p) + plan.lz_off;
+        const uint64_t n = plan.n;
+        d_tail.tile_base = lz;
+        d_tedge.xtiles = static_cast<uint64_t *>(ws.d_desc.p) + plan.xt_tail_off;
+        d_body.len = lz + 3 * n + 1;
+        prm.lz = LazyState{lz + 4 * n + 1, lz + 5 * n + 1, lz + 6 * n + 1, lz + 7 * n + 1};
+        win.have = prm.lz.have;
+        win.want = prm.lz.want;
+        win.body = lz + n + 1;
+        win.rec_off = lz + 2 * n + 1;
+        win.spare = plan.n_tiles;
+    }
     std::array<hipEvent_t, 4> ev{};
     if (ch->timing) {
         for (int k = 0; k < 4; ++k) {
@@ -436,7 +498,7 @@
     }
     prm.lean = ch->small && plan.max_len < (16ull << 30) ? 1u : 0u;
     prm.hot = group_hot_threshold(ch->window);
-    if (int rc = rc_launch_tiles(ch->d_tables, d, plan.n, plan.n_tiles,
+    if (int rc = rc_launch_tiles(ch->d_tables, plan.lazy ? d_body : d, plan.n, plan.n_tiles,
                                  static_cast<TileRecord *>(ws.d_records.p), grp, prm.hot, tie_lists(ws, plan),
                                  static_cast<uint32_t *>(ws.d_ctr.p), prm.epoch, ts,
                                  ch->timing ? ev[1] : nullptr,
@@ -450,15 +512,31 @@
         return abandon_launch(ws, ts, xs, rc_fail(RC_ERR_HIP, "hipEventRecord failed"));
     const uint32_t join = (ch->knobs[knJoinWalk] ? RC_JOIN_WALK_ONLY : 0u) |
                           (ch->knobs[knRepair] ? RC_JOIN_REPAIR : 0u);
-    if (int rc = rc_launch_chain(ch->d_tables, d, plan.n, prm, plan.n_segs,
-                                 static_cast<const TileRecord *>(ws.d_records.p), d_cuts, d_counts,
-                                 static_cast<uint64_t *>(ws.d_scratch.p),
-                                 static_cast<uint64_t *>(ws.d_seg_counts.p), plan.any_multi, join, xs))
-        return abandon_launch(ws, ts, xs, rc);
+    if (rounds && hipMemsetAsync(scanned, 0, 4 * kCtrScannedWords, xs) != hipSuccess)
+        return abandon_launch(ws, ts, xs, rc_fail(RC_ERR_HIP, "hipMemsetAsync failed"));
+    for (uint32_t r = 0; r <= rounds; ++r) {
+        if (r) {
+            win.closing = r == rounds ? 1u : 0u;
+            win.scanned = scanned + (r - 1);
+            if (int rc = rc_launch_tail_round(ch->d_tables, d_tail, d_tedge, plan.n, plan.n_tail, win,
+                                              static_cast<TileRecord *>(ws.d_records.p),
+                                              tail_tie_lists(ws, plan),
+                                              static_cast<uint32_t *>(ws.d_ctr.p), prm.epoch, xs,
+                                              ch->reserve, ch->sched))
+                return abandon_launch(ws, ts, xs, rc);
+        }
+        prm.lz_final = r == rounds ? 1u : 0u;
+        if (int rc = rc_launch_chain(ch->d_tables, d, plan.n, prm, plan.n_segs,
+                                     static_cast<const TileRecord *>(ws.d_records.p), d_cuts, d_counts,
+                                     static_cast<uint64_t *>(ws.d_scratch.p),
+                                     static_cast<uint64_t *>(ws.d_seg_counts.p), plan.any_multi, join, xs))
+            return abandon_launch(ws, ts, xs, rc);
+    }
     if (hipEventRecord(ws.done, xs) != hipSuccess)
         return abandon_launch(ws, ts, xs, rc_fail(RC_ERR_HIP, "hipEventRecord failed"));
     ws.pending = true;
     ws.piped = pipelined;
+    ws.lazy_rounds = rounds;
     if (ch->timing) {
         RC_HIP_TRY(hipEventRecord(ev[3], xs));
         ch->ev_rec.push_back(ev);
@@ -533,6 +611,8 @@
     p.hot = 0;
     p.fault = nullptr;
     p.epoch = 0;
+    p.lz = LazyState{nullptr, nullptr, nullptr, nullptr};
+    p.lz_final = 0;
     return p;
 }
 
@@ -569,6 +649,33 @@
     if (!any) return 0;
     const uint64_t jneed = bound / 4 + T, jmax = (L - 4) / 4;
     return std::min(jneed, jmax);
+}
+
+int rc_lazy_tail_split(uint64_t max_length, uint64_t L, uint64_t P, uint64_t *tiles,
+                       uint64_t *body_tiles) {
+    if (!tiles || !body_tiles) return rc_fail(RC_ERR_ARGUMENT, "null argument");
+    const uint64_t jneed = rc_keys_needed(max_length, L, P);
+    uint64_t bound = 0;
+    *tiles = *body_tiles = 0;
+    if (!jneed || !argmax_bound(max_length, L, P, bound)) return RC_OK;
+    *tiles = jneed / kTileKeys + 1;
+    *body_tiles = std::min(*tiles, bound / 4 / kTileKeys + 1);
+    return RC_OK;
+}
+
+int rc_chunker_tail_scanned(rc_chunker *ch, uint32_t *rounds, uint64_t *scanned, uint64_t cap) {
+    if (!ch || !rounds) return rc_fail(RC_ERR_ARGUMENT, "null argument");
+    std::lock_guard<std::mutex> lock(ch->mu);
+    DeviceGuard g(ch->device);
+    Workspace &ws = ch->ws[(ch->next_ws - 1) & 1];
+    *rounds = ws.lazy_rounds;
+    if (ws.pending) RC_HIP_TRY(hipEventSynchronize(ws.done));
+    uint32_t h[kCtrScannedWords] = {};
+    if (ws.lazy_rounds)
+        RC_HIP_TRY(hipMemcpy(h, static_cast<uint32_t *>(ws.d_ctr.p) + kCtrScannedWord, sizeof h,
+                             hipMemcpyDeviceToHost));
+    for (uint32_t r = 0; r < ws.lazy_rounds && r < cap && scanned; ++r) scanned[r] = h[r];
+    return RC_OK;
 }
 
 int rc_chunker_create(uint64_t min_length, uint64_t max_length, const uint8_t *key,
@@ -785,8 +892,11 @@
     ch->pipelined_calls += pipelined ? 1 : 0;
     Plan plan;
     Workspace &ws = acquire_ws(ch);
+    const bool lazy_ok = pipelined && !(flags & RC_PIPELINE_END) && !open && !ch->small &&
+                         !ch->groups && ch->window / kTileKeys + 3 > 64 &&
+                         ch->knobs[knTailRounds] > 0;
     if (int rc = stage_descriptors(ch, ws, n, d_streams, lens, last_piece, plan, open, false,
-                                   pipelined ? 16ull * ch->reserve : 0))
+                                   pipelined ? 16ull * ch->reserve : 0, lazy_ok))
         return rc;
     return upload_and_launch(ch, ws, plan, chain_params(ch, plan, ~0ull, flags), d_cuts, d_counts,
                              static_cast<hipStream_t>(hip_stream), pipelined,
diff --git a/replicat_amd/csrc/gclmul.h b/replicat_amd/csrc/gclmul.h
--- a/replicat_amd/csrc/gclmul.h
+++ b/replicat_amd/csrc/gclmul.h
@@ -59,6 +59,20 @@
     return below >= 65536 ? 0u : (uint32_t)(65536 - below);
 }
 
+constexpr uint64_t kLazyDone = ~0ull;
+struct LazyState {
+    uint64_t *have, *want, *pos, *ncut;
+};
+
+struct TileWindow {
+    const uint64_t *have, *want;
+    const uint64_t *body;
+    const uint64_t *rec_off;
+    uint64_t spare;
+    uint32_t *scanned;
+    uint32_t closing;
+};
+
 struct ChainParams {
     uint64_t min_length;
     uint64_t max_length;
@@ -75,9 +89,12 @@
     uint32_t hot;
     const uint64_t *fault;
     uint64_t epoch;
+    LazyState lz;
+    uint32_t lz_final;
 };
 
 constexpr uint32_t kCtrErrWord = 32, kCtrStampWord = 34, kCtrFaultsWord = 36;
+constexpr uint32_t kCtrScannedWord = 8, kCtrScannedWords = 16;
 constexpr int64_t kCountFault = -3;
 
 struct TileSched {
@@ -102,6 +119,11 @@
                     uint32_t hot, uint32_t *d_xlist, uint32_t *d_ctr, uint64_t epoch,
                     void *stream, void *mid_event, uint32_t cus, void *edge_stream, void *tiled,
                     rc::TileSched sched);
+int rc_launch_tail_round(const rc::KeyTables *d_tables, rc::StreamDesc tail_desc,
+                         rc::StreamDesc desc, uint64_t n_streams, uint64_t n_tail_tiles,
+                         rc::TileWindow win, rc::TileRecord *d_records, uint32_t *d_xlist,
+                         uint32_t *d_ctr, uint64_t epoch, void *stream, uint32_t cus,
+                         rc::TileSched sched);
 uint64_t rc_tie_list_words(uint64_t n_tiles);
 enum : uint32_t { RC_JOIN_WALK_ONLY = 1, RC_JOIN_REPAIR = 2 };
 int rc_launch_chain(const rc::KeyTables *d_tables, rc::StreamDesc desc, uint64_t n_streams,
diff --git a/replicat_amd/csrc/kernels.hip b/replicat_amd/csrc/kernels.hip
--- a/replicat_amd/csrc/kernels.hip
+++ b/replicat_amd/csrc/kernels.hip
@@ -324,13 +324,17 @@
     return pk_max_u16_s(pk_max_u16_s(r0, r1), pk_max_u16_s(r2, r3));
 }
 
-template <bool kCache, bool kClip = false>
+template <bool kCache, bool kClip = false, bool kWin = false>
 struct TileCursor {
     StreamDesc d;
     uint64_t s, cur, next;
     const uint8_t *base;
     uint32_t nfast;
     uint32_t nlast;
+    TileWindow win;
+    uint32_t wlo, whi;
+    uint64_t jbase;
+    uint64_t roff;
     __device__ void enter() {
         if constexpr (!kCache) return;
         base = sload_ptr(d.ptr + s);
@@ -341,6 +345,16 @@
             const uint64_t jl = sload(d.jneed + s) - (next - cur - 1) * kTileKeys;
             nlast = jl < (uint64_t)kTileKeys ? (uint32_t)(jl >> 8) + 1u : (uint32_t)kTileIters;
         }
+        if constexpr (kWin) {
+            const uint64_t nb = sload(win.body + s);
+            const uint64_t lo = sload(win.have + s) / kTileKeys;
+            const uint64_t hi = win.closing ? ~0ull : sload(win.want + s) / kTileKeys;
+            const uint64_t a = max(lo, nb), b = min(hi, (uint64_t)nfast);
+            wlo = (uint32_t)(a - nb);
+            whi = b > a ? (uint32_t)(b - nb) : wlo;
+            jbase = nb * kTileKeys;
+            roff = sload(win.rec_off + s);
+        }
     }
     __device__ void init(const StreamDesc &dd, uint64_t n_streams, uint64_t t) {
         d = dd;
@@ -367,7 +381,12 @@
         TileRef r;
         r.j0 = (t - cur) * kTileKeys;
         r.s = (uint32_t)s;
-        if constexpr (kCache) {
+        if constexpr (kWin) {
+            static_assert(kCache && !kClip, "the windowed cursor caches and does not clip");
+            r.j0 += jbase;
+            r.base = base;
+            r.fast = t - cur >= wlo && t - cur < whi ? (uint32_t)kTileIters : 0u;
+        } else if constexpr (kCache) {
             r.base = base;
             r.fast = t - cur < nfast ? (kClip && t + 1 == next ? nlast : (uint32_t)kTileIters) : 0u;
         } else {
@@ -377,6 +396,9 @@
         return r;
     }
 };
+
+__device__ __forceinline__ TileWindow window_of() { return TileWindow{}; }
+__device__ __forceinline__ TileWindow window_of(const TileWindow &w) { return w; }
 
 __device__ __forceinline__ void stage_tile_tables_nb(const KeyTables *tab) {
     const uint32_t nt = blockDim.x;
@@ -538,7 +560,7 @@
     }
 };
 
-template <int G, bool kGroup>
+template <int G, bool kGroup, typename... W>
 __global__ __launch_bounds__(1024) void rc_tile_kernel(const KeyTables *__restrict__ tab,
                                                        StreamDesc d, uint64_t n_streams,
                                                        TileUnits U,
@@ -547,7 +569,10 @@
                                                        uint32_t hot,
                                                        uint32_t *__restrict__ xlist,
                                                        uint32_t *__restrict__ xcount,
-                                                       uint32_t *__restrict__ ctr) {
+                                                       uint32_t *__restrict__ ctr, W... window) {
+    constexpr bool kWin = sizeof...(W) != 0;
+    static_assert(!kWin || G == 1, "windowed launches: large windows only (no group records)");
+    const TileWindow wnd = window_of(window...);
     UnitGrab<kGroup> grab;
     grab.start(U, ctr);
     stage_tile_tables_nb(tab);
@@ -566,7 +591,10 @@
     uint32_t n_ties = 0;
     RC_TILE_STAMP_BEGIN();
 
-    TileCursor<true, (G > 1)> cursor;
+    TileCursor<true, (G > 1), kWin> cursor;
+    uint64_t cur_roff = 0, nx_roff = 0;
+    uint32_t n_scanned = 0;
+    if constexpr (kWin) cursor.win = wnd;
     TileRef cur;
     uint64_t t = ub;
     bool seek = true;
@@ -575,6 +603,7 @@
             if (seek) cursor.init(d, n_streams, t);
             seek = false;
             cur = cursor.at(t);
+            if constexpr (kWin) cur_roff = cursor.roff;
             if (cur.fast) break;
             ++t;
             continue;
@@ -597,6 +626,7 @@
         }
     }
     uint64_t pend_t = n_tiles;
+    if constexpr (kWin) pend_t = wnd.spare;
     uint64_t pend_jm = 0;
     uint64_t pend_mask = 0;
     uint32_t pend_st = 0;
@@ -635,6 +665,7 @@
         for (;;) {
             if (tn < nue) {
                 nx = cursor.at(tn);
+                if constexpr (kWin) nx_roff = cursor.roff;
                 if (nx.fast) break;
                 ++tn;
                 continue;
@@ -675,9 +706,10 @@
                 if ((lane >> 2) == q) jl = f * 256 + c * 4 + (lane & 3);
             }
         }
-        if (lane == 0) xlist[ub + n_ties] = (uint32_t)t;
+        if (lane == 0) xlist[ub + n_ties] = (uint32_t)(t + cur_roff);
         n_ties += tie ? 1u : 0u;
-        pend_t = t;
+        pend_t = t + cur_roff;
+        if constexpr (kWin) ++n_scanned;
         pend_jm = cur.j0 | ((uint64_t)M << 48);
         pend_mask = tie ? cmask : (nc >= 16 ? ~0ull : (1ull << (4 * nc)) - 1);
         pend_st = (tie ? 0x80000000u : 0u) | (uint32_t)cur.s;
@@ -696,10 +728,12 @@
         if (!nx.fast) break;
         t = tn;
         cur = nx;
+        if constexpr (kWin) cur_roff = nx_roff;
     }
     retire();
     if (lane == 0) {
         xcount[u] = n_ties;
+        if constexpr (kWin) atomicAdd(wnd.scanned, n_scanned);
         RC_TILE_STAMP_END(gw);
     }
 }
@@ -762,6 +796,7 @@
     }
 }
 
+template <typename... W>
 __global__ __launch_bounds__(256) void rc_edge_kernel(const KeyTables *__restrict__ tab,
                                                       StreamDesc d, uint64_t n_streams,
                                                       TileUnits U,
@@ -769,7 +804,10 @@
                                                       GroupRecord *__restrict__ grp,
                                                       const uint32_t *__restrict__ xlist,
                                                       const uint32_t *__restrict__ xcount,
-                                                      uint32_t *__restrict__ ctr, uint64_t epoch) {
+                                                      uint32_t *__restrict__ ctr, uint64_t epoch,
+                                                      W... window) {
+    constexpr bool kWin = sizeof...(W) != 0;
+    const TileWindow win = window_of(window...);
     __shared__ __attribute__((aligned(16))) uint64_t s_full[2048];
     __shared__ uint32_t s_fault;
     if (threadIdx.x == 0) {
@@ -827,7 +865,14 @@
                 }
             } else {
                 const uint64_t t = sload(d.xtiles + 1 + (e - n_units));
-                exact_tile(tl, th, d, stream_of_tile(d, n_streams, t), t, rec, grp);
+                const uint64_t s = stream_of_tile(d, n_streams, t);
+                if constexpr (kWin) {
+                    const uint64_t k = t - sload(d.tile_base + s);
+                    if (k < sload(win.have + s) / kTileKeys ||
+                        (!win.closing && k >= sload(win.want + s) / kTileKeys))
+                        continue;
+                }
+                exact_tile(tl, th, d, s, t, rec, grp);
             }
         }
     }
@@ -1307,7 +1352,7 @@
     return lo;
 }
 
-template <int R, bool kLean>
+template <int R, bool kLean, bool kLazy = false>
 __global__ __launch_bounds__(kChainWaves * 64) void rc_spec_kernel(const KeyTables *__restrict__ tab,
                                                       StreamDesc d, uint64_t n_streams,
                                                       ChainParams prm, uint64_t n_segs,
@@ -1343,6 +1388,14 @@
 
     uint64_t pos = i * prm.seg_bytes, n = 0, ext = 0;
     bool overflow = false, term = false;
+    uint64_t have = ~0ull, want = 0;
+    bool suspend = false;
+    if constexpr (kLazy) {
+        pos = sload(prm.lz.pos + s);
+        if (pos == kLazyDone) return;
+        n = sload(prm.lz.ncut + s);
+        if (!prm.lz_final) have = sload(prm.lz.want + s);
+    }
     RecCache<R> cache;
     auto emit = [&](uint64_t c) {
         if (n >= cap) {
@@ -1358,6 +1411,16 @@
             break;
         }
         if (!direct && pos >= seg_end && ext++ >= prm.ext_steps) break;
+        if constexpr (kLazy) {
+            const bool argmax = (st.P >= pos && st.P - pos >= prm.max_length) ||
+                                st.L - pos >= 2 * prm.max_length;
+            const uint64_t jb = min((pos >> 2) + prm.window, st.jmax);
+            if (argmax && jb >= have) {
+                suspend = true;
+                want = (jb / kTileKeys + 1) * kTileKeys;
+                break;
+            }
+        }
         uint64_t c1 = 0, c2 = 0;
         int kind;
         if constexpr (kLean) {
@@ -1378,6 +1441,16 @@
         }
         if (overflow) break;
         pos = c1;
+    }
+    if constexpr (kLazy) {
+        if (lane == 0) {
+            prm.lz.have[s] = suspend ? have : kLazyDone;
+            prm.lz.want[s] = suspend ? want : kLazyDone;
+            prm.lz.pos[s] = suspend ? pos : kLazyDone;
+            prm.lz.ncut[s] = n;
+            if (!suspend) counts[s] = overflow ? -1 : (int64_t)n;
+        }
+        return;
     }
     if (lane == 0) {
         if (direct) {
@@ -2217,10 +2290,39 @@
     uint64_t egrid = (U.n_units + 3) / 4;
     if (egrid > 4 * cus) egrid = 4 * cus;
     if (egrid == 0) egrid = 1;
-    hipLaunchKernelGGL(rc_edge_kernel, dim3((unsigned)egrid), dim3(256), 0, est, d_tables, desc,
+    hipLaunchKernelGGL(rc_edge_kernel<>, dim3((unsigned)egrid), dim3(256), 0, est, d_tables, desc,
                        n_streams, U, d_records, d_grp, (const uint32_t *)d_xlist,
                        (const uint32_t *)d_xcount, d_ctr, epoch);
     return launch_status("rc_edge_kernel");
+}
+
+int rc_launch_tail_round(const KeyTables *d_tables, StreamDesc tail_desc, StreamDesc desc,
+                         uint64_t n_streams, uint64_t n_tail_tiles, TileWindow win,
+                         TileRecord *d_records, uint32_t *d_xlist, uint32_t *d_ctr, uint64_t epoch,
+                         void *stream, uint32_t cus, TileSched sched) {
+    if (n_tail_tiles == 0) return 0;
+    hipStream_t st = (hipStream_t)stream;
+    const uint64_t waves_per_wg = 1024 / kWaveSize;
+    uint64_t grid = (n_tail_tiles + waves_per_wg - 1) / waves_per_wg;
+    if (grid > cus) grid = cus;
+    const TileUnits U = tile_units(n_tail_tiles, grid * waves_per_wg, sched);
+    uint32_t *d_xcount = d_xlist + n_tail_tiles;
+    if (U.n_groups != 0)
+        hipLaunchKernelGGL((rc_tile_kernel<1, true, TileWindow>), dim3((unsigned)grid), dim3(1024), 0, st,
+                           d_tables, tail_desc, n_streams, U, d_records, (GroupRecord *)nullptr, 0u,
+                           d_xlist, d_xcount, d_ctr, win);
+    else
+        hipLaunchKernelGGL((rc_tile_kernel<1, false, TileWindow>), dim3((unsigned)grid), dim3(1024), 0, st,
+                           d_tables, tail_desc, n_streams, U, d_records, (GroupRecord *)nullptr, 0u,
+                           d_xlist, d_xcount, d_ctr, win);
+    if (int rc = launch_status("rc_tile_kernel (tail round)")) return rc;
+    uint64_t egrid = (U.n_units + 3) / 4;
+    if (egrid > 4 * (uint64_t)cus) egrid = 4 * (uint64_t)cus;
+    if (egrid == 0) egrid = 1;
+    hipLaunchKernelGGL(rc_edge_kernel<TileWindow>, dim3((unsigned)egrid), dim3(256), 0, st, d_tables, desc,
+                       n_streams, U, d_records, (GroupRecord *)nullptr, (const uint32_t *)d_xlist,
+                       (const uint32_t *)d_xcount, d_ctr, epoch, win);
+    return launch_status("rc_edge_kernel (tail round)");
 }
 
 int rc_tile_schedule(uint64_t n_tiles, uint32_t waves, uint32_t permille, uint32_t chunk,
@@ -2246,6 +2348,16 @@
                     uint64_t *d_seg_counts, bool any_multi, uint32_t join, void *stream) {
     if (n_streams == 0) return 0;
     hipStream_t st = (hipStream_t)stream;
+    if (prm.lz.pos) {
+        if (any_multi || n_segs != n_streams || prm.lean || prm.grp || prm.max_steps == 0)
+            return rc_fail(RC_ERR_ARGUMENT, "lazy tails: not a large-window one-segment call");
+        const uint64_t grid = (n_segs + kChainWaves - 1) / kChainWaves;
+        hipLaunchKernelGGL((rc_spec_kernel<kRecUnroll, false, true>), dim3((unsigned)grid),
+                           dim3(kChainWaves * kWaveSize), 0, st, d_tables, desc, n_streams, prm,
+                           n_segs, d_records, d_cuts, d_counts, d_scratch, d_seg_counts,
+                           d_seg_counts);
+        return launch_status("rc_spec_kernel (lazy)");
+    }
     if (prm.lane && prm.lean && prm.grp && !any_multi && n_segs == n_streams &&
         prm.max_steps != 0 && prm.window / kTileKeys <= (uint64_t)kLaneFull) {
         const bool narrow = prm.window / kTileKeys <= 4;
diff --git a/replicat_amd/csrc/knobs.h b/replicat_amd/csrc/knobs.h
--- a/replicat_amd/csrc/knobs.h
+++ b/replicat_amd/csrc/knobs.h
@@ -31,6 +31,9 @@
     knTileGroup,
     knTileMask,
     knHostBatchBytes,
+    knTailRounds,
+    knTailShare,
+    knCutCapMax,
     kKnobCount
 };
 
@@ -99,6 +102,19 @@
      "rc_chunk_host / rc_chunk_digest_host: bytes of whole streams per double-buffered batch "
      "(a stream longer than this is a batch of its own); test switch: a small value sends a "
      "few MiB through many batches, so the suite can check slot reuse and output offsets"},
+    {"RC_TAIL_ROUNDS", 3, 0, 16, nullptr,
+     "lazy tails: pipelined large-window calls read each stream's last max_length or so in this "
+     "many rounds on the chain stream, each round only as far as the stopped chains' next "
+     "windows reach, the last one whatever is left (1: that round alone); 0: every call reads "
+     "all its tiles in the one tile launch"},
+    {"RC_TAIL_SHARE", 100, 0, int64_t(1) << 30, nullptr,
+     "lazy tails: a call is lazy only when its tail tiles are at most this many per mille of "
+     "its body tiles, so that the rounds fit beside the next body launch (100: streams of about "
+     "12 max_lengths or more; the suite raises it to run the rounds on short streams)"},
+    {"RC_CUT_CAP_MAX", 0, 0, int64_t(1) << 40, nullptr,
+     "test switch: the kernels see at most this cut capacity per stream (0: no limit; the "
+     "arrays keep the layout of rc_cut_capacity), so the suite can check that a stream whose "
+     "cuts do not fit reports RC_COUNT_OVERFLOW"},
 };
 
 struct Knobs {
```

After: 7024 (median of 6 runs). 1.02x the previous value.
